# Ghostish/Open3DSOT

Hardware: AMD Instinct MI355X
Metric: template/search pairs/sec (fwd+bwd), BAT KITTI-Car 512/1024 pts (higher is better)
Workload: dtype f32; 1 GPU; BAT_Car.yaml KITTI-Car, template 512 / search 1024 pts, batch 48 per GPU, fwd+bwd+Adam, fp32; global_batch=48, parallelism=dp1, fused_kernels=True, hip_graph=True, rccl_world_size=1

## Files before the change

include/o3dsot.h:

```cpp
#ifndef O3DSOT_H_
#define O3DSOT_H_

#include <stdint.h>

#ifdef __cplusplus
extern "C" {
#endif

#define O3D_OK 0
#define O3D_EINVAL (-1)
#define O3D_ELAUNCH (-2)

const char* o3d_version(void);

int o3d_furthest_point_sampling(const float* xyz, int B, int N, int npoint, float* temp,
                                int32_t* idx, void* stream);

int o3d_furthest_point_sampling_shfl(const float* xyz, int B, int N, int npoint, float* temp, int32_t* idx,
                                     void* stream);

int o3d_furthest_point_sampling_pair(const float* xyz0, int N0, int npoint0, int32_t* idx0, const float* xyz1,
                                     int N1, int npoint1, int32_t* idx1, int B, void* stream);

int o3d_gather_points(const float* feats, const int32_t* idx, int B, int C, int N, int npoint,
                      float* out, void* stream);
int o3d_gather_points_grad(const float* grad_out, const int32_t* idx, int B, int C, int N,
                           int npoint, float* grad_feats, void* stream);

int o3d_gather_rows(const float* src, const int32_t* idx, int B, int N, int D, int npoint, float* out, void* stream);

int o3d_gather_rows2(const float* a, int Da, const float* b, int Db, const int32_t* idx, long ld_idx, int B, int N, int npoint,
                     float* outa, float* outb, void* stream);

int o3d_ball_query(const float* new_xyz, const float* xyz, int B, int N, int npoint, float radius,
                   int nsample, int32_t* idx, void* stream);

int o3d_sample_query(const float* xyz0, const int32_t* sidx0, int N0, int npoint0, int32_t* idx0, const float* xyz1,
                     const int32_t* sidx1, int N1, int npoint1, int32_t* idx1, int B, float radius, int nsample,
                     float* centers, void* stream);

int o3d_group_points(const float* feats, const int32_t* idx, int B, int C, int N, int npoint,
                     int nsample, float* out, void* stream);
int o3d_group_points_grad(const float* grad_out, const int32_t* idx, int B, int C, int N,
                          int npoint, int nsample, float* grad_feats, void* stream);

int o3d_three_nn(const float* unknown, const float* known, int B, int n, int m, float* dist2,
                 int32_t* idx, void* stream);
int o3d_three_interpolate(const float* feats, const int32_t* idx, const float* weight, int B,
                          int c, int m, int n, float* out, void* stream);
int o3d_three_interpolate_grad(const float* grad_out, const int32_t* idx, const float* weight,
                               int B, int c, int n, int m, float* grad_feats, void* stream);

int o3d_knn(const float* query, const float* ref, int B, int Q, int R, int D, int k,
            int32_t* idx, void* stream);



int o3d_mlp_conv_fwd(const float* X, const float* W, const float* in_scale, const float* in_shift,
                     int B, int Cin, int Cout, int P, float* Y, float* part, const float* stat_c,
                     void* stream);

typedef struct {
    const float* part; int nparts, C; double count; const float* stat_c; const float* gamma; const float* beta;
    float* running_mean; float* running_var; float momentum, eps; float* mean; float* invstd; float* scale; float* shift;
    const int32_t* meta; int tile, nparts1; double count1;
} o3d_bn_fin_args;
int o3d_bn_finalize(const o3d_bn_fin_args* jobs, int njobs, void* stream);

int o3d_bn_relu_maxpool_fwd(const float* Y, const float* scale, const float* shift, int B, int C,
                            int npoint, int ns, float* out, int32_t* arg, float* yarg, void* stream);

int o3d_pool_bwd_partials_split(const float* dOut, const float* out, const float* yarg, const float* mean, int C,
                                int npoint, int nsplit, float* part, const int32_t* arg, float* pk, void* stream);

typedef struct {
    const float* part; int nparts, C; double count; const float* gamma; const float* mean; const float* invstd;
    float* dgamma; float* dbeta; float* A1; float* A2; float* A3;
    const int32_t* meta; int tile, nparts1; double count1;
} o3d_bn_bwd_fin_args;
int o3d_bn_bwd_finalize(const o3d_bn_bwd_fin_args* jobs, int njobs, void* stream);

int o3d_mlp_conv_dgrad(const float* dN, const float* dOut, const float* out, const int32_t* arg,
                       int ns, const float* Y, const float* A1, const float* A2, const float* A3,
                       const float* W, int B, int Cin, int Cout, int P, const float* Yprev,
                       const float* scale_p, const float* shift_p, const float* mean_p,
                       float* dNprev, float* part, void* stream);

int o3d_mlp_conv_dgrad_wt(const float* dN, const float* dOut, const float* out, const int32_t* arg,
                          int ns, const float* Y, const float* A1, const float* A2, const float* A3,
                          const float* W, const float* Wt, const float* pk, int B, int Cin, int Cout, int P,
                          const float* Yprev, const float* scale_p, const float* shift_p,
                          const float* mean_p, float* dNprev, float* part, void* stream);

int o3d_mlp_conv_dgrad_plain(const float* dN, const float* Y, const float* A1, const float* A2,
                             const float* A3, const float* W, int B, int Cin, int Cout, int P,
                             float* dX, void* stream);

int o3d_mlp_conv_wgrad(const float* dN, const float* dOut, const float* out, const int32_t* arg, int ns,
                       const float* Y, const float* A1, const float* A2, const float* A3,
                       const float* X, const float* in_scale, const float* in_shift, int B, int Cin, int Cout,
                       int P, int nslices, float* part, float* dW, void* stream);


int o3d_compact_build(const int32_t* idx, int B, int npoint, int ns, int ld, int col_base, int pt_base,
                      int ball_base, int dummy_ball, int32_t* ball_cnt, int32_t* ball_off, int32_t* gp,
                      int32_t* cball, float* cw, int32_t* meta, void* stream);

int o3d_group_dw0_xyz(const float* dN, const float* Y0, long ldp, const float* A1, const float* A2, const float* A3,
                      const int32_t* gp, const int32_t* cball, const float* cw, const float* X, long ldz,
                      const float* centers, const int32_t* meta, long start1, int C0, float* part, float* dW, void* stream);

int o3d_compact_build2(const int32_t* idx0, int npoint0, int ld0, const int32_t* idx1, int npoint1, int ld1, int B,
                       int ns, int col_base1, int pt_base1, int dummy_ball, int32_t* ball_cnt, int32_t* ball_off,
                       int32_t* gp, int32_t* cball, float* cw, int32_t* meta, void* stream);

int o3d_group_expand_c(const float* Z, long ldz, const int32_t* gp, const int32_t* cball, const float* cw,
                       const float* centers, const float* W0, int ldw, int C0, const int32_t* meta, long start1,
                       long ldp, float* Y0, float* part, const float* stat_c, void* stream);

int o3d_group_expand_c3(const float* X3, long ldz, const int32_t* gp, const int32_t* cball, const float* cw,
                        const float* centers, const float* W0, int ldw, int C0, const int32_t* meta, long start1, long ldp,
                        float* Y0, float* part, const float* stat_c, void* stream);

int o3d_direct_tile(long P, int M, int compact);
int o3d_direct_tail_slots(int M);
int o3d_direct_tail_override(int slots);
int o3d_direct_class(long ldp, int M, int K, int tile);
int o3d_mlp_conv_fwd_c(const float* X, const float* W, const float* in_scale, const float* in_shift, int Cin,
                       int Cout, long ldp, const float* w, const int32_t* meta, long start1, int tile, float* Y,
                       float* part, const float* stat_c, void* stream);
int o3d_mlp_conv_dgrad_c(const float* dN, const float* Y, const float* A1, const float* A2, const float* A3,
                         const float* Wt, int Cin, int Cout, long ldp, const float* w, const int32_t* meta,
                         long start1, int tile, const float* Yprev, const float* scale_p, const float* shift_p,
                         const float* mean_p, float* dNprev, float* part, void* stream);
int o3d_mlp_conv_wgrad2_c(const float* dN, const float* Y, const float* A1, const float* A2, const float* A3,
                          const float* X, const float* in_scale, const float* in_shift, int Cin, int Cout,
                          long ldp, const float* w, const int32_t* meta, long start1, float* scratch, float* dW,
                          void* stream);

int o3d_pool_fwd_c(const float* Y, long ldp, const float* scale, const float* shift, const int32_t* ball_off,
                   const int32_t* ball_cnt, int B, int C, int npoint0, int npoint1, float* out, int32_t* argq,
                   float* yarg, void* stream);

int o3d_pool_fwd_ct(const float* Y, long ldp, const float* scale, const float* shift, const int32_t* ball_off,
                    const int32_t* ball_cnt, const int32_t* cball, const int32_t* meta, long start1, int B, int C,
                    int npoint0, int npoint1, int nsample, float* out, int32_t* argq, float* yarg, void* stream);

#define O3D_POOL_BWD_SPLIT 8
int o3d_pool_bwd_c(const float* dOut, const float* out, const int32_t* argq, const float* yarg,
                   const float* mean, int B, int C, int npoint0, int npoint1, const int32_t* meta, long start1,
                   long ldp, float* D, float* part, void* stream);

int o3d_pool_bwd_dense(const float* dOut0, long sb0, long sc0, const float* dOut1, long sb1, long sc1, const float* out,
                       const int32_t* argq, const float* yarg, const float* mean,
                       const int32_t* cball, const int32_t* ball_off, const int32_t* meta, long start1, long ldp, int B,
                       int C, int npoint0, int npoint1, float* D, float* part, void* stream);

long o3d_group_reduce_gather_scratch(int B, int nseg, int npoint0, int ld0, int npoint1, int ld1, int spanmax);
int o3d_group_reduce_gather(const float* dN, const float* Y0, long ldp, const float* A1, const float* A2,
                            const float* A3, const int32_t* gp, const float* cw, const int32_t* ball_off,
                            const int32_t* ball_cnt, int B, int nseg, int npoint0, int ld0, int npoint1, int ld1, int C0,
                            int spanmax, int32_t* perm, int32_t* poff, float* S, float* T, void* stream);

int o3d_pack_points(const float* xyz0, const float* feats0, int N0, int ld0, const float* xyz1, const float* feats1,
                    int N1, int ld1, int B, int nxyz, int C, float inv_radius, int rows, float* X0, void* stream);

int o3d_center_term(const float* T, const float* centers, int C0, int nballs, int ldw, float* dW, void* stream);
int o3d_center_term_out(const float* T, const float* centers, int C0, int nballs, int ldw, const float* dW, int ncols,
                        float* out, void* stream);

int o3d_center_grad(const float* T, const float* W0, int ldw, int C0, int nballs, float scale, float* out, void* stream);

int o3d_group_reduce_c(const float* dN, const float* Y0, long ldp, const float* A1, const float* A2,
                       const float* A3, const int32_t* gp, const int32_t* cball, const float* cw,
                       const int32_t* ball_off, const int32_t* ball_cnt, int B, int nseg, int npoint0, int ld0,
                       int npoint1, int ld1, int C0, float* S, float* T, void* stream);

int o3d_bn_relu_apply(const float* Y, const float* scale, const float* shift, int C, long P, float* out,
                      void* stream);
int o3d_act_bwd_partials(const float* g, const float* Y, const float* scale, const float* shift,
                         const float* mean, int C, long P, float* dN, float* part, void* stream);
int o3d_gmax_fwd(const float* Y, const float* scale, const float* shift, int B, int C, int N, float* out,
                 int32_t* argq, float* yarg, void* stream);

long o3d_mlp_conv_wgrad2_scratch(int B, int Cin, int Cout, int P);
int o3d_mlp_conv_wgrad2(const float* dN, const float* pk, int ns, const float* Y, const float* A1,
                        const float* A2, const float* A3, const float* X, const float* in_scale,
                        const float* in_shift, int B, int Cin, int Cout, int P, float* scratch, float* dW,
                        void* stream);

typedef struct { const float* p; long sb, sc, sn; int C; } o3d_rows_src;

int o3d_pack_rows(const o3d_rows_src* srcs, int nsrc, int B, int N, int rows, float* X, void* stream);
int o3d_pack_rows_ld(const o3d_rows_src* srcs, int nsrc, int B, int N, int rows, float* X, long ld, void* stream);

int o3d_rpn_votes_fwd(const float* cla, long cla_sb, long cla_sn, const float* vote, long v_sb, long v_sc, long v_sn, int B, int N,
                      int f, float* score, float* vote_xyz, float* vote_feature, void* stream);
int o3d_rpn_votes_bwd(const float* score, const float* dvf, long f_sb, long f_sc, long f_sn, const float* dvx, long x_sb, long x_sc,
                      long x_sn, int B, int N, int f, float* dcla, float* dvote, void* stream);
int o3d_box_assemble(const float* offsets, long o_sb, long o_sc, long o_sn, const float* centers, int B, int P, float* boxes,
                     void* stream);

int o3d_prep_weights(const long* jobs, int njobs, void* stream);

int o3d_row_sum(const float* G, int C, long P, float* out, void* stream);

int o3d_pw_tile(long P, int M);
int o3d_pw_class(long P, int M, int K);

int o3d_mlp_conv_bwd_fused_rows(int Cin, int Cout, long P);
long o3d_mlp_conv_bwd_fused_scratch(int Cin, int Cout, long P);
int o3d_mlp_conv_bwd_fused_c(const float* dN, const float* Y, const float* A1, const float* A2, const float* A3,
                             const float* X, const float* in_scale, const float* in_shift, const float* in_mean,
                             const float* Wt, int Cin, int Cout, long ldp, const float* w, const int32_t* meta,
                             long start1, float* scratch, float* dW, float* part_s, float* dNprev, void* stream);

typedef struct {
    const float* X; const float* W; const float* in_scale; const float* in_shift; const float* bias; const float* resid;
    int Cin, Cout; long P;
    float* Y; float* part; const float* stat_c;
} o3d_pw_fwd_args;
typedef struct {
    const float* dN; const float* Y; const float* A1; const float* A2; const float* A3; const float* Wt;
    int Cin, Cout; long P;
    const float* Yprev; const float* scale_p; const float* shift_p; const float* mean_p; const float* resid;
    float* dNprev; float* part;
} o3d_pw_dgrad_args;
int o3d_pw_fwd_pair(const o3d_pw_fwd_args* a, const o3d_pw_fwd_args* b, void* stream);
int o3d_pw_dgrad_pair(const o3d_pw_dgrad_args* a, const o3d_pw_dgrad_args* b, void* stream);

typedef struct {
    const float* dN; const float* Y; const float* A1; const float* A2; const float* A3;
    const float* X; const float* in_scale; const float* in_shift;
    int Cin, Cout; long P;
    float* scratch; float* dW;
    int out_rows, out_cols;
} o3d_wgrad_job;
int o3d_mlp_conv_wgrad2_group(const o3d_wgrad_job* jobs, int njobs, void* stream);

int o3d_adam_step(const long* jobs, int njobs, float* params, float* exp_avg, float* exp_avg_sq, double lr,
                  double beta1, double beta2, double eps, double weight_decay, double bc1, double bc2, void* stream);

int o3d_best_proposal(const float* boxes, int B, int P, float* out, int32_t* out_idx, void* stream);

int o3d_pw_fwd_cloud(const float* X, const float* W, const float* cbias, int B, int N, int Cin, int Cout, float* Y,
                     float* part, const float* stat_c, void* stream);
int o3d_cloud_sum_dy(const float* dN, const float* Y, const float* A1, const float* A2, const float* A3, int C, int B,
                     int N, float* out, void* stream);

int o3d_bn_eval_consts(const float* running_mean, const float* running_var, const float* gamma, const float* beta,
                       const float* conv_bias, float eps, int C, int nrep, float* vec, void* stream);

int o3d_pw_fwd(const float* X, const float* W, const float* in_scale, const float* in_shift, const float* bias,
               const float* resid, int Cin, int Cout, long P, float* Y, float* part, const float* stat_c,
               void* stream);

int o3d_pw_dgrad(const float* dN, const float* Y, const float* A1, const float* A2, const float* A3,
                 const float* Wt, int Cin, int Cout, long P, const float* Yprev, const float* scale_p,
                 const float* shift_p, const float* mean_p, const float* resid, float* dNprev, float* part,
                 void* stream);

int o3d_xcorr_expand(const float* Z, long ldz, const float* sim, const float* W0, int ldw, int B, int M, int N, int C0,
                     float* Y0, float* part, const float* stat_c, void* stream);

long o3d_xcorr_reduce_groups(int C0);
int o3d_xcorr_reduce(const float* dN, const float* Y0, const float* A1, const float* A2, const float* A3,
                     const float* sim, const float* W0, int ldw, int B, int M, int N, int C0, float* S, long lds,
                     float* dsim_part, float* dw_part, void* stream);

int o3d_sa_eval_fused(const float* Z, long ldz, const int32_t* idx, const float* centers, const float* W0, int ldw,
                      const float* v0, const float* W1, const float* v1, const float* W2, const float* v2, int C0, int C1,
                      int C2, int B, int np, int ns, int ld, long pt_base, float* out, void* stream);

int o3d_cosine_sim_fwd(const float* t, long tsb, long tsc, long tsn, const float* s, long ssb, long ssc, long ssn, int B, int f,
                       int M, int N, float* sim, float* tn, float* sn, void* stream);
// ... 166 lines not shown
```

open3dsot_amd/csrc/compact.hip:

```cpp
#include <cstdlib>
#include "o3d_common.hpp"

namespace {

__global__ __launch_bounds__(256) void compact_count_kernel(const int32_t* __restrict__ idx, long nslots, int ns,
                                                            int32_t* __restrict__ ball_cnt) {
    const long s = (long)blockIdx.x * 256 + threadIdx.x;
    const int lane = threadIdx.x & 63;
    const int v = s < nslots ? idx[s] : -1;
    const int base = lane & ~(ns - 1), k = lane - base;
    const int first = __shfl(v, base, 64);
    const unsigned long long m = __ballot(v != first);
    const unsigned long long seg = ns == 64 ? ~0ull : (((1ull << ns) - 1) << base);
    const unsigned long long other = m & seg;
    if (k == 0 && s < nslots) ball_cnt[s / ns] = other ? (63 - __clzll((long long)other)) - base + 1 : 1;
}

__global__ __launch_bounds__(1024) void compact_scan_kernel(const int32_t* __restrict__ ball_cnt, int n,
                                                            int col_base, int32_t* __restrict__ ball_off,
                                                            int32_t* __restrict__ meta) {
    __shared__ int sh[1024];
    const int per = (n + 1023) / 1024;
    const int i0 = threadIdx.x * per;
    int local = 0;
    for (int i = i0; i < i0 + per && i < n; ++i) local += ball_cnt[i];
    sh[threadIdx.x] = local;
    __syncthreads();
    for (int off = 1; off < 1024; off <<= 1) {
        const int v = (int)threadIdx.x >= off ? sh[threadIdx.x - off] : 0;
        __syncthreads();
        sh[threadIdx.x] += v;
        __syncthreads();
    }
    int run = col_base + sh[threadIdx.x] - local;
    for (int i = i0; i < i0 + per && i < n; ++i) {
        ball_off[i] = run;
        run += ball_cnt[i];
    }
    if (threadIdx.x == 1023) {
        const int tot = sh[1023];
        meta[0] = (tot + 255) & ~255;
        meta[1] = tot;
        meta[2] = n;
        meta[3] = 0;
    }
}

__global__ __launch_bounds__(256) void compact_fill_kernel(const int32_t* __restrict__ idx, long nslots, int ns,
                                                           int npoint, int ld, int col_base, int pt_base,
                                                           int ball_base, int dummy_ball,
                                                           const int32_t* __restrict__ ball_cnt,
                                                           const int32_t* __restrict__ ball_off,
                                                           const int32_t* __restrict__ meta,
                                                           int32_t* __restrict__ gp, int32_t* __restrict__ cball,
                                                           float* __restrict__ cw) {
    if (blockIdx.x == gridDim.x - 1) {
        const int q = meta[1] + threadIdx.x;
        if (q < meta[0]) { gp[col_base + q] = 0; cball[col_base + q] = dummy_ball; cw[col_base + q] = 0.f; }
        return;
    }
    const long s = (long)blockIdx.x * 256 + threadIdx.x;
    if (s >= nslots) return;
    const int ball = (int)(s / ns), k = (int)(s - (long)ball * ns);
    const int cnt = ball_cnt[ball];
    if (k >= cnt) return;
    const int q = ball_off[ball] + k;
    gp[q] = pt_base + (ball / npoint) * ld + idx[s];
    cball[q] = ball_base + ball;
    cw[q] = k == 0 ? (float)(1 + ns - cnt) : 1.f;
}

template <bool CENTERS, bool DIRECT = false>
__global__ __launch_bounds__(256) void expand_c_kernel(const float* __restrict__ Z, long ldz,
                                                       const int32_t* __restrict__ gp,
                                                       const int32_t* __restrict__ cball,
                                                       const float* __restrict__ cw,
                                                       const float* __restrict__ centers,
                                                       const float* __restrict__ W0, int ldw, int C0,
                                                       const int32_t* __restrict__ meta, long start1, long ldp,
                                                       float* __restrict__ Y0, float* __restrict__ part,
                                                       const float* __restrict__ stat_c) {
    const int q0 = blockIdx.x * 256;
    const int seg = (start1 > 0 && q0 >= start1) ? 1 : 0;
    if (q0 - (seg ? start1 : 0) >= meta[4 * seg]) return;
    if (stat_c && seg) stat_c += C0;
    const int lane = threadIdx.x & 63, wave = threadIdx.x >> 6;
    const int q = q0 + 4 * lane;
    const int4 id = *reinterpret_cast<const int4*>(&gp[q]);
    const float4 w = *reinterpret_cast<const float4*>(&cw[q]);
    float cx[4] = {0.f, 0.f, 0.f, 0.f}, cy[4] = {0.f, 0.f, 0.f, 0.f}, cz[4] = {0.f, 0.f, 0.f, 0.f};
    if constexpr (CENTERS) {
        const int4 bj = *reinterpret_cast<const int4*>(&cball[q]);
        const int bb[4] = {bj.x, bj.y, bj.z, bj.w};
#pragma unroll
        for (int t = 0; t < 4; ++t) {
            const float* c = centers + (long)bb[t] * 3;
            cx[t] = c[0]; cy[t] = c[1]; cz[t] = c[2];
        }
        if constexpr (DIRECT) {
            const int ids[4] = {id.x, id.y, id.z, id.w};
#pragma unroll
            for (int t = 0; t < 4; ++t) { cx[t] -= Z[ids[t]]; cy[t] -= Z[ldz + ids[t]]; cz[t] -= Z[2 * ldz + ids[t]]; }
        }
    }
    constexpr int EG = 8;
    const int cper = (C0 + gridDim.y - 1) / gridDim.y;
    const int cbeg = blockIdx.y * cper, cend = cbeg + cper < C0 ? cbeg + cper : C0;
    for (int g0 = cbeg + wave; g0 < cend; g0 += 4 * EG) {
        float4 y[EG];
        float w0[EG], w1[EG], w2[EG], sc_[EG];
#pragma unroll
        for (int g = 0; g < EG; ++g) {
            const int co = g0 + 4 * g < cend ? g0 + 4 * g : cend - 1;
            if constexpr (DIRECT) {
                y[g] = make_float4(0.f, 0.f, 0.f, 0.f);
            } else {
                const float* z = Z + (long)co * ldz;
                y[g].x = z[id.x]; y[g].y = z[id.y]; y[g].z = z[id.z]; y[g].w = z[id.w];
            }
            w0[g] = w1[g] = w2[g] = 0.f;
            if constexpr (CENTERS) { const float* wr = W0 + (long)co * ldw; w0[g] = wr[0]; w1[g] = wr[1]; w2[g] = wr[2]; }
            sc_[g] = (part && stat_c) ? stat_c[co] : 0.f;
        }
        float s[EG], v[EG];
#pragma unroll
        for (int g = 0; g < EG; ++g) {
            const int co = g0 + 4 * g;
            if (co >= cend) { s[g] = 0.f; v[g] = 0.f; continue; }
            y[g].x -= fmaf(w2[g], cz[0], fmaf(w1[g], cy[0], w0[g] * cx[0]));
            y[g].y -= fmaf(w2[g], cz[1], fmaf(w1[g], cy[1], w0[g] * cx[1]));
            y[g].z -= fmaf(w2[g], cz[2], fmaf(w1[g], cy[2], w0[g] * cx[2]));
            y[g].w -= fmaf(w2[g], cz[3], fmaf(w1[g], cy[3], w0[g] * cx[3]));
            *reinterpret_cast<float4*>(&Y0[(long)co * ldp + q]) = y[g];
            const float c = sc_[g];
            s[g] = fmaf(w.x, y[g].x, fmaf(w.y, y[g].y, fmaf(w.z, y[g].z, w.w * y[g].w)));
            v[g] = w.x * (y[g].x - c) * (y[g].x - c) + w.y * (y[g].y - c) * (y[g].y - c) +
                   w.z * (y[g].z - c) * (y[g].z - c) + w.w * (y[g].w - c) * (y[g].w - c);
        }
        if (part) {
#pragma unroll
            for (int g = 0; g < EG; ++g) { s[g] = wave_sum(s[g]); v[g] = wave_sum(v[g]); }
            if (lane == 0)
#pragma unroll
                for (int g = 0; g < EG; ++g) {
                    const int co = g0 + 4 * g;
                    if (co < cend) {
                        part[((long)blockIdx.x * 2 + 0) * C0 + co] = s[g];
                        part[((long)blockIdx.x * 2 + 1) * C0 + co] = v[g];
                    }
                }
        }
    }
}

constexpr int POOL_BWD_SPLIT = 8;

__device__ __forceinline__ long pool_index(int c, int ball, int C, int seg1_ball, int np0, int np1) {
    const bool s1 = ball >= seg1_ball;
    const int local = s1 ? ball - seg1_ball : ball, np = s1 ? np1 : np0;
    const int b = local / np, j = local - b * np;
    return (s1 ? (long)seg1_ball * C : 0) + ((long)b * C + c) * np + j;
}

template <int POOL_CH>
__global__ __launch_bounds__(256) void pool_c_kernel(const float* __restrict__ Y, long ldp,
                                                     const float* __restrict__ scale,
                                                     const float* __restrict__ shift,
                                                     const int32_t* __restrict__ ball_off,
                                                     const int32_t* __restrict__ ball_cnt, int C, int seg1_ball,
                                                     int np0, int np1, int nballs, float* __restrict__ out,
                                                     int32_t* __restrict__ argq, float* __restrict__ yarg) {
    const int e = threadIdx.x & 7;
    int ball = blockIdx.x * 32 + (threadIdx.x >> 3);
    const bool live = ball < nballs;
    if (!live) ball = nballs - 1;
    const int q0 = ball_off[ball], q1 = q0 + ball_cnt[ball];
    const int c0 = blockIdx.y * POOL_CH;
    if (ball >= seg1_ball) { scale += C; shift += C; }
    constexpr int PU = 4;
    float v[POOL_CH][PU], sc[POOL_CH], sf[POOL_CH];
#pragma unroll
    for (int cc = 0; cc < POOL_CH; ++cc) {
        const int c = c0 + cc < C ? c0 + cc : C - 1;
        const float* y = Y + (long)c * ldp;
#pragma unroll
        for (int i = 0; i < PU; ++i) {
            const int q = q0 + e + 8 * i;
            v[cc][i] = y[q < q1 ? q : q1 - 1];
        }
        sc[cc] = scale[c];
        sf[cc] = shift[c];
    }
    float rbest[POOL_CH], ryb[POOL_CH];
    int rbq[POOL_CH];
#pragma unroll
    for (int cc = 0; cc < POOL_CH; ++cc) {
        float best = -INFINITY, yb = 0.f;
        int bq = 0x7fffffff;
#pragma unroll
        for (int i = 0; i < PU; ++i) {
            const int q = q0 + e + 8 * i;
            const float n = fmaf(v[cc][i], sc[cc], sf[cc]);
            if (q < q1 && n > best) { best = n; bq = q; yb = v[cc][i]; }
        }
        if (q1 - q0 > 8 * PU) {
            const float* y = Y + (long)(c0 + cc < C ? c0 + cc : C - 1) * ldp;
            for (int q = q0 + e + 8 * PU; q < q1; q += 8) {
                const float w = y[q], n = fmaf(w, sc[cc], sf[cc]);
                if (n > best) { best = n; bq = q; yb = w; }
            }
        }
        {
            const float ob = dpp_f<0xB1>(best), oy = dpp_f<0xB1>(yb);
            const int oq = dpp_i<0xB1>(bq);
            if (ob > best || (ob == best && oq < bq)) { best = ob; bq = oq; yb = oy; }
        }
        {
            const float ob = dpp_f<0x4E>(best), oy = dpp_f<0x4E>(yb);
            const int oq = dpp_i<0x4E>(bq);
            if (ob > best || (ob == best && oq < bq)) { best = ob; bq = oq; yb = oy; }
        }
        {
            const float ob = dpp_f<0x141>(best), oy = dpp_f<0x141>(yb);
            const int oq = dpp_i<0x141>(bq);
            if (ob > best || (ob == best && oq < bq)) { best = ob; bq = oq; yb = oy; }
        }
        rbest[cc] = best; ryb[cc] = yb; rbq[cc] = bq;
    }
    if (live && e == 0) {
#pragma unroll
        for (int cc = 0; cc < POOL_CH; ++cc) {
            const int c = c0 + cc;
            if (c < C) {
                const long o = pool_index(c, ball, C, seg1_ball, np0, np1);
                out[o] = fmaxf(rbest[cc], 0.f);
                if (argq) { argq[o] = rbq[cc]; yarg[o] = ryb[cc]; }
            }
        }
    }
}

constexpr int PT_CH = 32, PT_COLS = 128, PT_OVER = 32, PT_LD = PT_COLS + PT_OVER + 3;
constexpr int PT_RB = 32, PT_RLD = PT_CH + 1;

__device__ __forceinline__ void pool_t_item(const float* __restrict__ Y, long ldp,
                                            const float* __restrict__ scale, const float* __restrict__ shift,
                                            const int32_t* __restrict__ ball_off,
                                            const int32_t* __restrict__ ball_cnt,
                                            const int32_t* __restrict__ cball,
                                            const int32_t* __restrict__ meta, long start1, int C,
                                            int seg1_ball, int np0, int np1, int nballs,
                                            float* __restrict__ out, int32_t* __restrict__ argq,
                                            float* __restrict__ yarg, const long q0, const int c0, float* pt_tile) {
    int* pt_off = reinterpret_cast<int*>(pt_tile + PT_CH * PT_LD);
    int* pt_cnt = pt_off + PT_COLS;
    int* pt_ob = pt_cnt + PT_COLS;
    float* pt_res = reinterpret_cast<float*>(pt_ob + PT_COLS);
    const int seg = (start1 > 0 && q0 >= start1) ? 1 : 0;
    const long sbase = seg ? start1 : 0;
    if (q0 - sbase >= meta[4 * seg]) return;
    const long qend = sbase + meta[4 * seg + 1];
    if (q0 >= qend) return;
    int bfirst = cball[q0];
    if (ball_off[bfirst] < q0) ++bfirst;
    const long qlast = (q0 + PT_COLS < qend ? q0 + PT_COLS : qend) - 1;
    const int blast = cball[qlast];
    const int nb = blast - bfirst + 1;
    const int np = seg ? np1 : np0;
    const long segbase = seg ? (long)seg1_ball * C : 0;
    const int ball0 = seg ? seg1_ball : 0;
    constexpr int F4 = (PT_COLS + PT_OVER) / 4;
    constexpr int NLD = PT_CH * F4 / 256;
    static_assert(PT_CH * F4 % 256 == 0, "tile loads must divide evenly over the workgroup");
    {
        float4 v[NLD];
        int bo = 0, bc = 0;
        if ((int)threadIdx.x < nb) { bo = ball_off[bfirst + threadIdx.x]; bc = ball_cnt[bfirst + threadIdx.x]; }
#pragma unroll
        for (int u = 0; u < NLD; ++u) {
            const int i = threadIdx.x + 256 * u;
            const int r = i / F4, f = i - r * F4;
            long q = q0 + 4 * f;
            if (q + 4 > ldp) q = ldp - 4;
            v[u] = *reinterpret_cast<const float4*>(&Y[(long)(c0 + r) * ldp + q]);
        }
        __builtin_amdgcn_sched_barrier(0);
// ... 456 lines not shown
#pragma unroll
            for (int c = 0; c < CS; ++c) {
                d[it][c] = *reinterpret_cast<const float4*>(&dN[(long)crow[c] * ldp + qc]);
                y[it][c] = *reinterpret_cast<const float4*>(&Y0[(long)crow[c] * ldp + qc]);
            }
        }
        __builtin_amdgcn_sched_barrier(0);
        __syncthreads();
#pragma unroll
        for (int it = 0; it < CH / 1024; ++it) {
            const int i = 4 * threadIdx.x + 1024 * it;
#pragma unroll
            for (int c = 0; c < CS; ++c) {
                float4 o;
                o.x = fmaf(a1[c], d[it][c].x, w4[it].x * fmaf(a2[c], y[it][c].x, a3[c]));
                o.y = fmaf(a1[c], d[it][c].y, w4[it].y * fmaf(a2[c], y[it][c].y, a3[c]));
                o.z = fmaf(a1[c], d[it][c].z, w4[it].z * fmaf(a2[c], y[it][c].z, a3[c]));
                o.w = fmaf(a1[c], d[it][c].w, w4[it].w * fmaf(a2[c], y[it][c].w, a3[c]));
                *reinterpret_cast<float4*>(&dy[c * CH + i]) = o;
            }
        }
#pragma unroll
        for (int u = 0; u < CH / 256; ++u) lst[threadIdx.x + 256 * u] = ent[u];
        __syncthreads();
        {
            const int per = (cnt + 255) / 256;
            const int e0 = threadIdx.x * per, e1 = e0 + per < cnt ? e0 + per : cnt;
            int cur = -1;
            float sr[CS];
#pragma unroll
            for (int c = 0; c < CS; ++c) sr[c] = 0.f;
            for (int a = e0; a < e1; ++a) {
                const int e = lst[a];
                const int n = e >> 16, i = e & 0xffff;
                if (n != cur) {
                    if (cur >= 0) {
#pragma unroll
                        for (int c = 0; c < CS; ++c) atomicAdd(&sacc[c * ld + cur], sr[c]);
                    }
                    cur = n;
#pragma unroll
                    for (int c = 0; c < CS; ++c) sr[c] = 0.f;
                }
#pragma unroll
                for (int c = 0; c < CS; ++c) sr[c] += dy[c * CH + i];
            }
            if (cur >= 0) {
#pragma unroll
                for (int c = 0; c < CS; ++c) atomicAdd(&sacc[c * ld + cur], sr[c]);
            }
        }
        if (T)
            for (int j = threadIdx.x; j < npoint; j += 256) {
                const int b0 = ball_off[bbase + j], b1 = b0 + ball_cnt[bbase + j];
                const int s0 = b0 > lo ? b0 : lo, s1 = b1 < hi ? b1 : hi;
                if (s0 >= s1) continue;
                float t[CS];
#pragma unroll
                for (int c = 0; c < CS; ++c) t[c] = 0.f;
                for (int q = s0; q < s1; ++q)
#pragma unroll
                    for (int c = 0; c < CS; ++c) t[c] += dy[c * CH + (q - lo)];
#pragma unroll
                for (int c = 0; c < CS; ++c) tacc[c * npoint + j] += t[c];
            }
    }
    __syncthreads();
    for (int i = threadIdx.x; i < CS * ld; i += 256) {
        const int c = i / ld, n = i - c * ld;
        if (c0 + c < C0) S[(long)(c0 + c) * lds_row + pbase + n] = sacc[i];
    }
    if (T)
        for (int i = threadIdx.x; i < CS * npoint; i += 256) {
            const int c = i / npoint, j = i - c * npoint;
            if (c0 + c < C0) T[(long)(c0 + c) * nballs + bbase + j] = tacc[i];
        }
}

__global__ __launch_bounds__(1024) void center_term_kernel(const float* __restrict__ T,
                                                           const float* __restrict__ centers, int nballs, int ldw,
                                                           float* __restrict__ dW, float* __restrict__ out = nullptr,
                                                           int ncols = 0) {
    __shared__ float red[16][3];
    const int c = blockIdx.x, tid = threadIdx.x;
    const float* t = T + (long)c * nballs;
    float s0 = 0.f, s1 = 0.f, s2 = 0.f;
    for (int ball = tid; ball < nballs; ball += 1024) {
        const float v = t[ball];
        s0 = fmaf(v, centers[3 * ball], s0);
        s1 = fmaf(v, centers[3 * ball + 1], s1);
        s2 = fmaf(v, centers[3 * ball + 2], s2);
    }
#pragma unroll
    for (int off = 32; off >= 1; off >>= 1) {
        s0 += __shfl_xor(s0, off, 64);
        s1 += __shfl_xor(s1, off, 64);
        s2 += __shfl_xor(s2, off, 64);
    }
    if ((tid & 63) == 0) { red[tid >> 6][0] = s0; red[tid >> 6][1] = s1; red[tid >> 6][2] = s2; }
    __syncthreads();
    if (tid < 3) {
        float a = 0.f;
#pragma unroll
        for (int w = 0; w < 16; ++w) a += red[w][tid];
        if (out) out[(long)c * ncols + tid] = dW[(long)c * ldw + tid] - a;
        else dW[(long)c * ldw + tid] -= a;
    }
    if (out)
        for (int k = 3 + tid; k < ncols; k += 1024) out[(long)c * ncols + k] = dW[(long)c * ldw + k];
}

struct PackSeg { const float* xyz; const float* feats; int N, ld; };

__global__ __launch_bounds__(256) void pack_points_kernel(PackSeg s0, PackSeg s1, int B, int nxyz, int C, float inv_radius,
                                                          long ldz, float* __restrict__ X0) {
    const long col = (long)blockIdx.x * 256 + threadIdx.x;
    if (col >= ldz) return;
    const int r = blockIdx.y;
    const long base1 = (long)B * s0.ld;
    const bool second = col >= base1;
    const PackSeg sg = second ? s1 : s0;
    const long local = second ? col - base1 : col;
    const int b = (int)(local / sg.ld), n = (int)(local - (long)b * sg.ld);
    float v = 0.f;
    if (n < sg.N) {
        if (r < nxyz) v = sg.xyz[((long)b * sg.N + n) * 3 + r] * inv_radius;
        else if (r < nxyz + C) v = sg.feats[((long)b * C + (r - nxyz)) * sg.N + n];
    }
    X0[(long)r * ldz + col] = v;
}

}

static bool pow2(int v) { return v > 0 && (v & (v - 1)) == 0; }
constexpr long O3D_MAX_BALLS = 1L << 20;

extern "C" int o3d_compact_build(const int32_t* idx, int B, int npoint, int ns, int ld, int col_base, int pt_base,
                                 int ball_base, int dummy_ball, int32_t* ball_cnt, int32_t* ball_off, int32_t* gp,
                                 int32_t* cball, float* cw, int32_t* meta, void* stream) {
    const long nballs = (long)B * npoint, nslots = nballs * ns;
    if (!idx || !ball_cnt || !ball_off || !gp || !cball || !cw || !meta || B <= 0 || npoint <= 0 || ns < 1 ||
        ns > 64 || !pow2(ns) || nballs > O3D_MAX_BALLS || nslots % 256 != 0 || ld <= 0 || col_base < 0 || col_base % 256 != 0)
        return O3D_EINVAL;
    hipStream_t s = o3d_stream(stream);
    const int blocks = (int)(nslots / 256);
    hipLaunchKernelGGL(compact_count_kernel, dim3(blocks), dim3(256), 0, s, idx, nslots, ns, ball_cnt);
    hipLaunchKernelGGL(compact_scan_kernel, dim3(1), dim3(1024), 0, s, ball_cnt, (int)nballs, col_base, ball_off, meta);
    hipLaunchKernelGGL(compact_fill_kernel, dim3(blocks + 1), dim3(256), 0, s, idx, nslots, ns, npoint, ld, col_base,
                       pt_base, ball_base, dummy_ball, ball_cnt, ball_off, meta, gp, cball, cw);
    return o3d_launch_status();
}

namespace {
template <int CPW>
__global__ __launch_bounds__(256) void dw0_xyz_kernel(const float* __restrict__ dN, const float* __restrict__ Y0, long ldp,
                                                      const float* __restrict__ A1, const float* __restrict__ A2,
                                                      const float* __restrict__ A3, const int32_t* __restrict__ gp,
                                                      const int32_t* __restrict__ cball, const float* __restrict__ cw,
                                                      const float* __restrict__ X, long ldz,
                                                      const float* __restrict__ centers,
                                                      const int32_t* __restrict__ meta, long start1, int C0,
                                                      float* __restrict__ part) {
    const long q0 = (long)blockIdx.x * 256;
    const int seg = (start1 > 0 && q0 >= start1) ? 1 : 0;
    float* prow = part + (long)blockIdx.x * C0 * 3;
    if (q0 - (seg ? start1 : 0) >= meta[4 * seg]) {
        for (int i = threadIdx.x; i < C0 * 3; i += 256) prow[i] = 0.f;
        return;
    }
    const int lane = threadIdx.x & 63, wave = threadIdx.x >> 6;
    const long q = q0 + 4 * lane;
    const int4 id = *reinterpret_cast<const int4*>(&gp[q]);
    const int4 bj = *reinterpret_cast<const int4*>(&cball[q]);
    const float4 w = *reinterpret_cast<const float4*>(&cw[q]);
    const int ids[4] = {id.x, id.y, id.z, id.w}, bb[4] = {bj.x, bj.y, bj.z, bj.w};
    const float wv[4] = {w.x, w.y, w.z, w.w};
    float rel[4][3];
#pragma unroll
    for (int t = 0; t < 4; ++t)
#pragma unroll
        for (int k = 0; k < 3; ++k)
            rel[t][k] = wv[t] != 0.f ? X[(long)k * ldz + ids[t]] - centers[(long)bb[t] * 3 + k] : 0.f;
    const float* a1 = A1 + seg * C0;
    const float* a2 = A2 + seg * C0;
    const float* a3 = A3 + seg * C0;
    for (int cbase = 0; cbase < C0; cbase += 4 * CPW) {
        float acc[CPW][3];
        float4 d[CPW], y[CPW];
#pragma unroll
        for (int i = 0; i < CPW; ++i) {
            const int c = cbase + wave + 4 * i;
            const int cc = c < C0 ? c : C0 - 1;
            d[i] = *reinterpret_cast<const float4*>(&dN[(long)cc * ldp + q]);
            y[i] = *reinterpret_cast<const float4*>(&Y0[(long)cc * ldp + q]);
        }
#pragma unroll
        for (int i = 0; i < CPW; ++i) {
            const int c = cbase + wave + 4 * i;
            const int cc = c < C0 ? c : C0 - 1;
            const float k1 = a1[cc], k2 = a2[cc], k3 = a3[cc];
            const float dv[4] = {d[i].x, d[i].y, d[i].z, d[i].w}, yv[4] = {y[i].x, y[i].y, y[i].z, y[i].w};
            float s0 = 0.f, s1 = 0.f, s2 = 0.f;
#pragma unroll
            for (int t = 0; t < 4; ++t) {
                const float dy = wv[t] != 0.f ? fmaf(k1, dv[t], wv[t] * fmaf(k2, yv[t], k3)) : 0.f;
                s0 = fmaf(dy, rel[t][0], s0); s1 = fmaf(dy, rel[t][1], s1); s2 = fmaf(dy, rel[t][2], s2);
            }
            acc[i][0] = s0; acc[i][1] = s1; acc[i][2] = s2;
        }
#pragma unroll
        for (int i = 0; i < CPW; ++i) {
            const int c = cbase + wave + 4 * i;
#pragma unroll
            for (int k = 0; k < 3; ++k) {
                const float t = wave_sum(acc[i][k]);
                if (lane == 0 && c < C0) prow[c * 3 + k] = t;
            }
        }
    }
}

__global__ __launch_bounds__(256) void dw0_reduce_kernel(const float* __restrict__ part, int nblk, int n,
                                                         float* __restrict__ out) {
    __shared__ float sh[4];
    const int i = blockIdx.x;
    float s = 0.f;
    for (int r = threadIdx.x; r < nblk; r += 256) s += part[(long)r * n + i];
    s = wave_sum(s);
    if ((threadIdx.x & 63) == 0) sh[threadIdx.x >> 6] = s;
    __syncthreads();
    if (threadIdx.x == 0) out[i] = (sh[0] + sh[1]) + (sh[2] + sh[3]);
}
}

extern "C" int o3d_group_dw0_xyz(const float* dN, const float* Y0, long ldp, const float* A1, const float* A2,
                                 const float* A3, const int32_t* gp, const int32_t* cball, const float* cw,
                                 const float* X, long ldz, const float* centers, const int32_t* meta, long start1, int C0,
                                 float* part, float* dW, void* stream) {
    if (!dN || !Y0 || !A1 || !A2 || !A3 || !gp || !cball || !cw || !X || !centers || !meta || !part || !dW || C0 <= 0 ||
        ldp <= 0 || ldp % 256 != 0 || ldz <= 0 || start1 < 0 || start1 % 256 != 0)
        return O3D_EINVAL;
    hipStream_t s = o3d_stream(stream);
    const int nblk = (int)(ldp / 256);
    hipLaunchKernelGGL(dw0_xyz_kernel<8>, dim3(nblk), dim3(256), 0, s, dN, Y0, ldp, A1, A2, A3, gp, cball, cw, X, ldz, centers,
                       meta, start1, C0, part);
    hipLaunchKernelGGL(dw0_reduce_kernel, dim3(C0 * 3), dim3(256), 0, s, part, nblk, C0 * 3, dW);
    return o3d_launch_status();
}

namespace {
struct CompactSeg {
    const int32_t* idx; long nslots; int npoint, ld, col_base, pt_base, ball_base, nballs;
    int32_t* ball_cnt; int32_t* ball_off; int32_t* meta;
};

__global__ __launch_bounds__(256) void compact_count2_kernel(CompactSeg s0, CompactSeg s1, int ns, int blocks0) {
    const bool second = (int)blockIdx.x >= blocks0;
    const CompactSeg& sg = second ? s1 : s0;
    const long s = (long)(blockIdx.x - (second ? blocks0 : 0)) * 256 + threadIdx.x;
    const int lane = threadIdx.x & 63;
    const int v = s < sg.nslots ? sg.idx[s] : -1;
    const int base = lane & ~(ns - 1), k = lane - base;
    const int first = __shfl(v, base, 64);
    const unsigned long long m = __ballot(v != first);
    const unsigned long long seg = ns == 64 ? ~0ull : (((1ull << ns) - 1) << base);
    const unsigned long long other = m & seg;
    if (k == 0 && s < sg.nslots) sg.ball_cnt[s / ns] = other ? (63 - __clzll((long long)other)) - base + 1 : 1;
}

__global__ __launch_bounds__(1024) void compact_scan2_kernel(CompactSeg s0, CompactSeg s1) {
    const CompactSeg& sg = blockIdx.x ? s1 : s0;
    const int n = sg.nballs;
    __shared__ int sh[1024];
    const int per = (n + 1023) / 1024;
    const int i0 = threadIdx.x * per;
    int local = 0;
    for (int i = i0; i < i0 + per && i < n; ++i) local += sg.ball_cnt[i];
    sh[threadIdx.x] = local;
    __syncthreads();
    for (int off = 1; off < 1024; off <<= 1) {
        const int v = (int)threadIdx.x >= off ? sh[threadIdx.x - off] : 0;
        __syncthreads();
        sh[threadIdx.x] += v;
        __syncthreads();
    }
    int run = sg.col_base + sh[threadIdx.x] - local;
    for (int i = i0; i < i0 + per && i < n; ++i) {
        sg.ball_off[i] = run;
        run += sg.ball_cnt[i];
    }
    if (threadIdx.x == 1023) {
        const int tot = sh[1023];
        sg.meta[0] = (tot + 255) & ~255;
        sg.meta[1] = tot;
        sg.meta[2] = n;
        sg.meta[3] = 0;
    }
}

__global__ __launch_bounds__(256) void compact_fill2_kernel(CompactSeg s0, CompactSeg s1, int ns, int blocks0, int dummy_ball,
                                                            int32_t* __restrict__ gp, int32_t* __restrict__ cball,
                                                            float* __restrict__ cw) {
    const bool second = (int)blockIdx.x >= blocks0 + 1;
    const CompactSeg& sg = second ? s1 : s0;
    const int blk = blockIdx.x - (second ? blocks0 + 1 : 0);
    const int nblk = (int)(sg.nslots / 256);
    if (blk == nblk) {
        const int q = sg.meta[1] + threadIdx.x;
        if (q < sg.meta[0]) { gp[sg.col_base + q] = 0; cball[sg.col_base + q] = dummy_ball; cw[sg.col_base + q] = 0.f; }
        return;
    }
    const long s = (long)blk * 256 + threadIdx.x;
    if (s >= sg.nslots) return;
    const int ball = (int)(s / ns), k = (int)(s - (long)ball * ns);
    const int cnt = sg.ball_cnt[ball];
    if (k >= cnt) return;
    const int q = sg.ball_off[ball] + k;
    gp[q] = sg.pt_base + (ball / sg.npoint) * sg.ld + sg.idx[s];
    cball[q] = sg.ball_base + ball;
    cw[q] = k == 0 ? (float)(1 + ns - cnt) : 1.f;
}
}

extern "C" int o3d_compact_build2(const int32_t* idx0, int npoint0, int ld0, const int32_t* idx1, int npoint1, int ld1,
                                  int B, int ns, int col_base1, int pt_base1, int dummy_ball, int32_t* ball_cnt,
                                  int32_t* ball_off, int32_t* gp, int32_t* cball, float* cw, int32_t* meta, void* stream) {
    const long nb0 = (long)B * npoint0, nb1 = (long)B * npoint1;
    if (!idx0 || !idx1 || !ball_cnt || !ball_off || !gp || !cball || !cw || !meta || B <= 0 || npoint0 <= 0 ||
        npoint1 <= 0 || ns < 1 || ns > 64 || !pow2(ns) || nb0 > O3D_MAX_BALLS || nb1 > O3D_MAX_BALLS || (nb0 * ns) % 256 != 0 ||
        (nb1 * ns) % 256 != 0 || ld0 <= 0 || ld1 <= 0 || col_base1 < 0 || col_base1 % 256 != 0 || pt_base1 < 0)
        return O3D_EINVAL;
    CompactSeg s0 = {idx0, nb0 * ns, npoint0, ld0, 0, 0, 0, (int)nb0, ball_cnt, ball_off, meta};
    CompactSeg s1 = {idx1, nb1 * ns, npoint1, ld1, col_base1, pt_base1, (int)nb0, (int)nb1, ball_cnt + nb0, ball_off + nb0,
                     meta + 4};
    hipStream_t s = o3d_stream(stream);
    const int b0 = (int)(s0.nslots / 256), b1 = (int)(s1.nslots / 256);
    hipLaunchKernelGGL(compact_count2_kernel, dim3(b0 + b1), dim3(256), 0, s, s0, s1, ns, b0);
    hipLaunchKernelGGL(compact_scan2_kernel, dim3(2), dim3(1024), 0, s, s0, s1);
    hipLaunchKernelGGL(compact_fill2_kernel, dim3(b0 + b1 + 2), dim3(256), 0, s, s0, s1, ns, b0, dummy_ball, gp, cball, cw);
    return o3d_launch_status();
}

extern "C" int o3d_group_expand_c(const float* Z, long ldz, const int32_t* gp, const int32_t* cball,
                                  const float* cw, const float* centers, const float* W0, int ldw, int C0,
                                  const int32_t* meta, long start1, long ldp, float* Y0, float* part,
                                  const float* stat_c, void* stream) {
    if (!Z || !gp || !cball || !cw || !meta || !Y0 || C0 <= 0 || ldp <= 0 || ldp % 256 != 0 || start1 < 0 ||
        start1 % 256 != 0 || (centers && (!W0 || ldw < 3)))
        return O3D_EINVAL;
    const int ysplit = C0 >= 128 ? 4 : C0 >= 64 ? 2 : 1;
    if (centers)
        hipLaunchKernelGGL(expand_c_kernel<true>, dim3((unsigned)(ldp / 256), ysplit), dim3(256), 0, o3d_stream(stream), Z,
                           ldz, gp, cball, cw, centers, W0, ldw, C0, meta, start1, ldp, Y0, part, stat_c);
    else
        hipLaunchKernelGGL(expand_c_kernel<false>, dim3((unsigned)(ldp / 256), ysplit), dim3(256), 0, o3d_stream(stream), Z,
                           ldz, gp, cball, cw, centers, W0, ldw, C0, meta, start1, ldp, Y0, part, stat_c);
    return o3d_launch_status();
}

extern "C" int o3d_group_expand_c3(const float* X3, long ldz, const int32_t* gp, const int32_t* cball, const float* cw,
                                   const float* centers, const float* W0, int ldw, int C0, const int32_t* meta,
                                   long start1, long ldp, float* Y0, float* part, const float* stat_c, void* stream) {
    if (!X3 || !gp || !cball || !cw || !centers || !W0 || ldw < 3 || !meta || !Y0 || C0 <= 0 || ldp <= 0 ||
        ldp % 256 != 0 || start1 < 0 || start1 % 256 != 0)
        return O3D_EINVAL;
    const int ysplit = C0 >= 128 ? 4 : C0 >= 64 ? 2 : 1;
    hipLaunchKernelGGL((expand_c_kernel<true, true>), dim3((unsigned)(ldp / 256), ysplit), dim3(256), 0, o3d_stream(stream),
                       X3, ldz, gp, cball, cw, centers, W0, ldw, C0, meta, start1, ldp, Y0, part, stat_c);
    return o3d_launch_status();
}

extern "C" int o3d_pool_fwd_c(const float* Y, long ldp, const float* scale, const float* shift,
                              const int32_t* ball_off, const int32_t* ball_cnt, int B, int C, int npoint0,
                              int npoint1, float* out, int32_t* argq, float* yarg, void* stream) {
    if (!Y || !scale || !shift || !ball_off || !ball_cnt || !out || B <= 0 || C <= 0 || npoint0 <= 0 || npoint1 < 0 ||
        (argq && !yarg))
        return O3D_EINVAL;
    const int seg1_ball = B * npoint0, nballs = B * (npoint0 + npoint1);
    constexpr int POOL_CH = 8;
    hipLaunchKernelGGL(pool_c_kernel<8>, dim3(o3d_cdiv(nballs, 32), o3d_cdiv(C, POOL_CH)), dim3(256), 0,
                       o3d_stream(stream), Y, ldp, scale, shift, ball_off, ball_cnt, C, seg1_ball, npoint0,
                       npoint1 > 0 ? npoint1 : npoint0, nballs, out, argq, yarg);
    return o3d_launch_status();
}

extern "C" int o3d_pool_fwd_ct(const float* Y, long ldp, const float* scale, const float* shift, const int32_t* ball_off,
                               const int32_t* ball_cnt, const int32_t* cball, const int32_t* meta, long start1, int B, int C,
                               int npoint0, int npoint1, int nsample, float* out, int32_t* argq, float* yarg, void* stream) {
    if (!Y || !scale || !shift || !ball_off || !ball_cnt || !cball || !meta || !out || B <= 0 || C <= 0 || C % PT_CH != 0 ||
        npoint0 <= 0 || npoint1 < 0 || nsample < 1 || nsample > PT_OVER || (argq && !yarg) || ldp < PT_COLS + PT_OVER ||
        ldp % PT_COLS != 0 || start1 < 0 || start1 % PT_COLS != 0)
        return O3D_EINVAL;
    const int seg1_ball = B * npoint0, nballs = B * (npoint0 + npoint1);
    const size_t lds = sizeof(float) * (PT_CH * PT_LD + 3 * PT_RB * PT_RLD) + sizeof(int) * 3 * PT_COLS;
    static const bool attr_ok = hipFuncSetAttribute(reinterpret_cast<const void*>(pool_t_kernel),
                                                    hipFuncAttributeMaxDynamicSharedMemorySize, (int)lds) == hipSuccess;
    if (!attr_ok) return O3D_ELAUNCH;
    const long worst = (ldp / PT_COLS) * (C / PT_CH);
    hipLaunchKernelGGL(pool_t_kernel, dim3((unsigned)(worst < PT_GRID ? worst : PT_GRID)), dim3(256), lds, o3d_stream(stream), Y, ldp,
                       scale, shift, ball_off, ball_cnt, cball, meta, start1, C, seg1_ball, npoint0,
                       npoint1 > 0 ? npoint1 : npoint0, nballs, out, argq, yarg);
    return o3d_launch_status();
}

extern "C" int o3d_pool_bwd_c(const float* dOut, const float* out, const int32_t* argq, const float* yarg,
                              const float* mean, int B, int C, int npoint0, int npoint1, const int32_t* meta,
                              long start1, long ldp, float* D, float* part, void* stream) {
    if (!dOut || !out || !argq || !yarg || !mean || !meta || !D || !part || B <= 0 || C <= 0 || npoint0 <= 0 ||
        npoint1 < 0 || ldp <= 0 || ldp % 4 != 0)
        return O3D_EINVAL;
    hipStream_t s = o3d_stream(stream);
    const int nseg = npoint1 > 0 ? 2 : 1;
    const int seg1_ball = B * npoint0, nballs = B * (npoint0 + npoint1), np1 = npoint1 > 0 ? npoint1 : npoint0;
    hipLaunchKernelGGL(zero_cols_kernel, dim3((unsigned)o3d_cdiv(ldp, 1024), C), dim3(256), 0, s, D, ldp, meta, start1);
    hipLaunchKernelGGL(pool_bwd_partials_c_kernel, dim3(C, nseg, POOL_BWD_SPLIT), dim3(256), 0, s, dOut, out, yarg, mean, C,
                       nballs, seg1_ball, npoint0, np1, part, argq, D, ldp);
    return o3d_launch_status();
}

extern "C" int o3d_pool_bwd_dense(const float* dOut0, long sb0, long sc0, const float* dOut1, long sb1, long sc1,
                                  const float* out, const int32_t* argq, const float* yarg,
                                  const float* mean, const int32_t* cball, const int32_t* ball_off, const int32_t* meta,
                                  long start1, long ldp, int B, int C, int npoint0, int npoint1, float* D, float* part,
                                  void* stream) {
    if (!out || !argq || !yarg || !mean || !cball || !ball_off || !meta || !D || !part || B <= 0 || C <= 0 ||
        C % PBD_CH != 0 || npoint0 <= 0 || npoint1 < 0 || ldp <= 0 || ldp % PBD_COLS != 0 || start1 < 0 ||
        start1 % PBD_COLS != 0 || ldp > 0x7fffffffL)
        return O3D_EINVAL;
    const int seg1_ball = B * npoint0, np1 = npoint1 > 0 ? npoint1 : npoint0;
    const PoolGrad g0 = {dOut0, sb0, sc0}, g1 = {dOut1, sb1, sc1};
    PoolBwdDense a = {g0, g1, out, argq, yarg, mean, cball, ball_off, meta, npoint1 > 0 ? start1 : 0, ldp, C,
                      B * (npoint0 + npoint1), seg1_ball, npoint0, np1, D, part};
    const long worst = (ldp / PBD_COLS) * (C / PBD_CH);
    const unsigned grid = (unsigned)(worst < PBD_GRID ? worst : PBD_GRID);
    hipLaunchKernelGGL(pool_bwd_dense_kernel, dim3(grid), dim3(256), 0, o3d_stream(stream), a);
    return o3d_launch_status();
}

template <int CS, int BT = 256>
static int launch_reduce_c(const float* dN, const float* Y0, long ldp, const float* A1, const float* A2,
                           const float* A3, const int32_t* gp, const int32_t* cball, const float* cw,
                           const int32_t* ball_off, const int32_t* ball_cnt, int B, int nseg, SegParams sp0,
                           SegParams sp1, int C0,
                           long lds_row, int nballs, float* S, float* T, hipStream_t s) {
    const int span = (sp0.ld + sp0.npoint) > (sp1.ld + sp1.npoint) ? (sp0.ld + sp0.npoint) : (sp1.ld + sp1.npoint);
    const size_t lds = sizeof(float) * CS * (size_t)span;
    if (lds > 64 * 1024) return O3D_EINVAL;
    if (lds > 48 * 1024 &&
        hipFuncSetAttribute(reinterpret_cast<const void*>(reduce_c_kernel<CS, BT>),
                            hipFuncAttributeMaxDynamicSharedMemorySize, (int)lds) != hipSuccess)
        return O3D_ELAUNCH;
    const int slabs = (C0 + CS - 1) / CS;
    hipLaunchKernelGGL((reduce_c_kernel<CS, BT>), dim3(B * nseg * slabs), dim3(BT), lds, s, dN, Y0, ldp, A1, A2, A3, gp, cball,
                       cw, ball_off, ball_cnt, B, sp0, sp1, C0, lds_row, S, T, nballs);
    return o3d_launch_status();
}

extern "C" int o3d_group_reduce_c(const float* dN, const float* Y0, long ldp, const float* A1, const float* A2,
                                  const float* A3, const int32_t* gp, const int32_t* cball, const float* cw,
                                  const int32_t* ball_off, const int32_t* ball_cnt, int B, int nseg, int npoint0,
                                  int ld0, int npoint1, int ld1, int C0, float* S, float* T, void* stream) {
    if (!dN || !Y0 || !A1 || !A2 || !A3 || !gp || !cball || !cw || !ball_off || !ball_cnt || !S || B <= 0 || npoint0 <= 0 ||
        ld0 <= 0 || C0 <= 0 || (nseg != 1 && nseg != 2) || (nseg == 2 && (npoint1 <= 0 || ld1 <= 0)))
        return O3D_EINVAL;
    hipStream_t s = o3d_stream(stream);
    const SegParams sp0 = {npoint0, ld0, 0, 0};
    const SegParams sp1 = nseg == 2 ? SegParams{npoint1, ld1, B * ld0, B * npoint0} : sp0;
    const long lds_row = (long)B * ld0 + (nseg == 2 ? (long)B * ld1 : 0);
    const int nballs = B * npoint0 + (nseg == 2 ? B * npoint1 : 0);
    return launch_reduce_c<1>(dN, Y0, ldp, A1, A2, A3, gp, cball, cw, ball_off, ball_cnt, B, nseg, sp0, sp1, C0,
                              lds_row, nballs, S, T, s);
}

extern "C" int o3d_center_term(const float* T, const float* centers, int C0, int nballs, int ldw, float* dW,
                               void* stream) {
    if (!T || !centers || !dW || C0 <= 0 || nballs <= 0 || ldw < 3) return O3D_EINVAL;
    hipLaunchKernelGGL(center_term_kernel, dim3(C0), dim3(1024), 0, o3d_stream(stream), T, centers, nballs, ldw, dW,
                       static_cast<float*>(nullptr), 0);
    return o3d_launch_status();
}

extern "C" int o3d_center_term_out(const float* T, const float* centers, int C0, int nballs, int ldw, const float* dW,
                                   int ncols, float* out, void* stream) {
    if (!T || !centers || !dW || !out || C0 <= 0 || nballs <= 0 || ncols < 3 || ldw < ncols) return O3D_EINVAL;
    hipLaunchKernelGGL(center_term_kernel, dim3(C0), dim3(1024), 0, o3d_stream(stream), T, centers, nballs, ldw,
                       const_cast<float*>(dW), out, ncols);
    return o3d_launch_status();
}

namespace {
__global__ __launch_bounds__(256) void center_grad_kernel(const float* __restrict__ T, const float* __restrict__ W0, int ldw, int C0,
                                                          int nballs, float scale, float* __restrict__ out) {
    const int ball = blockIdx.x * 256 + threadIdx.x;
    if (ball >= nballs) return;
    float s0 = 0.f, s1 = 0.f, s2 = 0.f;
#pragma unroll 8
    for (int c = 0; c < C0; ++c) {
        const float t = T[(long)c * nballs + ball];
        s0 = fmaf(W0[(long)c * ldw + 0], t, s0);
        s1 = fmaf(W0[(long)c * ldw + 1], t, s1);
        s2 = fmaf(W0[(long)c * ldw + 2], t, s2);
    }
    out[ball] = scale * s0;
    out[(long)nballs + ball] = scale * s1;
    out[2L * nballs + ball] = scale * s2;
}
}

extern "C" int o3d_center_grad(const float* T, const float* W0, int ldw, int C0, int nballs, float scale, float* out, void* stream) {
    if (!T || !W0 || !out || C0 <= 0 || nballs <= 0 || ldw < 3) return O3D_EINVAL;
    hipLaunchKernelGGL(center_grad_kernel, dim3(o3d_cdiv(nballs, 256)), dim3(256), 0, o3d_stream(stream), T, W0, ldw, C0, nballs,
                       scale, out);
    return o3d_launch_status();
}

extern "C" int o3d_pack_points(const float* xyz0, const float* feats0, int N0, int ld0, const float* xyz1,
                               const float* feats1, int N1, int ld1, int B, int nxyz, int C, float inv_radius, int rows,
                               float* X0, void* stream) {
    if (!X0 || B <= 0 || N0 <= 0 || ld0 < N0 || N1 < 0 || (N1 > 0 && ld1 < N1) || (nxyz != 0 && nxyz != 3) || C < 0 ||
        rows < nxyz + C || (nxyz && (!xyz0 || (N1 > 0 && !xyz1))) || (C && (!feats0 || (N1 > 0 && !feats1))))
        return O3D_EINVAL;
// ... 56 lines not shown
```

open3dsot_amd/csrc/mlp_direct.hip:

```cpp
#include <type_traits>
#include "mlp_common.hpp"

namespace {

constexpr int DT_M = 64;

template <int NT>
__device__ __forceinline__ void ldv(float (&d)[NT], const float* p) {
    if constexpr (NT == 4) {
        const float4 t = *reinterpret_cast<const float4*>(p);
        d[0] = t.x; d[1] = t.y; d[2] = t.z; d[3] = t.w;
    } else if constexpr (NT == 2) {
        const float2 t = *reinterpret_cast<const float2*>(p);
        d[0] = t.x; d[1] = t.y;
    } else {
        d[0] = *p;
    }
}
template <int NT>
__device__ __forceinline__ void stv(float* p, const float (&d)[NT]) {
    if constexpr (NT == 4)      *reinterpret_cast<float4*>(p) = make_float4(d[0], d[1], d[2], d[3]);
    else if constexpr (NT == 2) *reinterpret_cast<float2*>(p) = make_float2(d[0], d[1]);
    else                        *p = d[0];
}

template <int NT>
struct RawB {
    float v[4][NT];
    float y[4][NT];
    float4 c1, c2, c3;
};

enum BMode { B_PLAIN = 0, B_XFORM = 1, B_DY = 2, B_DYPOOL = 3 };

struct DirectArgs {
    const float* A;
    const float* X;
    const float* Y;
    const float* c1; const float* c2; const float* c3;
    const float2* pk; int ns;
    float* Out;
    int M, K, P, B;
    const float* w;
    const int32_t* meta;
    long start1;
    float* part;
    const float* stat_c;
    const float* Yprev; const float* scale_p; const float* shift_p; const float* mean_p;
    const float* bias;
    const float* resid;
    const float* cbias; int cb_N, cb_B;
    int tail_slots; long extra_row0;
};

template <int MODE, int NT>
__device__ __forceinline__ void load_b(const DirectArgs& a, const float* xb, const float* yb, long rowP, int kb,
                                       long pool_base, int np, RawB<NT>& f) {
#pragma unroll
    for (int s = 0; s < 4; ++s) {
        if (MODE != B_DYPOOL) ldv<NT>(f.v[s], xb + (long)(kb + s) * rowP);
        if (MODE >= B_DY) ldv<NT>(f.y[s], yb + (long)(kb + s) * rowP);
        if constexpr (MODE == B_DYPOOL && NT >= 2) {
            const float2 t = a.pk[pool_base + (long)(kb + s) * np];
            f.v[s][0] = t.x; f.v[s][1] = t.y;
        }
    }
    if (MODE != B_PLAIN) {
        f.c1 = *reinterpret_cast<const float4*>(a.c1 + kb);
        f.c2 = *reinterpret_cast<const float4*>(a.c2 + kb);
        if (MODE >= B_DY) f.c3 = *reinterpret_cast<const float4*>(a.c3 + kb);
    }
}

template <int MODE, int NT, int MT>
__device__ __forceinline__ void compute_group(const RawB<NT>& f, const float4& a0v, const float4& a1v, int kk,
                                              const float (&wv)[NT], f32x16 (&acc)[MT][NT]) {
    const float a0[4] = {a0v.x, a0v.y, a0v.z, a0v.w}, a1[4] = {a1v.x, a1v.y, a1v.z, a1v.w};
    const float c1[4] = {f.c1.x, f.c1.y, f.c1.z, f.c1.w}, c2[4] = {f.c2.x, f.c2.y, f.c2.z, f.c2.w};
    const float c3[4] = {f.c3.x, f.c3.y, f.c3.z, f.c3.w};
#pragma unroll
    for (int s = 0; s < 4; ++s) {
        float bv[NT];
        if constexpr (MODE == B_DYPOOL && NT >= 2) {
            const float go = f.v[s][0];
            const int ak = __float_as_int(f.v[s][1]);
#pragma unroll
            for (int t = 0; t < NT; ++t) bv[t] = (kk + t == ak) ? go : 0.f;
        } else {
#pragma unroll
            for (int t = 0; t < NT; ++t) bv[t] = f.v[s][t];
        }
        if (MODE == B_XFORM) {
#pragma unroll
            for (int t = 0; t < NT; ++t) bv[t] = fmaxf(fmaf(bv[t], c1[s], c2[s]), 0.f);
        } else if (MODE >= B_DY) {
#pragma unroll
            for (int t = 0; t < NT; ++t) bv[t] = fmaf(c1[s], bv[t], wv[t] * fmaf(c2[s], f.y[s][t], c3[s]));
        }
#pragma unroll
        for (int t = 0; t < NT; ++t) {
            acc[0][t] = mfma32(a0[s], bv[t], acc[0][t]);
            if constexpr (MT == 2) acc[1][t] = mfma32(a1[s], bv[t], acc[1][t]);
        }
    }
}

template <int WAVES, int MODE, int EPI, int NT, int MT = 2>
__device__ __forceinline__ void direct_gemm_body(DirectArgs& a, const int bx, const int by, const long part_row = -1) {
    constexpr int POS = 32 * NT;
    constexpr int DT_MW = 32 * MT;
    const int lane = threadIdx.x & 63, wave = threadIdx.x >> 6;
    const int l31 = lane & 31, h = lane >> 5;
    const int tiles_per_b = a.P / POS;
    const int tile = bx;
    const int b = tile / tiles_per_b, p0 = (tile - b * tiles_per_b) * POS;
    if (a.meta) {
        const long c0 = (long)tile * POS;
        const int seg = (a.start1 > 0 && c0 >= a.start1) ? 1 : 0;
        if (c0 - (seg ? a.start1 : 0) >= a.meta[4 * seg]) return;
        if (seg) {
            if (a.c1) a.c1 += a.K;
            if (a.c2) a.c2 += a.K;
            if (a.c3) a.c3 += a.K;
            if (a.stat_c) a.stat_c += a.M;
            if (a.scale_p) { a.scale_p += a.M; a.shift_p += a.M; a.mean_p += a.M; }
        }
    }
    const int m0 = (by * WAVES + wave) * DT_MW;
    const int p = p0 + NT * l31;
    float wv[NT];
#pragma unroll
    for (int t = 0; t < NT; ++t) wv[t] = 1.f;
    if (a.w) ldv<NT>(wv, a.w + (long)b * a.P + p);
    const long rowP = a.P;
    const float* xb = (MODE != B_DYPOOL) ? a.X + (long)b * a.K * rowP + p : nullptr;
    const float* yb = (MODE >= B_DY) ? a.Y + (long)b * a.K * rowP + p : nullptr;
    const float* wa = a.A + (long)(m0 + l31) * a.K + 4 * h;
    const long wstep = 32L * a.K;
    int np = 1, kk = 0;
    long pool_base = 0;
    if (MODE == B_DYPOOL) {
        np = a.P / a.ns;
        const int j = p / a.ns;
        kk = p - j * a.ns;
        pool_base = (long)b * a.K * np + j;
    }

    f32x16 acc[MT][NT];
#pragma unroll
    for (int i = 0; i < MT; ++i)
#pragma unroll
        for (int t = 0; t < NT; ++t)
#pragma unroll
            for (int r = 0; r < 16; ++r) acc[i][t][r] = 0.f;

    const int G = a.K / 8;
    RawB<NT> f[2];
    float4 wa0[2], wa1[2];
    auto load = [&](auto stc, int g) {
        constexpr int st = decltype(stc)::value;
        const int kb = 8 * g + 4 * h;
        load_b<MODE, NT>(a, xb, yb, rowP, kb, pool_base, np, f[st]);
        wa0[st] = *reinterpret_cast<const float4*>(wa + 8 * g);
        if constexpr (MT == 2) wa1[st] = *reinterpret_cast<const float4*>(wa + 8 * g + wstep);
        else wa1[st] = wa0[st];
    };
    {
        load(std::integral_constant<int, 0>{}, 0);
        for (int g = 0; g < G; g += 2) {
            load(std::integral_constant<int, 1>{}, g + 1);
            __builtin_amdgcn_sched_barrier(0);
            compute_group<MODE, NT, MT>(f[0], wa0[0], wa1[0], kk, wv, acc);
            __builtin_amdgcn_sched_barrier(0);
            load(std::integral_constant<int, 0>{}, g + 2 < G ? g + 2 : G - 1);
            __builtin_amdgcn_sched_barrier(0);
            compute_group<MODE, NT, MT>(f[1], wa0[1], wa1[1], kk, wv, acc);
            __builtin_amdgcn_sched_barrier(0);
        }
    }

    int cloud = 0;
    if constexpr (EPI == 3) cloud = (int)(((long)b * a.P + p0) / a.cb_N);
    const bool stats = EPI != 2 && a.part != nullptr;
    float4 kc1[MT][4], kc2[MT][4];
    if constexpr (EPI != 1) {
#pragma unroll
        for (int i = 0; i < MT; ++i)
#pragma unroll
            for (int q = 0; q < 4; ++q) {
                const int mb = m0 + 32 * i + 4 * h + 8 * q;
                kc1[i][q] = kc2[i][q] = make_float4(0.f, 0.f, 0.f, 0.f);
                if constexpr (EPI == 2) {
                    if (a.bias) kc1[i][q] = *reinterpret_cast<const float4*>(a.bias + mb);
                } else {
                    if (a.stat_c) kc1[i][q] = *reinterpret_cast<const float4*>(a.stat_c + mb);
                    if constexpr (EPI == 3) {
                        kc2[i][q].x = a.cbias[(long)(mb + 0) * a.cb_B + cloud];
                        kc2[i][q].y = a.cbias[(long)(mb + 1) * a.cb_B + cloud];
                        kc2[i][q].z = a.cbias[(long)(mb + 2) * a.cb_B + cloud];
                        kc2[i][q].w = a.cbias[(long)(mb + 3) * a.cb_B + cloud];
                    }
                }
            }
    }
#pragma unroll
    for (int i = 0; i < MT; ++i) {
        float red[32];
#pragma unroll
        for (int hb = 0; hb < 2; ++hb) {
            const int mb = m0 + 32 * i + 16 * hb + 4 * h;
            const long ob = ((long)b * a.M + mb) * rowP + p;
            float ex[8][NT];
            float4 k1[2], k2[2], k3[2];
            if constexpr (EPI == 1 || EPI == 2) {
                const float* src = EPI == 1 ? a.Yprev : a.resid;
#pragma unroll
                for (int r = 0; r < 8; ++r) {
#pragma unroll
                    for (int t = 0; t < NT; ++t) ex[r][t] = 0.f;
                    if (EPI == 1 || src) ldv<NT>(ex[r], src + ob + (long)(8 * (r >> 2) + (r & 3)) * rowP);
                }
            }
#pragma unroll
            for (int q = 0; q < 2; ++q) {
                k3[q] = make_float4(0.f, 0.f, 0.f, 0.f);
                if constexpr (EPI == 1) {
                    k1[q] = *reinterpret_cast<const float4*>(a.scale_p + mb + 8 * q);
                    k2[q] = *reinterpret_cast<const float4*>(a.shift_p + mb + 8 * q);
                    k3[q] = *reinterpret_cast<const float4*>(a.mean_p + mb + 8 * q);
                } else {
                    k1[q] = kc1[i][2 * hb + q];
                    k2[q] = kc2[i][2 * hb + q];
                }
            }
#pragma unroll
            for (int r8 = 0; r8 < 8; ++r8) {
                const int q = r8 >> 2, j = r8 & 3, r = 8 * hb + r8;
                const float c1 = j == 0 ? k1[q].x : j == 1 ? k1[q].y : j == 2 ? k1[q].z : k1[q].w;
                const float c2 = j == 0 ? k2[q].x : j == 1 ? k2[q].y : j == 2 ? k2[q].z : k2[q].w;
                const float c3 = j == 0 ? k3[q].x : j == 1 ? k3[q].y : j == 2 ? k3[q].z : k3[q].w;
                float v[NT];
#pragma unroll
                for (int t = 0; t < NT; ++t) v[t] = acc[i][t][r];
                float s1 = 0.f, s2 = 0.f;
                if constexpr (EPI == 1) {
#pragma unroll
                    for (int t = 0; t < NT; ++t) {
                        v[t] = fmaf(ex[r8][t], c1, c2) > 0.f ? v[t] : 0.f;
                        s1 += v[t];
                        s2 = fmaf(v[t], ex[r8][t] - c3, s2);
                    }
                } else if constexpr (EPI == 2) {
#pragma unroll
                    for (int t = 0; t < NT; ++t) v[t] = (v[t] + c1) + ex[r8][t];
                } else {
#pragma unroll
                    for (int t = 0; t < NT; ++t) {
                        if constexpr (EPI == 3) v[t] += c2;
                        s1 = fmaf(wv[t], v[t], s1);
                        s2 += wv[t] * (v[t] - c1) * (v[t] - c1);
                    }
                }
                stv<NT>(a.Out + ob + (long)(8 * q + j) * rowP, v);
                red[r] = s1;
                red[16 + r] = s2;
            }
        }
        if (stats) {
            reduce_scatter32(red, l31);
            a.part[(part_row >= 0 ? part_row : (long)tile) * 2 * a.M + (long)(l31 >> 4) * a.M + m0 + 32 * i + acc_row(l31 & 15, h)] = red[0];
        }
    }
}


template <int WAVES, int MODE, int EPI, int NT, int MT = 2>
__global__ __launch_bounds__(WAVES * 64) __attribute__((amdgpu_waves_per_eu(2, (NT == 4 && MT == 2) ? 2 : 4)))
void direct_gemm_kernel(DirectArgs a) {
    direct_gemm_body<WAVES, MODE, EPI, NT, MT>(a, blockIdx.x, blockIdx.y);
}

template <int WAVES, int MODE, int EPI>
__global__ __launch_bounds__(WAVES * 64) __attribute__((amdgpu_waves_per_eu(2, 2)))
void direct_gemm_tail_kernel(DirectArgs a) {
    const int tile = blockIdx.x;
    const int seg = (a.start1 > 0 && (long)tile * 128 >= a.start1) ? 1 : 0;
    const int t0 = seg ? (int)(a.start1 / 128) : 0;
    const int cap = a.start1 > 0 ? (seg ? (int)((a.P - a.start1) / 128) : (int)(a.start1 / 128)) : a.P / 128;
    const int T = a.meta[4 * seg] / 128;
    const TailPlan pl = tail_plan(T, a.tail_slots, cap);
    const int tl = tile - t0;
    if (tl < pl.full) { direct_gemm_body<WAVES, MODE, EPI, 4, 2>(a, tile, blockIdx.y); return; }
    const int u = tl - pl.full;
    if (u >= pl.R * pl.f) return;
    const int j = u / pl.f, blk = u - j * pl.f;
    const int tt = t0 + pl.full + j;
    const long row = blk == 0 ? (long)tt : a.extra_row0 + (long)seg * a.tail_slots + (long)j * (pl.f - 1) + (blk - 1);
    if (pl.f == 4) direct_gemm_body<WAVES, MODE, EPI, 1, 2>(a, tt * 4 + blk, blockIdx.y, row);
    else           direct_gemm_body<WAVES, MODE, EPI, 2, 2>(a, tt * 2 + blk, blockIdx.y, row);
}

template <int WAVES, int MODE, int EPI, int NT, int MT>
__global__ __launch_bounds__(WAVES * 64) __attribute__((amdgpu_waves_per_eu(2, NT == 4 ? 2 : 4)))
void direct_gemm_pair_kernel(DirectArgs a0, DirectArgs a1) {
    if (blockIdx.z == 0) {
        if ((int)blockIdx.y * WAVES * 32 * MT < a0.M) direct_gemm_body<WAVES, MODE, EPI, NT, MT>(a0, blockIdx.x, blockIdx.y);
    } else {
        if ((int)blockIdx.y * WAVES * 32 * MT < a1.M) direct_gemm_body<WAVES, MODE, EPI, NT, MT>(a1, blockIdx.x, blockIdx.y);
    }
}

constexpr int SK_ROWS = 32, SK_COLS = 64;

__device__ __forceinline__ float reduce_scatter8(float (&x)[8], int l31) {
#pragma unroll
    for (int m = 4; m >= 1; m >>= 1) {
        const bool up = (l31 & m) != 0;
#pragma unroll
        for (int v = 0; v < m; ++v) {
            float lo = x[v], hi = x[v + m];
            asm volatile("" : "+v"(lo), "+v"(hi));
            const float keep = up ? hi : lo;
            const float send = up ? lo : hi;
            x[v] = keep + __shfl_xor(send, m, 64);
        }
    }
    float r = x[0];
    r += __shfl_xor(r, 8, 64);
    r += __shfl_xor(r, 16, 64);
    return r;
}

template <int MODE, int EPI>
__device__ __forceinline__ void splitk_body(DirectArgs& a, const int bx, const int by, float* __restrict__ red) {
    static_assert(MODE <= B_DY && EPI <= 2, "split-K tile: plain / transformed / BatchNorm-backward operands only");
    constexpr int NT = 2;
    const int lane = threadIdx.x & 63, wave = threadIdx.x >> 6;
    const int l31 = lane & 31, h = lane >> 5;
    const int tiles_per_b = a.P / SK_COLS;
    const int tile = bx;
    const int b = tile / tiles_per_b, p0 = (tile - b * tiles_per_b) * SK_COLS;
    if (a.meta) {
        const long c0 = (long)tile * SK_COLS;
        const int seg = (a.start1 > 0 && c0 >= a.start1) ? 1 : 0;
        if (c0 - (seg ? a.start1 : 0) >= a.meta[4 * seg]) return;
        if (seg) {
            if (a.c1) a.c1 += a.K;
            if (a.c2) a.c2 += a.K;
            if (a.c3) a.c3 += a.K;
            if (a.stat_c) a.stat_c += a.M;
            if (a.scale_p) { a.scale_p += a.M; a.shift_p += a.M; a.mean_p += a.M; }
        }
    }
    const int m0 = by * SK_ROWS;
    const int p = p0 + NT * l31;
    float wv[NT] = {1.f, 1.f};
    if (a.w) ldv<NT>(wv, a.w + (long)b * a.P + p);
    const long rowP = a.P;
    const float* xb = a.X + (long)b * a.K * rowP + p;
    const float* yb = (MODE >= B_DY) ? a.Y + (long)b * a.K * rowP + p : nullptr;
    const float* wa = a.A + (long)(m0 + l31) * a.K + 4 * h;

    const int mrow = m0 + 8 * wave + 4 * h;
    const long ob = ((long)b * a.M + mrow) * rowP + p;
    float ex[4][NT];
    float4 k1 = make_float4(0.f, 0.f, 0.f, 0.f), k2 = k1, k3 = k1;
    if constexpr (EPI == 1 || EPI == 2) {
        const float* src = EPI == 1 ? a.Yprev : a.resid;
#pragma unroll
        for (int j = 0; j < 4; ++j) {
            ex[j][0] = ex[j][1] = 0.f;
            if (EPI == 1 || src) ldv<NT>(ex[j], src + ob + (long)j * rowP);
        }
    }
    if constexpr (EPI == 1) {
        k1 = *reinterpret_cast<const float4*>(a.scale_p + mrow);
        k2 = *reinterpret_cast<const float4*>(a.shift_p + mrow);
        k3 = *reinterpret_cast<const float4*>(a.mean_p + mrow);
    } else if constexpr (EPI == 2) {
        if (a.bias) k1 = *reinterpret_cast<const float4*>(a.bias + mrow);
    } else {
        if (a.stat_c) k1 = *reinterpret_cast<const float4*>(a.stat_c + mrow);
    }

    f32x16 acc[1][NT];
#pragma unroll
    for (int t = 0; t < NT; ++t)
#pragma unroll
        for (int r = 0; r < 16; ++r) acc[0][t][r] = 0.f;

    const int npair = a.K / 16;
    const int q = npair / 4, rem = npair - 4 * q;
    const int ps = wave * q + (wave < rem ? wave : rem);
    const int gs = 2 * ps, ge = 2 * (ps + q + (wave < rem ? 1 : 0));
    RawB<NT> f[2];
    float4 wa0[2];
    auto load = [&](auto stc, int g) {
        constexpr int st = decltype(stc)::value;
        load_b<MODE, NT>(a, xb, yb, rowP, 8 * g + 4 * h, 0, 1, f[st]);
        wa0[st] = *reinterpret_cast<const float4*>(wa + 8 * g);
    };
    if (gs < ge) {
        load(std::integral_constant<int, 0>{}, gs);
        for (int g = gs; g < ge; g += 2) {
            load(std::integral_constant<int, 1>{}, g + 1);
            __builtin_amdgcn_sched_barrier(0);
            compute_group<MODE, NT, 1>(f[0], wa0[0], wa0[0], 0, wv, acc);
            __builtin_amdgcn_sched_barrier(0);
            load(std::integral_constant<int, 0>{}, g + 2 < ge ? g + 2 : ge - 1);
            __builtin_amdgcn_sched_barrier(0);
            compute_group<MODE, NT, 1>(f[1], wa0[1], wa0[1], 0, wv, acc);
            __builtin_amdgcn_sched_barrier(0);
        }
    }

#pragma unroll
    for (int r = 0; r < 16; ++r)
        *reinterpret_cast<float2*>(red + ((wave * SK_ROWS + acc_row(r, h)) * SK_COLS + NT * l31)) =
            make_float2(acc[0][0][r], acc[0][1][r]);
    __syncthreads();
    float x8[8];
    const bool stats = EPI != 2 && a.part != nullptr;
#pragma unroll
    for (int j = 0; j < 4; ++j) {
        const int row = 8 * wave + 4 * h + j;
        float v[NT] = {0.f, 0.f};
#pragma unroll
        for (int w4 = 0; w4 < 4; ++w4) {
            const float2 t = *reinterpret_cast<const float2*>(red + ((w4 * SK_ROWS + row) * SK_COLS + NT * l31));
            v[0] += t.x; v[1] += t.y;
        }
        const float c1 = j == 0 ? k1.x : j == 1 ? k1.y : j == 2 ? k1.z : k1.w;
        const float c2 = j == 0 ? k2.x : j == 1 ? k2.y : j == 2 ? k2.z : k2.w;
        const float c3 = j == 0 ? k3.x : j == 1 ? k3.y : j == 2 ? k3.z : k3.w;
        float s1 = 0.f, s2 = 0.f;
        if constexpr (EPI == 1) {
#pragma unroll
            for (int t = 0; t < NT; ++t) {
                v[t] = fmaf(ex[j][t], c1, c2) > 0.f ? v[t] : 0.f;
                s1 += v[t];
                s2 = fmaf(v[t], ex[j][t] - c3, s2);
            }
        } else if constexpr (EPI == 2) {
#pragma unroll
            for (int t = 0; t < NT; ++t) v[t] = (v[t] + c1) + ex[j][t];
        } else {
#pragma unroll
            for (int t = 0; t < NT; ++t) {
                s1 = fmaf(wv[t], v[t], s1);
                s2 += wv[t] * (v[t] - c1) * (v[t] - c1);
            }
        }
        stv<NT>(a.Out + ob + (long)j * rowP, v);
        x8[j] = s1;
        x8[4 + j] = s2;
    }
    if (stats) {
        const float r = reduce_scatter8(x8, l31);
        if (l31 < 8) a.part[(long)tile * 2 * a.M + (long)(l31 >> 2) * a.M + mrow + (l31 & 3)] = r;
    }
}

template <int MODE, int EPI>
__global__ __launch_bounds__(256) __attribute__((amdgpu_waves_per_eu(3, 4)))
void splitk_gemm_kernel(DirectArgs a) {
    __shared__ float red[4 * SK_ROWS * SK_COLS];
    splitk_body<MODE, EPI>(a, blockIdx.x, blockIdx.y, red);
}

template <int MODE, int EPI>
__global__ __launch_bounds__(256) __attribute__((amdgpu_waves_per_eu(3, 4)))
void splitk_gemm_pair_kernel(DirectArgs a0, DirectArgs a1) {
    __shared__ float red[4 * SK_ROWS * SK_COLS];
    if (blockIdx.z == 0) {
        if ((int)blockIdx.y * SK_ROWS < a0.M) splitk_body<MODE, EPI>(a0, blockIdx.x, blockIdx.y, red);
    } else {
        if ((int)blockIdx.y * SK_ROWS < a1.M) splitk_body<MODE, EPI>(a1, blockIdx.x, blockIdx.y, red);
    }
}

static long splitk_max() { return 16L << 20; }
static bool splitk_ok(const DirectArgs& a, int tile) {
    return tile == 64 && a.K % 16 == 0 && a.K >= 64 && a.M % SK_ROWS == 0 && a.P % SK_COLS == 0 && !a.pk &&
           (long)a.M * a.B * a.P <= splitk_max();
}
template <int MODE, int EPI>
int launch_splitk(const DirectArgs& a, hipStream_t st) {
    if constexpr (MODE <= B_DY && EPI <= 2) {
        hipLaunchKernelGGL((splitk_gemm_kernel<MODE, EPI>), dim3(a.B * (a.P / SK_COLS), a.M / SK_ROWS), dim3(256), 0, st, a);
        return o3d_launch_status();
    } else {
        return O3D_EINVAL;
    }
}

template <int MODE, int EPI, int NT, int MT = 2>
int launch_direct_nt(const DirectArgs& a, hipStream_t st) {
    const int tiles = a.B * (a.P / (32 * NT));
    const int slabs = a.M / (32 * MT);
    if constexpr (NT == 4 && MT == 2 && MODE != B_DYPOOL && EPI <= 1) {
        if (a.tail_slots > 0 && a.meta && a.B == 1) {
            if (slabs % 4 == 0)      hipLaunchKernelGGL((direct_gemm_tail_kernel<4, MODE, EPI>), dim3(tiles, slabs / 4), dim3(256), 0, st, a);
            else if (slabs % 2 == 0) hipLaunchKernelGGL((direct_gemm_tail_kernel<2, MODE, EPI>), dim3(tiles, slabs / 2), dim3(128), 0, st, a);
            else                     hipLaunchKernelGGL((direct_gemm_tail_kernel<1, MODE, EPI>), dim3(tiles, slabs), dim3(64), 0, st, a);
            return o3d_launch_status();
        }
    }
    if (slabs % 4 == 0) {
        hipLaunchKernelGGL((direct_gemm_kernel<4, MODE, EPI, NT, MT>), dim3(tiles, slabs / 4), dim3(256), 0, st, a);
    } else if (slabs % 2 == 0) {
        hipLaunchKernelGGL((direct_gemm_kernel<2, MODE, EPI, NT, MT>), dim3(tiles, slabs / 2), dim3(128), 0, st, a);
    } else {
        hipLaunchKernelGGL((direct_gemm_kernel<1, MODE, EPI, NT, MT>), dim3(tiles, slabs), dim3(64), 0, st, a);
    }
    return o3d_launch_status();
}

static int pw_tile(long P, int M) { return o3d_direct_tile(P, M, 0); }

static bool narrow_ok(const DirectArgs& a, int tile) { return tile == 128 && a.M <= 128 && !a.pk; }

static int small_class(const DirectArgs& a, int tile) {
    if (splitk_ok(a, tile)) return 4;
    return tile == 64 ? 2 : 3;
}

template <int MODE, int EPI>
int launch_direct_small(const DirectArgs& a, int tile, hipStream_t st) {
    if constexpr (MODE <= B_DY && EPI <= 2) {
        if (splitk_ok(a, tile)) return launch_splitk<MODE, EPI>(a, st);
    }
    if constexpr (MODE != B_DYPOOL) {
        if (narrow_ok(a, tile)) return launch_direct_nt<MODE, EPI, 4, 1>(a, st);
    }
    return tile == 64 ? launch_direct_nt<MODE, EPI, 2>(a, st) : launch_direct_nt<MODE, EPI, 4>(a, st);
}

template <int MODE, int EPI>
int launch_direct(const DirectArgs& a, int tile, hipStream_t st) {
    if constexpr (MODE <= B_DY && EPI <= 2) {
        if (splitk_ok(a, tile)) return launch_splitk<MODE, EPI>(a, st);
    }
    return tile == 64 ? launch_direct_nt<MODE, EPI, 2>(a, st) : launch_direct_nt<MODE, EPI, 4>(a, st);
}

}

bool o3d_direct_ok(int M, int K, int P) { return M % DT_M == 0 && K % 16 == 0 && P % 128 == 0; }

static int g_tail_override = -1;
extern "C" int o3d_direct_tail_override(int slots) { g_tail_override = slots; return O3D_OK; }

extern "C" int o3d_direct_tail_slots(int M) {
    if (g_tail_override >= 0) return (M > 0 && M % DT_M == 0) ? g_tail_override : 0;
    static int cus_of[64] = {};
    int dev = 0;
    if (hipGetDevice(&dev) != hipSuccess || dev < 0 || dev >= 64) dev = 0;
    if (cus_of[dev] == 0) {
        int n = 0;
        if (hipDeviceGetAttribute(&n, hipDeviceAttributeMultiprocessorCount, dev) != hipSuccess || n <= 0) n = 256;
        cus_of[dev] = n;
    }
    const int cus = cus_of[dev];
    if (M <= 0 || M % DT_M != 0) return 0;
    const int slabs = M / DT_M;
    const int waves = slabs % 4 == 0 ? 4 : (slabs % 2 == 0 ? 2 : 1);
    const int per_tile = slabs / waves;
    const int slots = (8 / waves) * cus / per_tile;
    return slots >= 64 ? slots : 0;
}

extern "C" int o3d_direct_tile(long P, int M, int compact) {
    (void)M; (void)compact;
    return P <= 65536L ? 64 : 128;
}

extern "C" int o3d_direct_class(long ldp, int M, int K, int tile) {
    if (ldp <= 0 || ldp > 0x7fffffff || M <= 0 || K <= 0 || !o3d_direct_ok(M, K, (int)ldp) || (tile != 64 && tile != 128)) return -1;
    DirectArgs a = {};
    a.M = M; a.K = K; a.P = (int)ldp; a.B = 1;
    return small_class(a, tile);
}

int o3d_direct_fwd(const float* X, const float* W, const float* in_scale, const float* in_shift, int B, int Cin,
                   int Cout, int P, float* Y, float* part, const float* stat_c, const float* w, const int32_t* meta,
                   long start1, int tile, hipStream_t st) {
    DirectArgs a = {};
    a.w = w; a.meta = meta; a.start1 = start1;
    a.A = W; a.X = X; a.c1 = in_scale; a.c2 = in_shift; a.Out = Y; a.M = Cout; a.K = Cin; a.P = P; a.B = B;
    a.part = part; a.stat_c = stat_c; a.ns = 4;
    if (meta && tile == 128 && B == 1 && in_scale) { a.tail_slots = o3d_direct_tail_slots(Cout); a.extra_row0 = P / 128; }
    return in_scale ? launch_direct<B_XFORM, 0>(a, tile, st) : launch_direct<B_PLAIN, 0>(a, tile, st);
}

int o3d_direct_dgrad(const float* dN, const float* pk, int ns,
                     const float* Y, const float* A1, const float* A2, const float* A3, const float* Wt, int B,
                     int Cin, int Cout, int P, const float* Yprev, const float* scale_p, const float* shift_p,
                     const float* mean_p, float* dNprev, float* part, const float* w, const int32_t* meta,
                     long start1, int tile, hipStream_t st) {
    DirectArgs a = {};
    a.w = w; a.meta = meta; a.start1 = start1;
    a.A = Wt; a.X = dN; a.Y = Y; a.c1 = A1; a.c2 = A2; a.c3 = A3; a.pk = reinterpret_cast<const float2*>(pk); a.ns = ns;
    a.Out = dNprev; a.M = Cin; a.K = Cout; a.P = P; a.B = B; a.part = part;
    a.Yprev = Yprev; a.scale_p = scale_p; a.shift_p = shift_p; a.mean_p = mean_p;
    if (meta && tile == 128 && B == 1 && dN) { a.tail_slots = o3d_direct_tail_slots(Cin); a.extra_row0 = P / 128; }
    return dN ? launch_direct<B_DY, 1>(a, tile, st) : launch_direct<B_DYPOOL, 1>(a, tile, st);
}


extern "C" int o3d_pw_tile(long P, int M) { return pw_tile(P, M); }

extern "C" int o3d_pw_class(long P, int M, int K) {
    if (P <= 0 || P > 0x7fffffff || P % 64 != 0 || M <= 0 || M % DT_M != 0 || K <= 0 || K % 16 != 0) return -1;
    const int tile = pw_tile(P, M);
    if (tile == 128 && P % 128 != 0) return -1;
    DirectArgs a = {};
    a.M = M; a.K = K; a.P = (int)P; a.B = 1;
    const int cls = small_class(a, tile);
    return cls == 3 && narrow_ok(a, tile) ? 5 : cls;
}

extern "C" int o3d_pw_fwd(const float* X, const float* W, const float* in_scale, const float* in_shift,
                          const float* bias, const float* resid, int Cin, int Cout, long P, float* Y, float* part,
                          const float* stat_c, void* stream) {
    if (!X || !W || !Y || P <= 0 || P > 0x7fffffff || P % 64 != 0 || Cin <= 0 || Cin % 16 != 0 || Cout <= 0 ||
        Cout % DT_M != 0 || (in_scale == nullptr) != (in_shift == nullptr) || (part && (bias || resid)))
        return O3D_EINVAL;
    const int tile = pw_tile(P, Cout);
    if (tile == 128 && P % 128 != 0) return O3D_EINVAL;
    DirectArgs a = {};
    a.A = W; a.X = X; a.c1 = in_scale; a.c2 = in_shift; a.Out = Y; a.M = Cout; a.K = Cin; a.P = (int)P; a.B = 1;
    a.part = part; a.stat_c = stat_c; a.ns = 4; a.bias = bias; a.resid = resid;
    hipStream_t st = reinterpret_cast<hipStream_t>(stream);
    if (part || (!bias && !resid))
        return in_scale ? launch_direct_small<B_XFORM, 0>(a, tile, st) : launch_direct_small<B_PLAIN, 0>(a, tile, st);
    return in_scale ? launch_direct_small<B_XFORM, 2>(a, tile, st) : launch_direct_small<B_PLAIN, 2>(a, tile, st);
}

extern "C" int o3d_pw_dgrad(const float* dN, const float* Y, const float* A1, const float* A2, const float* A3,
                            const float* Wt, int Cin, int Cout, long P, const float* Yprev, const float* scale_p,
                            const float* shift_p, const float* mean_p, const float* resid, float* dNprev, float* part,
                            void* stream) {
    if (!dN || !Wt || !dNprev || P <= 0 || P > 0x7fffffff || P % 64 != 0 || Cin <= 0 || Cin % DT_M != 0 ||
        Cout <= 0 || Cout % 16 != 0 || (Y && (!A1 || !A2 || !A3)) ||
        (Yprev && (!scale_p || !shift_p || !mean_p || !part || resid)) || (!Yprev && part))
        return O3D_EINVAL;
    const int tile = pw_tile(P, Cin);
    if (tile == 128 && P % 128 != 0) return O3D_EINVAL;
    DirectArgs a = {};
    a.A = Wt; a.X = dN; a.Y = Y; a.c1 = A1; a.c2 = A2; a.c3 = A3; a.ns = 4;
    a.Out = dNprev; a.M = Cin; a.K = Cout; a.P = (int)P; a.B = 1; a.part = part;
    a.Yprev = Yprev; a.scale_p = scale_p; a.shift_p = shift_p; a.mean_p = mean_p; a.resid = resid;
    hipStream_t st = reinterpret_cast<hipStream_t>(stream);
    if (Yprev) return Y ? launch_direct_small<B_DY, 1>(a, tile, st) : launch_direct_small<B_PLAIN, 1>(a, tile, st);
    return Y ? launch_direct_small<B_DY, 2>(a, tile, st) : launch_direct_small<B_PLAIN, 2>(a, tile, st);
}

namespace {
template <int MODE, int EPI, int NT, int MT>
int launch_pair_nt(const DirectArgs& a, const DirectArgs& b, hipStream_t st) {
    const int tiles = a.P / (32 * NT);
    const int sa = a.M / (32 * MT), sb = b.M / (32 * MT);
    const int smax = sa > sb ? sa : sb;
    if (sa % 4 == 0 && sb % 4 == 0)
        hipLaunchKernelGGL((direct_gemm_pair_kernel<4, MODE, EPI, NT, MT>), dim3(tiles, smax / 4, 2), dim3(256), 0, st, a, b);
    else if (sa % 2 == 0 && sb % 2 == 0)
        hipLaunchKernelGGL((direct_gemm_pair_kernel<2, MODE, EPI, NT, MT>), dim3(tiles, smax / 2, 2), dim3(128), 0, st, a, b);
    else
        hipLaunchKernelGGL((direct_gemm_pair_kernel<1, MODE, EPI, NT, MT>), dim3(tiles, smax, 2), dim3(64), 0, st, a, b);
    return o3d_launch_status();
}

template <int MODE, int EPI>
int launch_pair(const DirectArgs& a, const DirectArgs& b, int cls, hipStream_t st) {
    if (cls == 4) {
        const int sa = a.M / SK_ROWS, sb = b.M / SK_ROWS;
        hipLaunchKernelGGL((splitk_gemm_pair_kernel<MODE, EPI>), dim3(a.P / SK_COLS, sa > sb ? sa : sb, 2), dim3(256), 0, st, a, b);
        return o3d_launch_status();
    }
    return cls == 2 ? launch_pair_nt<MODE, EPI, 2, 2>(a, b, st) : launch_pair_nt<MODE, EPI, 4, 2>(a, b, st);
}

static bool pw_fwd_args_ok(const o3d_pw_fwd_args& q) {
    return q.X && q.W && q.Y && q.P > 0 && q.P <= 0x7fffffff && q.P % 64 == 0 && q.Cin > 0 && q.Cin % 16 == 0 && q.Cout > 0 &&
           q.Cout % DT_M == 0 && (q.in_scale == nullptr) == (q.in_shift == nullptr) && !(q.part && (q.bias || q.resid));
}
static DirectArgs pw_fwd_direct(const o3d_pw_fwd_args& q) {
    DirectArgs a = {};
    a.A = q.W; a.X = q.X; a.c1 = q.in_scale; a.c2 = q.in_shift; a.Out = q.Y; a.M = q.Cout; a.K = q.Cin; a.P = (int)q.P; a.B = 1;
    a.part = q.part; a.stat_c = q.stat_c; a.ns = 4; a.bias = q.bias; a.resid = q.resid;
    return a;
}
static bool pw_dgrad_args_ok(const o3d_pw_dgrad_args& q) {
    return q.dN && q.Wt && q.dNprev && q.P > 0 && q.P <= 0x7fffffff && q.P % 64 == 0 && q.Cin > 0 && q.Cin % DT_M == 0 &&
           q.Cout > 0 && q.Cout % 16 == 0 && !(q.Y && (!q.A1 || !q.A2 || !q.A3)) &&
           !(q.Yprev && (!q.scale_p || !q.shift_p || !q.mean_p || !q.part || q.resid)) && !(!q.Yprev && q.part);
}
static DirectArgs pw_dgrad_direct(const o3d_pw_dgrad_args& q) {
    DirectArgs a = {};
    a.A = q.Wt; a.X = q.dN; a.Y = q.Y; a.c1 = q.A1; a.c2 = q.A2; a.c3 = q.A3; a.ns = 4;
    a.Out = q.dNprev; a.M = q.Cin; a.K = q.Cout; a.P = (int)q.P; a.B = 1; a.part = q.part;
    a.Yprev = q.Yprev; a.scale_p = q.scale_p; a.shift_p = q.shift_p; a.mean_p = q.mean_p; a.resid = q.resid;
    return a;
}
}

extern "C" int o3d_pw_fwd_pair(const o3d_pw_fwd_args* pa, const o3d_pw_fwd_args* pb, void* stream) {
    if (!pa || !pb || !pw_fwd_args_ok(*pa) || !pw_fwd_args_ok(*pb)) return O3D_EINVAL;
    const o3d_pw_fwd_args &x = *pa, &y = *pb;
    const int ta = pw_tile(x.P, x.Cout), tb = pw_tile(y.P, y.Cout);
    if ((ta == 128 && x.P % 128) || (tb == 128 && y.P % 128)) return O3D_EINVAL;
    DirectArgs a = pw_fwd_direct(x), b = pw_fwd_direct(y);
    const bool epi2a = !(x.part || (!x.bias && !x.resid)), epi2b = !(y.part || (!y.bias && !y.resid));
    const int ca = small_class(a, ta), cb = small_class(b, tb);
    hipStream_t st = reinterpret_cast<hipStream_t>(stream);
    if (x.P != y.P || ta != tb || ca != cb || epi2a != epi2b || (x.in_scale == nullptr) != (y.in_scale == nullptr)) {
        const int rc = o3d_pw_fwd(x.X, x.W, x.in_scale, x.in_shift, x.bias, x.resid, x.Cin, x.Cout, x.P, x.Y, x.part, x.stat_c, stream);
        if (rc != O3D_OK) return rc;
        return o3d_pw_fwd(y.X, y.W, y.in_scale, y.in_shift, y.bias, y.resid, y.Cin, y.Cout, y.P, y.Y, y.part, y.stat_c, stream);
    }
    if (!epi2a) return x.in_scale ? launch_pair<B_XFORM, 0>(a, b, ca, st) : launch_pair<B_PLAIN, 0>(a, b, ca, st);
    return x.in_scale ? launch_pair<B_XFORM, 2>(a, b, ca, st) : launch_pair<B_PLAIN, 2>(a, b, ca, st);
}

extern "C" int o3d_pw_dgrad_pair(const o3d_pw_dgrad_args* pa, const o3d_pw_dgrad_args* pb, void* stream) {
    if (!pa || !pb || !pw_dgrad_args_ok(*pa) || !pw_dgrad_args_ok(*pb)) return O3D_EINVAL;
    const o3d_pw_dgrad_args &x = *pa, &y = *pb;
    const int ta = pw_tile(x.P, x.Cin), tb = pw_tile(y.P, y.Cin);
    if ((ta == 128 && x.P % 128) || (tb == 128 && y.P % 128)) return O3D_EINVAL;
    DirectArgs a = pw_dgrad_direct(x), b = pw_dgrad_direct(y);
    const int ca = small_class(a, ta), cb = small_class(b, tb);
    hipStream_t st = reinterpret_cast<hipStream_t>(stream);
    if (x.P != y.P || ta != tb || ca != cb || (x.Yprev == nullptr) != (y.Yprev == nullptr) || (x.Y == nullptr) != (y.Y == nullptr)) {
        const int rc = o3d_pw_dgrad(x.dN, x.Y, x.A1, x.A2, x.A3, x.Wt, x.Cin, x.Cout, x.P, x.Yprev, x.scale_p, x.shift_p, x.mean_p,
                                    x.resid, x.dNprev, x.part, stream);
        if (rc != O3D_OK) return rc;
        return o3d_pw_dgrad(y.dN, y.Y, y.A1, y.A2, y.A3, y.Wt, y.Cin, y.Cout, y.P, y.Yprev, y.scale_p, y.shift_p, y.mean_p, y.resid,
                            y.dNprev, y.part, stream);
    }
    if (x.Yprev) return x.Y ? launch_pair<B_DY, 1>(a, b, ca, st) : launch_pair<B_PLAIN, 1>(a, b, ca, st);
    return x.Y ? launch_pair<B_DY, 2>(a, b, ca, st) : launch_pair<B_PLAIN, 2>(a, b, ca, st);
}

extern "C" int o3d_pw_fwd_cloud(const float* X, const float* W, const float* cbias, int B, int N, int Cin, int Cout,
                                float* Y, float* part, const float* stat_c, void* stream) {
// ... 10 lines not shown
```

open3dsot_amd/csrc/mlp_wgrad.hip:

```cpp
#include "mlp_common.hpp"

namespace {

struct Wgrad2Args {
    const float* dN;
    const float2* pk;
    int ns;
    const float* Y;
    const float* A1; const float* A2; const float* A3;
    const float* X;
    const float* in_scale; const float* in_shift;
    int B, Cin, Cout, P;
    int chunks_per_block, total_chunks, nslices;
    float* part;
    const float* w;
    const int32_t* meta;
    long start1;
};

template <int TM, int TN, int POOLED>
__device__ __forceinline__ void wgrad2_body(const Wgrad2Args& a, const int bid, float* smem) {
    constexpr int WM = TM / 64, WN = TN / 64, WK = 4 / (WM * WN);
    constexpr int CP = (TM + TN == 128) ? 64 : 32;
    constexpr int LD = CP + 4;
    constexpr int F = CP / 4;
    constexpr int RPP = 256 / F;
    constexpr int PA = TM / RPP, PB = TN / RPP;
    constexpr int NG = CP / WK / 8;
    auto As = [&](int buf) -> float* { return smem + buf * ((TM + TN) * LD); };
    auto Bs = [&](int buf) -> float* { return smem + buf * ((TM + TN) * LD) + TM * LD; };

    const int tid = threadIdx.x, lane = tid & 63, wave = tid >> 6;
    const int l31 = lane & 31, h = lane >> 5;
    const int wk = wave / (WM * WN), wmn = wave - wk * (WM * WN);
    const int wm0 = (wmn / WN) * 64, wn0 = (wmn % WN) * 64;
    const int tiles_ci = a.Cin / TN, ntile = tiles_ci * (a.Cout / TM);
    int tile_id, slice;
    if ((a.nslices & 7) == 0) {
        const int xcd = bid & 7, local = bid >> 3;
        tile_id = local % ntile;
        slice = (local / ntile) * 8 + xcd;
    } else {
        tile_id = bid % ntile;
        slice = bid / ntile;
    }
    const int ci0 = (tile_id % tiles_ci) * TN, co0 = (tile_id / tiles_ci) * TM;
    int c_begin, c_end;
    int seg = 0;
    long col0 = 0;
    if (a.meta) {
        const int n0 = a.meta[0] / CP, n1 = a.start1 > 0 ? a.meta[4] / CP : 0;
        int nsl0 = a.nslices;
        if (n1 > 0) {
            nsl0 = (int)(((long)a.nslices * n0 + (n0 + n1) / 2) / (n0 + n1));
            nsl0 = nsl0 < 1 ? 1 : (nsl0 > a.nslices - 1 ? a.nslices - 1 : nsl0);
        }
        seg = slice >= nsl0 ? 1 : 0;
        const int nsl = seg ? a.nslices - nsl0 : nsl0, ls = seg ? slice - nsl0 : slice, n = seg ? n1 : n0;
        const int per = (n + nsl - 1) / nsl;
        c_begin = ls * per;
        c_end = c_begin + per < n ? c_begin + per : n;
        col0 = seg ? a.start1 : 0;
    } else {
        c_begin = slice * a.chunks_per_block;
        c_end = c_begin + a.chunks_per_block < a.total_chunks ? c_begin + a.chunks_per_block : a.total_chunks;
    }
    const float* A1 = a.A1 + (seg ? a.Cout : 0);
    const float* A2 = a.A2 + (seg ? a.Cout : 0);
    const float* A3 = a.A3 + (seg ? a.Cout : 0);
    const bool plain_x = a.in_scale == nullptr;
    const float* in_scale = plain_x ? nullptr : a.in_scale + (seg ? a.Cin : 0);
    const float* in_shift = plain_x ? nullptr : a.in_shift + (seg ? a.Cin : 0);
    const float x_floor = plain_x ? -INFINITY : 0.f;
    const int chunks_per_b = a.P / CP;
    const int r0 = tid / F, c4 = tid % F;
    const int np = POOLED == 1 ? a.P / a.ns : 1;

    float ka1[PA], ka2[PA], ka3[PA], ksc[PB], ksh[PB];
#pragma unroll
    for (int i = 0; i < PA; ++i) {
        const int co = co0 + r0 + RPP * i;
        ka1[i] = A1[co]; ka2[i] = A2[co]; ka3[i] = A3[co];
    }
#pragma unroll
    for (int i = 0; i < PB; ++i) {
        const int ci = ci0 + r0 + RPP * i;
        ksc[i] = plain_x ? 1.f : in_scale[ci]; ksh[i] = plain_x ? 0.f : in_shift[ci];
    }

    float4 rg[PA], ry[PA], rx[PB];
    float4 rw = make_float4(1.f, 1.f, 1.f, 1.f);
    int rk = 0;
    auto load_chunk = [&](int chl) {
        const long chg = col0 / CP + chl;
        const long b = chg / chunks_per_b;
        const int p = (int)(chg - b * chunks_per_b) * CP + 4 * c4;
        if (a.w) rw = *reinterpret_cast<const float4*>(&a.w[b * a.P + p]);
#pragma unroll
        for (int i = 0; i < PA; ++i) {
            const long row = b * a.Cout + co0 + r0 + RPP * i;
            ry[i] = *reinterpret_cast<const float4*>(&a.Y[row * a.P + p]);
            if (POOLED) {
                const int j = p / a.ns;
                const float2 t = a.pk[row * np + j];
                rg[i].x = t.x; rg[i].y = t.y;
                rk = p - j * a.ns;
            } else {
                rg[i] = *reinterpret_cast<const float4*>(&a.dN[row * a.P + p]);
            }
        }
#pragma unroll
        for (int i = 0; i < PB; ++i)
            rx[i] = *reinterpret_cast<const float4*>(&a.X[(b * a.Cin + ci0 + r0 + RPP * i) * a.P + p]);
    };
    auto store_chunk = [&](int buf) {
#pragma unroll
        for (int i = 0; i < PA; ++i) {
            float4 g;
            if (POOLED) {
                const int ak = __float_as_int(rg[i].y);
                const float go = rg[i].x;
                g.x = (rk + 0 == ak) ? go : 0.f; g.y = (rk + 1 == ak) ? go : 0.f;
                g.z = (rk + 2 == ak) ? go : 0.f; g.w = (rk + 3 == ak) ? go : 0.f;
            } else {
                g = rg[i];
            }
            float4 o;
            o.x = fmaf(ka1[i], g.x, rw.x * fmaf(ka2[i], ry[i].x, ka3[i])); o.y = fmaf(ka1[i], g.y, rw.y * fmaf(ka2[i], ry[i].y, ka3[i]));
            o.z = fmaf(ka1[i], g.z, rw.z * fmaf(ka2[i], ry[i].z, ka3[i])); o.w = fmaf(ka1[i], g.w, rw.w * fmaf(ka2[i], ry[i].w, ka3[i]));
            *reinterpret_cast<float4*>(&As(buf)[(r0 + RPP * i) * LD + 4 * c4]) = o;
        }
#pragma unroll
        for (int i = 0; i < PB; ++i) {
            float4 v = rx[i];
            v.x = fmaxf(fmaf(v.x, ksc[i], ksh[i]), x_floor); v.y = fmaxf(fmaf(v.y, ksc[i], ksh[i]), x_floor);
            v.z = fmaxf(fmaf(v.z, ksc[i], ksh[i]), x_floor); v.w = fmaxf(fmaf(v.w, ksc[i], ksh[i]), x_floor);
            *reinterpret_cast<float4*>(&Bs(buf)[(r0 + RPP * i) * LD + 4 * c4]) = v;
        }
    };

    f32x16 acc[2][2];
#pragma unroll
    for (int i = 0; i < 2; ++i)
#pragma unroll
        for (int j = 0; j < 2; ++j)
#pragma unroll
            for (int r = 0; r < 16; ++r) acc[i][j][r] = 0.f;

    if (c_begin < c_end) {
        load_chunk(c_begin);
        store_chunk(0);
        __syncthreads();
        for (int ch = c_begin; ch < c_end; ++ch) {
            const int t = ch - c_begin;
            if (ch + 1 < c_end) load_chunk(ch + 1);
            const float* A_ = As(t & 1) + wk * (CP / WK);
            const float* B_ = Bs(t & 1) + wk * (CP / WK);
#pragma unroll
            for (int g = 0; g < NG; ++g) {
                float av[2][4], bv[2][4];
#pragma unroll
                for (int u = 0; u < 2; ++u) {
                    const float4 x = *reinterpret_cast<const float4*>(&A_[(wm0 + 32 * u + l31) * LD + 8 * g + 4 * h]);
                    av[u][0] = x.x; av[u][1] = x.y; av[u][2] = x.z; av[u][3] = x.w;
                    const float4 y = *reinterpret_cast<const float4*>(&B_[(wn0 + 32 * u + l31) * LD + 8 * g + 4 * h]);
                    bv[u][0] = y.x; bv[u][1] = y.y; bv[u][2] = y.z; bv[u][3] = y.w;
                }
#pragma unroll
                for (int s = 0; s < 4; ++s)
#pragma unroll
                    for (int tm = 0; tm < 2; ++tm)
#pragma unroll
                        for (int tn = 0; tn < 2; ++tn) acc[tm][tn] = mfma32(av[tm][s], bv[tn][s], acc[tm][tn]);
            }
            if (ch + 1 < c_end) store_chunk((t + 1) & 1);
            __syncthreads();
        }
    }
    float* dst = a.part + (long)(slice * WK + wk) * a.Cout * a.Cin;
#pragma unroll
    for (int tm = 0; tm < 2; ++tm)
#pragma unroll
        for (int r = 0; r < 16; ++r) {
            const int co = co0 + wm0 + 32 * tm + acc_row(r, h);
#pragma unroll
            for (int tn = 0; tn < 2; ++tn) dst[(long)co * a.Cin + ci0 + wn0 + 32 * tn + l31] = acc[tm][tn][r];
        }
}

template <int TM, int TN, int POOLED>
__global__ __launch_bounds__(256) void wgrad2_kernel(Wgrad2Args a) {
    extern __shared__ __attribute__((aligned(16))) float smem[];
    wgrad2_body<TM, TN, POOLED>(a, blockIdx.x, smem);
}

constexpr int WG_MAXJOBS = 8;
struct Wgrad2Group {
    Wgrad2Args job[WG_MAXJOBS];
    int first[WG_MAXJOBS + 1];
    int kind[WG_MAXJOBS];
    int njobs;
};

__device__ __forceinline__ void row_sum_body(const Wgrad2Args& a, const int bid, float* smem) {
    const float* g = a.dN + (long)bid * a.P;
    float s = 0.f;
    for (long p = 4L * threadIdx.x; p < a.P; p += 1024) {
        const float4 v = *reinterpret_cast<const float4*>(g + p);
        s += (v.x + v.y) + (v.z + v.w);
    }
#pragma unroll
    for (int off = 32; off >= 1; off >>= 1) s += __shfl_xor(s, off, 64);
    if ((threadIdx.x & 63) == 0) smem[threadIdx.x >> 6] = s;
    __syncthreads();
    if (threadIdx.x == 0) a.part[bid] = (smem[0] + smem[1]) + (smem[2] + smem[3]);
}

__global__ __launch_bounds__(256) void wgrad2_group_kernel(Wgrad2Group g) {
    extern __shared__ __attribute__((aligned(16))) float smem[];
    int j = 0;
    while (j + 1 < g.njobs && (int)blockIdx.x >= g.first[j + 1]) ++j;
    const int bid = blockIdx.x - g.first[j];
    switch (g.kind[j]) {
        case 0: wgrad2_body<128, 128, 0>(g.job[j], bid, smem); break;
        case 1: wgrad2_body<128, 64, 0>(g.job[j], bid, smem); break;
        case 2: wgrad2_body<64, 128, 0>(g.job[j], bid, smem); break;
        case 3: wgrad2_body<64, 64, 0>(g.job[j], bid, smem); break;
        default: row_sum_body(g.job[j], bid, smem); break;
    }
}

struct ReduceGroup {
    const float* part[WG_MAXJOBS]; float* out[WG_MAXJOBS];
    long n[WG_MAXJOBS]; int nslices[WG_MAXJOBS]; int first[WG_MAXJOBS + 1]; int njobs;
    int ld[WG_MAXJOBS], orows[WG_MAXJOBS], ocols[WG_MAXJOBS];
};

__global__ __launch_bounds__(256) void wgrad_reduce_group_kernel(ReduceGroup r) {
    __shared__ float sh[8][32];
    int j = 0;
    while (j + 1 < r.njobs && (int)blockIdx.x >= r.first[j + 1]) ++j;
    const float* __restrict__ part = r.part[j];
    const long n = r.n[j];
    const int nslices = r.nslices[j];
    const int col = threadIdx.x & 31, grp = threadIdx.x >> 5;
    const long i = (long)(blockIdx.x - r.first[j]) * 32 + col;
    const int per = (nslices + 7) / 8, z0 = grp * per;
    int z1 = z0 + per;
    if (z1 > nslices) z1 = nslices;
    float s0 = 0.f, s1 = 0.f, s2 = 0.f, s3 = 0.f;
    if (i < n) {
        int z = z0;
        for (; z + 3 < z1; z += 4) {
            s0 += part[(long)z * n + i]; s1 += part[(long)(z + 1) * n + i];
            s2 += part[(long)(z + 2) * n + i]; s3 += part[(long)(z + 3) * n + i];
        }
        for (; z < z1; ++z) s0 += part[(long)z * n + i];
    }
    sh[grp][col] = (s0 + s1) + (s2 + s3);
    __syncthreads();
    if (grp == 0 && i < n) {
        float t = 0.f;
#pragma unroll
        for (int g = 0; g < 8; ++g) t += sh[g][col];
        const int ld = r.ld[j];
        const long row = i / ld;
        const int cc = (int)(i - row * ld);
        if (row < r.orows[j] && cc < r.ocols[j]) r.out[j][row * r.ocols[j] + cc] = t;
    }
}

template <int TM, int TN>
int launch_wgrad2(const Wgrad2Args& a, hipStream_t s) {
    constexpr int CP = (TM + TN == 128) ? 64 : 32;
    const size_t lds = sizeof(float) * 2 * (TM + TN) * (CP + 4);
    const void* fn = a.dN ? reinterpret_cast<const void*>(wgrad2_kernel<TM, TN, 0>)
                          : reinterpret_cast<const void*>(wgrad2_kernel<TM, TN, 1>);
    if (lds > 48 * 1024 &&
        hipFuncSetAttribute(fn, hipFuncAttributeMaxDynamicSharedMemorySize, (int)lds) != hipSuccess)
        return O3D_ELAUNCH;
    const int ntile = (a.Cout / TM) * (a.Cin / TN);
    if (a.dN) hipLaunchKernelGGL((wgrad2_kernel<TM, TN, 0>), dim3(ntile * a.nslices), dim3(256), lds, s, a);
    else      hipLaunchKernelGGL((wgrad2_kernel<TM, TN, 1>), dim3(ntile * a.nslices), dim3(256), lds, s, a);
    return o3d_launch_status();
}

struct FusedBwdArgs {
    const float* dN; const float* Y;
    const float* A1; const float* A2; const float* A3;
    const float* X;
    const float* in_scale; const float* in_shift; const float* in_mean;
    const float* Wt;
    int Cin, Cout, P;
    int chunks_per_block, total_chunks, nslices;
    const float* w; const int32_t* meta; long start1;
    float* part_w;
    float* part_s;
    float* dX;
};

template <int TM>
__global__ __launch_bounds__(256) void fused_bwd_kernel(FusedBwdArgs a) {
    constexpr int TN = 64;
    constexpr int WM = TM / 64, WK = 4 / WM;
    constexpr int CP = (TM + TN == 128) ? 64 : 32;
    constexpr int NPT = CP / 32;
    constexpr int LD = CP + 4;
    constexpr int F = CP / 4, RPP = 256 / F, PA = TM / RPP, PB = TN / RPP;
    constexpr int NG = CP / WK / 8;
    constexpr int GD = TM / 8;
    extern __shared__ __attribute__((aligned(16))) float smem[];
    auto As = [&](int buf) -> float* { return smem + buf * ((TM + TN) * LD); };
    auto Bs = [&](int buf) -> float* { return smem + buf * ((TM + TN) * LD) + TM * LD; };

    const int tid = threadIdx.x, lane = tid & 63, wave = tid >> 6;
    const int l31 = lane & 31, h = lane >> 5;
    const int wk = wave / WM, wm0 = (wave % WM) * 64;
    const int dci = (wave & 1) * 32, dpt = wave >> 1;
    const bool dactive = dpt < NPT;
    const int slice = blockIdx.x;
    int c_begin, c_end, seg = 0;
    long col0 = 0;
    if (a.meta) {
        const int n0 = a.meta[0] / CP, n1 = a.start1 > 0 ? a.meta[4] / CP : 0;
        int nsl0 = a.nslices;
        if (n1 > 0) {
            nsl0 = (int)(((long)a.nslices * n0 + (n0 + n1) / 2) / (n0 + n1));
            nsl0 = nsl0 < 1 ? 1 : (nsl0 > a.nslices - 1 ? a.nslices - 1 : nsl0);
        }
        seg = slice >= nsl0 ? 1 : 0;
        const int nsl = seg ? a.nslices - nsl0 : nsl0, ls = seg ? slice - nsl0 : slice, n = seg ? n1 : n0;
        const int per = (n + nsl - 1) / nsl;
        c_begin = ls * per;
        c_end = c_begin + per < n ? c_begin + per : n;
        col0 = seg ? a.start1 : 0;
    } else {
        c_begin = slice * a.chunks_per_block;
        c_end = c_begin + a.chunks_per_block < a.total_chunks ? c_begin + a.chunks_per_block : a.total_chunks;
    }
    const float* A1 = a.A1 + (seg ? a.Cout : 0);
    const float* A2 = a.A2 + (seg ? a.Cout : 0);
    const float* A3 = a.A3 + (seg ? a.Cout : 0);
    const float* in_scale = a.in_scale + (seg ? a.Cin : 0);
    const float* in_shift = a.in_shift + (seg ? a.Cin : 0);
    const float* in_mean = a.in_mean + (seg ? a.Cin : 0);
    const int r0 = tid / F, c4 = tid % F;

    float ka1[PA], ka2[PA], ka3[PA], ksc[PB], ksh[PB];
#pragma unroll
    for (int i = 0; i < PA; ++i) { const int co = r0 + RPP * i; ka1[i] = A1[co]; ka2[i] = A2[co]; ka3[i] = A3[co]; }
#pragma unroll
    for (int i = 0; i < PB; ++i) { const int ci = r0 + RPP * i; ksc[i] = in_scale[ci]; ksh[i] = in_shift[ci]; }

    float4 wt[GD];
#pragma unroll
    for (int g = 0; g < GD; ++g) wt[g] = *reinterpret_cast<const float4*>(a.Wt + (long)(dci + l31) * TM + 8 * g + 4 * h);

    float4 rg[PA], ry[PA], rx[PB];
    float4 rw = make_float4(1.f, 1.f, 1.f, 1.f);
    auto load_chunk = [&](int chl) {
        const long p = (col0 / CP + chl) * CP + 4 * c4;
        if (a.w) rw = *reinterpret_cast<const float4*>(&a.w[p]);
#pragma unroll
        for (int i = 0; i < PA; ++i) {
            const long row = r0 + RPP * i;
            ry[i] = *reinterpret_cast<const float4*>(&a.Y[row * a.P + p]);
            rg[i] = *reinterpret_cast<const float4*>(&a.dN[row * a.P + p]);
        }
#pragma unroll
        for (int i = 0; i < PB; ++i) rx[i] = *reinterpret_cast<const float4*>(&a.X[(long)(r0 + RPP * i) * a.P + p]);
    };
    auto store_chunk = [&](int buf) {
#pragma unroll
        for (int i = 0; i < PA; ++i) {
            float4 o;
            o.x = fmaf(ka1[i], rg[i].x, rw.x * fmaf(ka2[i], ry[i].x, ka3[i]));
            o.y = fmaf(ka1[i], rg[i].y, rw.y * fmaf(ka2[i], ry[i].y, ka3[i]));
            o.z = fmaf(ka1[i], rg[i].z, rw.z * fmaf(ka2[i], ry[i].z, ka3[i]));
            o.w = fmaf(ka1[i], rg[i].w, rw.w * fmaf(ka2[i], ry[i].w, ka3[i]));
            *reinterpret_cast<float4*>(&As(buf)[(r0 + RPP * i) * LD + 4 * c4]) = o;
        }
#pragma unroll
        for (int i = 0; i < PB; ++i) {
            float4 v = rx[i];
            v.x = fmaxf(fmaf(v.x, ksc[i], ksh[i]), 0.f); v.y = fmaxf(fmaf(v.y, ksc[i], ksh[i]), 0.f);
            v.z = fmaxf(fmaf(v.z, ksc[i], ksh[i]), 0.f); v.w = fmaxf(fmaf(v.w, ksc[i], ksh[i]), 0.f);
            *reinterpret_cast<float4*>(&Bs(buf)[(r0 + RPP * i) * LD + 4 * c4]) = v;
        }
    };

    f32x16 acc[2][2];
#pragma unroll
    for (int i = 0; i < 2; ++i)
#pragma unroll
        for (int j = 0; j < 2; ++j)
#pragma unroll
            for (int r = 0; r < 16; ++r) acc[i][j][r] = 0.f;

    float sacc[32];
#pragma unroll
    for (int r = 0; r < 32; ++r) sacc[r] = 0.f;

    if (c_begin < c_end) {
        load_chunk(c_begin);
        store_chunk(0);
        __syncthreads();
        for (int ch = c_begin; ch < c_end; ++ch) {
            const int t = ch - c_begin;
            if (ch + 1 < c_end) load_chunk(ch + 1);
            const float* A_ = As(t & 1);
            const float* B_ = Bs(t & 1);
            {
                const float* Aw = A_ + wk * (CP / WK);
                const float* Bw = B_ + wk * (CP / WK);
#pragma unroll
                for (int g = 0; g < NG; ++g) {
                    float av[2][4], bv[2][4];
#pragma unroll
                    for (int u = 0; u < 2; ++u) {
                        const float4 x = *reinterpret_cast<const float4*>(&Aw[(wm0 + 32 * u + l31) * LD + 8 * g + 4 * h]);
                        av[u][0] = x.x; av[u][1] = x.y; av[u][2] = x.z; av[u][3] = x.w;
                        const float4 y = *reinterpret_cast<const float4*>(&Bw[(32 * u + l31) * LD + 8 * g + 4 * h]);
                        bv[u][0] = y.x; bv[u][1] = y.y; bv[u][2] = y.z; bv[u][3] = y.w;
                    }
#pragma unroll
                    for (int s = 0; s < 4; ++s)
#pragma unroll
                        for (int tm = 0; tm < 2; ++tm)
#pragma unroll
                            for (int tn = 0; tn < 2; ++tn) acc[tm][tn] = mfma32(av[tm][s], bv[tn][s], acc[tm][tn]);
                }
            }
            if (dactive) {
                f32x16 d;
#pragma unroll
                for (int r = 0; r < 16; ++r) d[r] = 0.f;
                const float* Bd = A_ + 32 * dpt + l31;
#pragma unroll
                for (int g = 0; g < GD; ++g) {
                    const float b0 = Bd[(8 * g + 4 * h + 0) * LD], b1 = Bd[(8 * g + 4 * h + 1) * LD];
                    const float b2 = Bd[(8 * g + 4 * h + 2) * LD], b3 = Bd[(8 * g + 4 * h + 3) * LD];
                    d = mfma32(wt[g].x, b0, d);
                    d = mfma32(wt[g].y, b1, d);
                    d = mfma32(wt[g].z, b2, d);
                    d = mfma32(wt[g].w, b3, d);
                }
                const long q = (col0 / CP + ch) * CP + 32 * dpt + l31;
#pragma unroll
                for (int r = 0; r < 16; ++r) {
                    const int row = acc_row(r, h);
                    const float xt = B_[(dci + row) * LD + 32 * dpt + l31];
                    const float gq = xt > 0.f ? d[r] : 0.f;
                    a.dX[(long)(dci + row) * a.P + q] = gq;
                    sacc[r] += gq;
                    sacc[16 + r] = fmaf(gq, xt, sacc[16 + r]);
                }
            }
            if (ch + 1 < c_end) store_chunk((t + 1) & 1);
            __syncthreads();
        }
    }
    float* dst = a.part_w + (long)(slice * WK + wk) * TM * TN;
#pragma unroll
    for (int tm = 0; tm < 2; ++tm)
#pragma unroll
        for (int r = 0; r < 16; ++r) {
            const int co = wm0 + 32 * tm + acc_row(r, h);
#pragma unroll
            for (int tn = 0; tn < 2; ++tn) dst[(long)co * TN + 32 * tn + l31] = acc[tm][tn][r];
        }
    if (dactive) {
        reduce_scatter32(sacc, l31);
        const int ci = dci + acc_row(l31 & 15, h);
        const int which = l31 >> 4;
        const float other = __shfl_xor(sacc[0], 16, 64);
        const float s1 = which ? other : sacc[0], s2x = which ? sacc[0] : other;
        const float sc = in_scale[ci], beta = fmaf(sc, in_mean[ci], in_shift[ci]);
        float s2 = sc != 0.f ? (s2x - beta * s1) / sc : 0.f;
        if (sc == 0.f && which) {
            asm volatile("s_waitcnt vmcnt(0)" ::: "memory");
            const float mu = in_mean[ci];
            float t2 = 0.f;
            for (int ch = c_begin; ch < c_end; ++ch) {
                const long qb = (col0 / CP + ch) * CP + 32 * dpt;
                for (int j = 0; j < 32; ++j)
                    t2 = fmaf(a.dX[(long)ci * a.P + qb + j], a.X[(long)ci * a.P + qb + j] - mu, t2);
            }
            s2 = t2;
        }
        const long rows = (long)a.nslices * NPT, row = (long)slice * NPT + dpt;
        float* mine = a.part_s + ((long)seg * rows + row) * 2 * TN;
        float* theirs = a.part_s + ((long)(1 - seg) * rows + row) * 2 * TN;
        mine[which * TN + ci] = which ? s2 : s1;
        theirs[which * TN + ci] = 0.f;
    }
}

template <int TM>
int launch_fused_bwd(const FusedBwdArgs& a, hipStream_t s) {
    constexpr int CP = (TM + 64 == 128) ? 64 : 32;
    const size_t lds = sizeof(float) * 2 * (TM + 64) * (CP + 4);
    const void* fn = reinterpret_cast<const void*>(fused_bwd_kernel<TM>);
    if (lds > 48 * 1024 && hipFuncSetAttribute(fn, hipFuncAttributeMaxDynamicSharedMemorySize, (int)lds) != hipSuccess)
        return -3;
    hipLaunchKernelGGL((fused_bwd_kernel<TM>), dim3(a.nslices), dim3(256), lds, s, a);
    return hipGetLastError() == hipSuccess ? 0 : -3;
}

}

void o3d_wgrad_reduce(const float* part, int nslices, long n, float* dW, hipStream_t s);

static void wgrad2_plan(int Cin, int Cout, int B, int P, int& TM, int& TN, int& WK, int& CP, int& nsl) {
    TM = Cout % 128 == 0 ? 128 : 64;
    TN = Cin % 128 == 0 ? 128 : 64;
    WK = 4 / ((TM / 64) * (TN / 64));
    CP = (TM + TN == 128) ? 64 : 32;
    const int ntile = (Cout / TM) * (Cin / TN);
    const long total = (long)B * (P / CP);
    constexpr int wgs = 512;
    nsl = wgs / ntile;
    if (nsl < 8) nsl = 8;
    while (nsl > 8 && total / nsl < 4) nsl -= 8;
    if (nsl > total) nsl = (int)total;
}

extern "C" long o3d_mlp_conv_wgrad2_scratch(int B, int Cin, int Cout, int P) {
    if (Cin <= 0 || Cout <= 0 || Cin % 64 || Cout % 64 || P <= 0 || P % 64 || B <= 0) return -1;
    int TM, TN, WK, CP, nsl;
    wgrad2_plan(Cin, Cout, B, P, TM, TN, WK, CP, nsl);
    return ((long)nsl * WK + 16) * Cout * Cin;
}

static int wgrad2_impl(const float* dN, const float* pk, int ns, const float* Y, const float* A1, const float* A2,
                       const float* A3, const float* X, const float* in_scale, const float* in_shift, int B, int Cin,
                       int Cout, int P, const float* w, const int32_t* meta, long start1, float* scratch, float* dW,
                       void* stream) {
    if (B <= 0 || Cin <= 0 || Cout <= 0 || Cin % 64 || Cout % 64 || P <= 0 || P % 64 || !Y || !A1 || !A2 || !A3 ||
        !X || (in_scale == nullptr) != (in_shift == nullptr) || !scratch || !dW || (!dN && (!pk || ns < 4 || ns % 4)))
        return O3D_EINVAL;
    int TM, TN, WK, CP, nsl;
    wgrad2_plan(Cin, Cout, B, P, TM, TN, WK, CP, nsl);
    Wgrad2Args a = {};
    a.dN = dN; a.pk = reinterpret_cast<const float2*>(pk); a.ns = ns > 0 ? ns : 4; a.Y = Y;
    a.A1 = A1; a.A2 = A2; a.A3 = A3; a.X = X; a.in_scale = in_scale; a.in_shift = in_shift;
    a.B = B; a.Cin = Cin; a.Cout = Cout; a.P = P;
    a.total_chunks = B * (P / CP);
    a.chunks_per_block = (a.total_chunks + nsl - 1) / nsl;
    a.nslices = nsl;
    a.part = scratch;
    a.w = w; a.meta = meta; a.start1 = start1;
    hipStream_t s = o3d_stream(stream);
    int rc;
    if (TM == 128 && TN == 128) rc = launch_wgrad2<128, 128>(a, s);
    else if (TM == 128)         rc = launch_wgrad2<128, 64>(a, s);
    else if (TN == 128)         rc = launch_wgrad2<64, 128>(a, s);
    else                        rc = launch_wgrad2<64, 64>(a, s);
    if (rc != O3D_OK) return rc;
    const long n = (long)Cout * Cin;
    o3d_wgrad_reduce(scratch, nsl * WK, n, dW, s);
    return o3d_launch_status();
}

extern "C" int o3d_mlp_conv_wgrad2(const float* dN, const float* pk, int ns, const float* Y, const float* A1,
                                   const float* A2, const float* A3, const float* X, const float* in_scale,
                                   const float* in_shift, int B, int Cin, int Cout, int P, float* scratch,
                                   float* dW, void* stream) {
    return wgrad2_impl(dN, pk, ns, Y, A1, A2, A3, X, in_scale, in_shift, B, Cin, Cout, P, nullptr, nullptr, 0, scratch,
                       dW, stream);
}

extern "C" int o3d_mlp_conv_wgrad2_c(const float* dN, const float* Y, const float* A1, const float* A2,
                                     const float* A3, const float* X, const float* in_scale, const float* in_shift,
                                     int Cin, int Cout, long ldp, const float* w, const int32_t* meta, long start1,
                                     float* scratch, float* dW, void* stream) {
    if (!dN || !w || !meta || ldp <= 0 || ldp > 0x7fffffff || start1 < 0 || start1 % 256 != 0) return O3D_EINVAL;
    return wgrad2_impl(dN, nullptr, 4, Y, A1, A2, A3, X, in_scale, in_shift, 1, Cin, Cout, (int)ldp, w, meta, start1,
                       scratch, dW, stream);
}


extern "C" int o3d_mlp_conv_wgrad2_group(const o3d_wgrad_job* jobs, int njobs, void* stream) {
    if (!jobs || njobs < 1 || njobs > WG_MAXJOBS) return O3D_EINVAL;
    Wgrad2Group g = {};
    ReduceGroup r = {};
    g.njobs = r.njobs = njobs;
    size_t lds = 0;
    int nblk = 0, rblk = 0;
    for (int i = 0; i < njobs; ++i) {
        const o3d_wgrad_job& q = jobs[i];
        if (q.dN && !q.X && !q.Y && q.dW && q.Cout > 0 && q.P > 0 && q.P % 4 == 0 && q.P <= 0x7fffffff) {
            Wgrad2Args& a = g.job[i];
            a.dN = q.dN; a.P = (int)q.P; a.Cout = q.Cout; a.part = q.dW;
            g.kind[i] = 4;
            g.first[i] = nblk;
            nblk += q.Cout;
            r.part[i] = q.dW; r.out[i] = q.dW; r.n[i] = 0; r.nslices[i] = 0; r.ld[i] = 1; r.orows[i] = r.ocols[i] = 0;
            r.first[i] = rblk;
            continue;
        }
        if (!q.dN || !q.Y || !q.A1 || !q.A2 || !q.A3 || !q.X || (q.in_scale == nullptr) != (q.in_shift == nullptr) ||
            !q.scratch || !q.dW || q.Cin <= 0 || q.Cout <= 0 || q.Cin % 64 || q.Cout % 64 || q.P <= 0 || q.P % 64 ||
            q.P > 0x7fffffff)
            return O3D_EINVAL;
        int TM, TN, WK, CP, nsl;
        wgrad2_plan(q.Cin, q.Cout, 1, (int)q.P, TM, TN, WK, CP, nsl);
        Wgrad2Args& a = g.job[i];
        a.dN = q.dN; a.ns = 4; a.Y = q.Y; a.A1 = q.A1; a.A2 = q.A2; a.A3 = q.A3; a.X = q.X;
        a.in_scale = q.in_scale; a.in_shift = q.in_shift; a.B = 1; a.Cin = q.Cin; a.Cout = q.Cout; a.P = (int)q.P;
        a.total_chunks = (int)(q.P / CP);
        a.chunks_per_block = (a.total_chunks + nsl - 1) / nsl;
        a.nslices = nsl;
        a.part = q.scratch;
        g.kind[i] = TM == 128 ? (TN == 128 ? 0 : 1) : (TN == 128 ? 2 : 3);
        g.first[i] = nblk;
        nblk += (q.Cout / TM) * (q.Cin / TN) * nsl;
        const size_t l = sizeof(float) * 2 * (TM + TN) * (CP + 4);
        lds = l > lds ? l : lds;
        if (q.out_rows < 0 || q.out_rows > q.Cout || q.out_cols < 0 || q.out_cols > q.Cin) return O3D_EINVAL;
        r.part[i] = q.scratch; r.out[i] = q.dW; r.n[i] = (long)q.Cout * q.Cin; r.nslices[i] = nsl * WK;
        r.ld[i] = q.Cin; r.orows[i] = q.out_rows > 0 ? q.out_rows : q.Cout; r.ocols[i] = q.out_cols > 0 ? q.out_cols : q.Cin;
        r.first[i] = rblk;
        rblk += o3d_cdiv(r.n[i], 32);
    }
    g.first[njobs] = nblk;
    r.first[njobs] = rblk;
    static const bool attr_ok = hipFuncSetAttribute(reinterpret_cast<const void*>(wgrad2_group_kernel),
                                                    hipFuncAttributeMaxDynamicSharedMemorySize, 80 * 1024) == hipSuccess;
    if (!attr_ok || lds > 80 * 1024) return O3D_ELAUNCH;
    hipStream_t s = o3d_stream(stream);
    if (lds < 16) lds = 16;
    hipLaunchKernelGGL(wgrad2_group_kernel, dim3(nblk), dim3(256), lds, s, g);
    if (rblk > 0) hipLaunchKernelGGL(wgrad_reduce_group_kernel, dim3(rblk), dim3(256), 0, s, r);
    return o3d_launch_status();
}


static int fused_bwd_slices(int Cout, long P) {
    constexpr int wgs = 256;
    const int CP = (Cout + 64 == 128) ? 64 : 32;
    const long total = P / CP;
    int nsl = wgs;
    while (nsl > 8 && total / nsl < 4) nsl -= 8;
    if (nsl > total) nsl = (int)total;
    return nsl < 1 ? 1 : nsl;
}
static bool fused_bwd_ok(int Cin, int Cout, long P) {
    return Cin == 64 && (Cout == 64 || Cout == 128) && P > 0 && P % 64 == 0 && P <= 0x7fffffff;
}

extern "C" int o3d_mlp_conv_bwd_fused_rows(int Cin, int Cout, long P) {
    return fused_bwd_ok(Cin, Cout, P) ? fused_bwd_slices(Cout, P) * (Cout == 64 ? 2 : 1) : -1;
}
extern "C" long o3d_mlp_conv_bwd_fused_scratch(int Cin, int Cout, long P) {
    return fused_bwd_ok(Cin, Cout, P) ? (long)fused_bwd_slices(Cout, P) * (4 / (Cout / 64)) * Cout * Cin : -1;
}

extern "C" int o3d_mlp_conv_bwd_fused_c(const float* dN, const float* Y, const float* A1, const float* A2, const float* A3,
                                        const float* X, const float* in_scale, const float* in_shift, const float* in_mean,
                                        const float* Wt, int Cin, int Cout, long ldp, const float* w, const int32_t* meta,
                                        long start1, float* scratch, float* dW, float* part_s, float* dNprev, void* stream) {
    if (!dN || !Y || !A1 || !A2 || !A3 || !X || !in_scale || !in_shift || !in_mean || !Wt || !scratch || !dW || !part_s ||
        !dNprev || !fused_bwd_ok(Cin, Cout, ldp) || (meta != nullptr) != (w != nullptr) || start1 < 0 || start1 % 256 != 0)
        return O3D_EINVAL;
    const int CP = (Cout + 64 == 128) ? 64 : 32;
    const int nsl = fused_bwd_slices(Cout, ldp);
    FusedBwdArgs a = {};
    a.dN = dN; a.Y = Y; a.A1 = A1; a.A2 = A2; a.A3 = A3; a.X = X; a.in_scale = in_scale; a.in_shift = in_shift;
    a.in_mean = in_mean; a.Wt = Wt; a.Cin = Cin; a.Cout = Cout; a.P = (int)ldp;
    a.total_chunks = (int)(ldp / CP);
    a.chunks_per_block = (a.total_chunks + nsl - 1) / nsl;
    a.nslices = nsl;
    a.w = w; a.meta = meta; a.start1 = start1; a.part_w = scratch; a.part_s = part_s; a.dX = dNprev;
    hipStream_t s = o3d_stream(stream);
    const int rc = Cout == 64 ? launch_fused_bwd<64>(a, s) : launch_fused_bwd<128>(a, s);
    if (rc != 0) return O3D_ELAUNCH;
    const long n = (long)Cout * Cin;
    o3d_wgrad_reduce(scratch, nsl * (4 / (Cout / 64)), n, dW, s);
    return o3d_launch_status();
}
```

open3dsot_amd/fused.py:

```python
import ctypes

import torch
from torch import nn
from torch.autograd.graph import increment_version as _increment_version

from . import capi
from .ops import QueryAndGroup

POOL_BWD_SPLIT = capi.CONSTANTS["O3D_POOL_BWD_SPLIT"]
_BnFinArgs = capi.struct("o3d_bn_fin_args")
_BnBwdFinArgs = capi.struct("o3d_bn_bwd_fin_args")

TILE = 128
ETILE = 256

_PROF = {"on": False, "events": []}


def _ptr(t):
    return t.data_ptr() if t is not None else None


def _stream():
    return torch.cuda.current_stream().cuda_stream
# ... 222 lines not shown
                     "frac": round(max(t_mfma, t_hbm) / ms1, 3)})
    return rows


def _layers(mlp):
    out = []
    for layer in mlp.children():
        kids = dict(layer.named_children())
        conv, bnw, act = kids.get("conv"), kids.get("bn"), kids.get("activation")
        if conv is None or bnw is None or not isinstance(act, nn.ReLU) or list(kids)[0] != "conv":
            return None
        bn = getattr(bnw, "bn", None)
        if not isinstance(conv, nn.Conv2d) or not isinstance(bn, nn.BatchNorm2d):
            return None
        if conv.bias is not None or conv.kernel_size != (1, 1) or conv.stride != (1, 1) or conv.groups != 1:
            return None
        if not bn.affine or not bn.track_running_stats or bn.momentum is None:
            return None
        out.append((conv, bn))
    return out or None


def supports_mlp(mlp):
    layers = _layers(mlp)
    return layers is not None and len(layers) >= 2


def supports(grouper, mlp, features):
    return isinstance(grouper, QueryAndGroup) and grouper.use_xyz and supports_mlp(mlp)


def _shape_ok(npoint, ns):
    return 4 <= ns <= 256 and (ns & (ns - 1)) == 0 and (npoint * ns) % ETILE == 0


def _const_vec(dev, n, value):
    key = (str(dev), n, value)
    v = _CONST.get(key)
    if v is None:
        v = _CONST[key] = torch.full((n,), float(value), device=dev, dtype=torch.float32)
    return v


_CONST = {}


class _Cfg:
    __slots__ = ("nxyz", "inv_radius", "training", "bns", "eps", "momentum", "centers", "geo", "geo_dims")


def _direct_tile(lib, pmax, m):
    return lib.o3d_direct_tile(pmax, m, 1)


_TAIL = {"on": True, "applied": -1}


def set_tail_split(slots):
    capi.load().o3d_direct_tail_override(int(slots))
    _TAIL["on"], _TAIL["applied"] = int(slots) != 0, int(slots)


def _tail_rows(lib, tile, rows, nseg, layer):
    if not _TAIL["on"] and _TAIL["applied"] != 0:
        lib.o3d_direct_tail_override(0)
        _TAIL["applied"] = 0
    return nseg * lib.o3d_direct_tail_slots(rows) if (tile == 128 and layer >= 1) else 0


class FusedGroupedMLPCompact(torch.autograd.Function):

    @staticmethod
    @capi.on_tensor_device
    def forward(ctx, cfg, nseg, *args):
        lib = capi.load()
        segs = [args[4 * s:4 * s + 4] for s in range(nseg)]
        params = args[4 * nseg:]
        L = len(params) // 3
        Ws = [params[3 * l].detach().reshape(params[3 * l].shape[0], -1).contiguous() for l in range(L)]
        gammas = [params[3 * l + 1].detach().contiguous() for l in range(L)]
        betas = [params[3 * l + 2].detach().contiguous() for l in range(L)]
        nxyz = cfg.nxyz
        geo = getattr(cfg, "geo", None)
        dev = segs[0][3].device if geo is None else geo["gp"].device
        f32, i32 = torch.float32, torch.int32
        st = _stream()
        if geo is None:
            B, _, ns = segs[0][3].shape
            npoints = [sg[3].shape[1] for sg in segs]
        else:
            B, ns, npoints = cfg.geo_dims[0], cfg.geo_dims[1], list(cfg.geo_dims[2])
        C = segs[0][2].shape[1] if segs[0][2] is not None else 0
        Cin0, C0 = nxyz + C, Ws[0].shape[0]
        Ns = [sg[2].shape[2] if sg[2] is not None else sg[0].shape[1] for sg in segs]
        Npads = [-(-n // TILE) * TILE for n in Ns]
        Pmaxs = [B * npt * ns for npt in npoints]
        starts = [0, Pmaxs[0]][:nseg]
        start1 = starts[1] if nseg == 2 else 0
        ldp = sum(Pmaxs)
        pt_bases = [0, B * Npads[0]][:nseg]
        ldz = sum(B * n for n in Npads)
        nballs_s = [B * npt for npt in npoints]
        ball_bases = [0, nballs_s[0]][:nseg]
        nballs = sum(nballs_s)
        need_bwd = any(ctx.needs_input_grad)
        unit = cfg.inv_radius == 1.0
        if geo is not None:
            ball_cnt, ball_off, gp, cball, cw, meta = (geo[k] for k in ("ball_cnt", "ball_off", "gp", "cball", "cw", "meta"))
            assert nseg == 2 and gp.numel() == ldp and ball_cnt.numel() == nballs and meta.numel() == 8
        else:
            ball_cnt = torch.empty((nballs,), device=dev, dtype=i32)
            ball_off = torch.empty((nballs + 1,), device=dev, dtype=i32)
            gp = torch.empty((ldp,), device=dev, dtype=i32)
            cball = torch.empty((ldp,), device=dev, dtype=i32)
            cw = torch.empty((ldp,), device=dev, dtype=f32)
            meta = torch.empty((nseg, 4), device=dev, dtype=i32)
            if nseg == 2:
                _call("compact_build", 0.0, lib.o3d_compact_build2, segs[0][3].data_ptr(), npoints[0], Npads[0],
                      segs[1][3].data_ptr(), npoints[1], Npads[1], B, ns, starts[1], pt_bases[1], nballs, ball_cnt.data_ptr(),
                      ball_off.data_ptr(), gp.data_ptr(), cball.data_ptr(), cw.data_ptr(), meta.data_ptr(), st)
            else:
                for s_, sg in enumerate(segs):
                    _call("compact_build", 0.0, lib.o3d_compact_build, sg[3].data_ptr(), B, npoints[s_], ns, Npads[s_],
                          starts[s_], pt_bases[s_], ball_bases[s_], nballs, ball_cnt[ball_bases[s_]:].data_ptr(),
                          ball_off[ball_bases[s_]:].data_ptr(), gp.data_ptr(), cball.data_ptr(), cw.data_ptr(),
                          meta[s_].data_ptr(), st)
        padded = any(n != npd for n, npd in zip(Ns, Npads))
        Cin0p = -(-Cin0 // 16) * 16 if Cin0 > 16 else Cin0
        Cin0m = -(-Cin0 // 64) * 64 if Cin0 > 16 else Cin0
        X0n = torch.empty((Cin0m, ldz), device=dev, dtype=f32)
        xs = [sg[0].detach().contiguous() if nxyz else None for sg in segs]
        fs = [sg[2].detach().contiguous() if C else None for sg in segs]
        _call("pack_points", 0.0, lib.o3d_pack_points, _ptr(xs[0]), _ptr(fs[0]), Ns[0], Npads[0],
              _ptr(xs[-1]) if nseg == 2 else None, _ptr(fs[-1]) if nseg == 2 else None, Ns[-1] if nseg == 2 else 0,
              Npads[-1] if nseg == 2 else 0, B, nxyz, C, float(cfg.inv_radius), Cin0m, X0n.data_ptr(), st)
        centers = None
        if nxyz:
            centers = getattr(cfg, "centers", None)
            if centers is None:
                centers = torch.cat([sg[1].detach().reshape(-1, 3) for sg in segs] + [_const_vec(dev, 3, 0.0).view(1, 3)])
            if not unit:
                centers = centers * cfg.inv_radius
        from .fused_heads import prep_for
        prep = prep_for(dev)
        direct3 = C == 0 and nxyz == 3
        Z = None
        if not direct3:
            Z = torch.empty((C0, ldz), device=dev, dtype=f32)
            W0p = prep.get(params[0], C0, Cin0p)
            _call("conv_fwd_points", 2.0 * Cin0p * C0 * ldz, lib.o3d_mlp_conv_fwd, X0n.data_ptr(), W0p.data_ptr(),
                  None, None, 1, Cin0p, C0, ldz, Z.data_ptr(), None, None, st, dims=(Cin0p, C0))
        counts = [float(pm) for pm in Pmaxs]
        Ys, means, invstds, scales, shifts = [], [], [], [], []
        if cfg.training:
            if nseg == 1:
                statcs = [bn.running_mean.detach().unsqueeze(0) for bn in cfg.bns]
            else:
                statcs = [prep.snapshot(bn.running_mean, nseg) for bn in cfg.bns]
        for l in range(L):
            Cout, Cin = Ws[l].shape
            bn = cfg.bns[l]
            tile = ETILE if l == 0 else _direct_tile(lib, ldp, Cout)
            Y = torch.empty((Cout, ldp), device=dev, dtype=f32)
            part = torch.empty((ldp // tile + _tail_rows(lib, tile, Cout, nseg, l), 2, Cout), device=dev, dtype=f32) \
                if cfg.training else None
            statc = statcs[l] if cfg.training else None
            if l == 0 and direct3:
                _call("group_expand", 0.0, lib.o3d_group_expand_c3, X0n.data_ptr(), ldz, gp.data_ptr(), cball.data_ptr(),
                      cw.data_ptr(), centers.data_ptr(), Ws[0].data_ptr(), Cin0, C0, meta.data_ptr(), start1, ldp,
                      Y.data_ptr(), _ptr(part), _ptr(statc), st)
            elif l == 0:
                _call("group_expand", 0.0, lib.o3d_group_expand_c, Z.data_ptr(), ldz, gp.data_ptr(), cball.data_ptr(),
                      cw.data_ptr(), _ptr(centers), Ws[0].data_ptr(), Cin0, C0, meta.data_ptr(), start1, ldp, Y.data_ptr(),
                      _ptr(part), _ptr(statc), st)
            else:
                _call("conv_fwd", (2.0 * Cin * Cout, meta, ldp), lib.o3d_mlp_conv_fwd_c, Ys[-1].data_ptr(), Ws[l].data_ptr(),
                      scales[-1].data_ptr(), shifts[-1].data_ptr(), Cin, Cout, ldp, cw.data_ptr(), meta.data_ptr(), start1,
                      tile, Y.data_ptr(), _ptr(part), _ptr(statc), st, dims=(Cin, Cout))
            vec = torch.empty((4, nseg, Cout), device=dev, dtype=f32)
            if cfg.training:
                bn_finalize(lib, st, part, [pm // tile for pm in Pmaxs], counts, bn, gammas[l], betas[l], vec, statc, meta, tile)
            else:
                _eval_consts(lib, bn, gammas[l], betas[l], vec, nseg, st)
            Ys.append(Y)
            means.append(vec[0]); invstds.append(vec[1]); scales.append(vec[2]); shifts.append(vec[3])
        if cfg.training:
            count_batches(cfg.bns, nseg)
        Cl = Ws[-1].shape[0]
        out = torch.empty((nballs * Cl,), device=dev, dtype=f32)
        argq = torch.empty((nballs * Cl,), device=dev, dtype=i32) if need_bwd else None
        yarg = torch.empty((nballs * Cl,), device=dev, dtype=f32) if need_bwd else None
        np1 = npoints[1] if nseg == 2 else 0
        if Cl % 64 == 0 and ns <= 32 and ldp >= 288:
            _call("pool_fwd", 0.0, lib.o3d_pool_fwd_ct, Ys[-1].data_ptr(), ldp, scales[-1].data_ptr(), shifts[-1].data_ptr(),
                  ball_off.data_ptr(), ball_cnt.data_ptr(), cball.data_ptr(), meta.data_ptr(), start1, B, Cl, npoints[0], np1,
                  ns, out.data_ptr(), _ptr(argq), _ptr(yarg), st)
        else:
            _call("pool_fwd", 0.0, lib.o3d_pool_fwd_c, Ys[-1].data_ptr(), ldp, scales[-1].data_ptr(), shifts[-1].data_ptr(),
                  ball_off.data_ptr(), ball_cnt.data_ptr(), B, Cl, npoints[0], np1, out.data_ptr(), _ptr(argq), _ptr(yarg), st)
        if need_bwd:
            ctx.cfg = cfg
            ctx.versions = _versions(params)
            ctx.Wts = [None] + [prep.get(params[3 * l], Ws[l].shape[1], Ws[l].shape[0], transpose=True) for l in range(1, L)]
            want_in = any(ctx.needs_input_grad[2:2 + 4 * nseg])
            ctx.W0t = prep.get(params[0], -(-Cin0 // 64) * 64, C0, transpose=True) if want_in else None
            ctx.geom = (B, ns, C, nseg, Ns, Npads, npoints, Pmaxs, starts, pt_bases, ball_bases, nballs_s)
            ctx.saved = (X0n, centers, ball_off, ball_cnt, gp, cball, cw, meta, Ws, gammas, Ys, means, invstds, scales,
                         shifts, out.detach(), argq, yarg)
        outs = tuple(out[ball_bases[s_] * Cl:(ball_bases[s_] + nballs_s[s_]) * Cl].view(B, Cl, npoints[s_])
                     for s_ in range(nseg))
        return outs if nseg > 1 else outs[0]

    @staticmethod
    @capi.on_tensor_device
    def backward(ctx, *dOuts):
        lib = capi.load()
        cfg = ctx.cfg
        _check_versions(ctx.versions, "FusedGroupedMLPCompact")
        B, ns, C, nseg, Ns, Npads, npoints, Pmaxs, starts, pt_bases, ball_bases, nballs_s = ctx.geom
        (X0n, centers, ball_off, ball_cnt, gp, cball, cw, meta, Ws, gammas, Ys, means, invstds, scales, shifts, out,
         argq, yarg) = ctx.saved
        L = len(Ws)
        dev = out.device
        st = _stream()
        f32 = torch.float32
        nxyz = cfg.nxyz
        ldp, ldz, nballs = sum(Pmaxs), X0n.shape[1], sum(nballs_s)
        start1 = starts[1] if nseg == 2 else 0
        counts = [float(pm) for pm in Pmaxs]
        grads = [None] * (3 * L)
        needs = ctx.needs_input_grad[2:2 + 4 * nseg]
        want_xyz = nxyz > 0 and any(needs[4 * s_] or needs[4 * s_ + 1] for s_ in range(nseg))
        want_feats = C > 0 and any(needs[4 * s_ + 2] for s_ in range(nseg))
        Cl = Ws[-1].shape[0]
        np1 = npoints[1] if nseg == 2 else 0
        dN = torch.empty((Cl, ldp), device=dev, dtype=f32)
        pool_dense = _POOL_BWD_DENSE["on"] and Cl % 8 == 0 and ldp % POOL_DENSE_COLS == 0 and start1 % POOL_DENSE_COLS == 0
        if pool_dense:
            gsrc = []
            for s_ in range(nseg):
                g = dOuts[s_]
                if g is not None and g.stride(2) != 1:
                    g = g.contiguous()
                gsrc += [_ptr(g), g.stride(0) if g is not None else 0, g.stride(1) if g is not None else 0]
            if nseg == 1:
                gsrc += [None, 0, 0]
            part = torch.empty((ldp // POOL_DENSE_COLS, 2, Cl), device=dev, dtype=f32)
            _call("pool_bwd", 0.0, lib.o3d_pool_bwd_dense, *gsrc, out.data_ptr(), argq.data_ptr(), yarg.data_ptr(),
                  means[-1].data_ptr(), cball.data_ptr(), ball_off.data_ptr(), meta.data_ptr(), start1, ldp, B, Cl, npoints[0],
                  np1, dN.data_ptr(), part.data_ptr(), st)
        else:
            if nseg == 1:
                dOut = dOuts[0].contiguous()
            else:
                dOut = torch.empty((nballs * Cl,), device=dev, dtype=f32)
                for s_ in range(nseg):
                    dst = dOut[ball_bases[s_] * Cl:(ball_bases[s_] + nballs_s[s_]) * Cl].view(B, Cl, npoints[s_])
                    if dOuts[s_] is None:
                        dst.zero_()
                    else:
                        dst.copy_(dOuts[s_])
            part = torch.empty((nseg, POOL_BWD_SPLIT, 2, Cl), device=dev, dtype=f32)
            _call("pool_bwd", 0.0, lib.o3d_pool_bwd_c, dOut.data_ptr(), out.data_ptr(), argq.data_ptr(), yarg.data_ptr(),
                  means[-1].data_ptr(), B, Cl, npoints[0], np1, meta.data_ptr(), start1, ldp, dN.data_ptr(),
                  part.data_ptr(), st)
        dtile = POOL_DENSE_COLS if pool_dense else 0
        part_rows = 0
        seg_grads = [[None, None, None] for _ in range(nseg)]
        for l in range(L - 1, -1, -1):
            Cout, Cin = Ws[l].shape
            if l == L - 1 and not pool_dense:
                rows, live = [POOL_BWD_SPLIT] * nseg, ()
            elif part_rows:
                rows, live = [part_rows] * nseg, ()
            else:
                rows, live = [pm // dtile for pm in Pmaxs], (meta, dtile)
            coef, A = bn_bwd_finalize(lib, st, cfg.training, part, rows, counts, gammas[l], means[l], invstds[l], *live)
            grads[3 * l + 1], grads[3 * l + 2] = coef[0, 0], coef[1, 0]
            if l == 0 and C == 0 and nxyz == 3 and not (want_xyz or want_feats):
                part0 = torch.empty((ldp // 256, Cout, 3), device=dev, dtype=f32)
                dW = torch.empty((Cout, 3), device=dev, dtype=f32)
                _call("group_dw0", 0.0, lib.o3d_group_dw0_xyz, dN.data_ptr(), Ys[0].data_ptr(), ldp, A[0], A[1], A[2],
                      gp.data_ptr(), cball.data_ptr(), cw.data_ptr(), X0n.data_ptr(), ldz, centers.data_ptr(), meta.data_ptr(),
                      start1, Cout, part0.data_ptr(), dW.data_ptr(), st)
                grads[0] = dW
                continue
            if l == 0:
                S = torch.empty((Cout, ldz), device=dev, dtype=f32)
                T = torch.empty((Cout, nballs), device=dev, dtype=f32) if nxyz else None
                spanmax = max(npoints) * ns
                npo = lib.o3d_group_reduce_gather_scratch(B, nseg, npoints[0], Npads[0], npoints[-1], Npads[-1],
                                                          spanmax) if _REDUCE_GATHER["on"] else -1
                if npo >= 0:
                    perm = torch.empty((ldp,), device=dev, dtype=torch.int32)
                    poff = torch.empty((npo,), device=dev, dtype=torch.int32)
                    _call("group_reduce", 0.0, lib.o3d_group_reduce_gather, dN.data_ptr(), Ys[0].data_ptr(), ldp, A[0], A[1],
                          A[2], gp.data_ptr(), cw.data_ptr(), ball_off.data_ptr(), ball_cnt.data_ptr(), B, nseg, npoints[0],
                          Npads[0], npoints[-1], Npads[-1], Cout, spanmax, perm.data_ptr(), poff.data_ptr(), S.data_ptr(),
                          _ptr(T), st)
                else:
                    _call("group_reduce", 0.0, lib.o3d_group_reduce_c, dN.data_ptr(), Ys[0].data_ptr(), ldp, A[0], A[1], A[2],
                          gp.data_ptr(), cball.data_ptr(), cw.data_ptr(), ball_off.data_ptr(), ball_cnt.data_ptr(), B, nseg,
                          npoints[0], Npads[0], npoints[-1], Npads[-1], Cout, S.data_ptr(), _ptr(T), st)
                one, zero = _const_vec(dev, Cout, 1.0), _const_vec(dev, Cout, 0.0)
                Cinm = X0n.shape[0]
                aligned = Cinm % 64 == 0
                if aligned:
                    wpart = torch.empty((lib.o3d_mlp_conv_wgrad2_scratch(1, Cinm, Cout, ldz),), device=dev, dtype=f32)
                    dWm = torch.empty((Cout, Cinm), device=dev, dtype=f32)
                else:
                    tiles = ((Cin + 127) // 128) * ((Cout + 127) // 128)
                    total_chunks = ldz // 32
                    nsl = max(1, min(total_chunks // 4 if total_chunks >= 4 else 1, 768 // tiles))
                    wpart = torch.empty((nsl + 16, Cout, Cin), device=dev, dtype=f32)
                    dWm = torch.empty((Cout, Cin), device=dev, dtype=f32)
                fold = bool(nxyz) and dWm.shape[1] != Cin
                dW = torch.empty((Cout, Cin), device=dev, dtype=f32) if fold else None
                if aligned:
                    _call("conv_wgrad_points", 2.0 * Cinm * Cout * ldz, lib.o3d_mlp_conv_wgrad2, S.data_ptr(), None, 4,
                          S.data_ptr(), one.data_ptr(), zero.data_ptr(), zero.data_ptr(), X0n.data_ptr(), None, None, 1,
                          Cinm, Cout, ldz, wpart.data_ptr(), dWm.data_ptr(), st, dims=(Cinm, Cout, True))
                else:
                    _call("conv_wgrad_points", 2.0 * Cin * Cout * ldz, lib.o3d_mlp_conv_wgrad, S.data_ptr(), None, None,
                          None, 4, S.data_ptr(), one.data_ptr(), zero.data_ptr(), zero.data_ptr(), X0n.data_ptr(), None,
                          None, 1, Cin, Cout, ldz, nsl, wpart.data_ptr(), dWm.data_ptr(), st)
                if fold:
                    _call("center_term", 0.0, lib.o3d_center_term_out, T.data_ptr(), centers.data_ptr(), Cout, nballs,
                          dWm.shape[1], dWm.data_ptr(), Cin, dW.data_ptr(), st)
                else:
                    if nxyz:
                        _call("center_term", 0.0, lib.o3d_center_term, T.data_ptr(), centers.data_ptr(), Cout, nballs,
                              dWm.shape[1], dWm.data_ptr(), st)
                    dW = dWm if dWm.shape[1] == Cin else dWm[:, :Cin].contiguous()
                grads[0] = dW
                if want_xyz or want_feats:
                    Cinm = -(-Cin // 64) * 64
                    W0t = ctx.W0t
                    dX = torch.empty((Cinm, ldz), device=dev, dtype=f32)
                    _call("conv_dgrad_points", 2.0 * Cinm * Cout * ldz, lib.o3d_mlp_conv_fwd, S.data_ptr(), W0t.data_ptr(),
                          None, None, 1, Cout, Cinm, ldz, dX.data_ptr(), None, None, st, dims=(Cout, Cinm))
                    dnew_all = None
                    if want_xyz:
                        dnew_all = torch.empty((3, nballs), device=dev, dtype=f32)
                        _call("center_grad", 0.0, lib.o3d_center_grad, T.data_ptr(), Ws[0].data_ptr(), Ws[0].shape[1], Cout, nballs,
                              -float(cfg.inv_radius), dnew_all.data_ptr(), st)
                    for s_ in range(nseg):
                        view = dX[:Cin, pt_bases[s_]:pt_bases[s_] + B * Npads[s_]].view(Cin, B, Npads[s_])
                        if want_feats:
                            seg_grads[s_][2] = view[nxyz:, :, :Ns[s_]].permute(1, 0, 2)
                        if want_xyz:
                            dxyz = view[:3, :, :Ns[s_]].permute(1, 2, 0)
                            seg_grads[s_][0] = dxyz if cfg.inv_radius == 1.0 else dxyz * cfg.inv_radius
                            seg_grads[s_][1] = dnew_all[:, ball_bases[s_]:ball_bases[s_] + nballs_s[s_]].reshape(
                                3, B, npoints[s_]).permute(1, 2, 0)
                continue
            rows_fb = lib.o3d_mlp_conv_bwd_fused_rows(Cin, Cout, ldp) if Cout <= FUSED_BWD_MAX_COUT else -1
            if rows_fb > 0:
                dW = torch.empty((Cout, Cin), device=dev, dtype=f32)
                wpart = torch.empty((lib.o3d_mlp_conv_bwd_fused_scratch(Cin, Cout, ldp),), device=dev, dtype=f32)
                dNp = torch.empty((Cin, ldp), device=dev, dtype=f32)
                part = torch.empty((2, rows_fb, 2, Cin), device=dev, dtype=f32)
                _call("conv_bwd_fused", (4.0 * Cin * Cout, meta, ldp), lib.o3d_mlp_conv_bwd_fused_c, dN.data_ptr(),
                      Ys[l].data_ptr(), A[0], A[1], A[2], Ys[l - 1].data_ptr(), scales[l - 1].data_ptr(),
                      shifts[l - 1].data_ptr(), means[l - 1].data_ptr(), ctx.Wts[l].data_ptr(), Cin, Cout, ldp, cw.data_ptr(),
                      meta.data_ptr(), start1, wpart.data_ptr(), dW.data_ptr(), part.data_ptr(), dNp.data_ptr(), st,
                      dims=(Cin, Cout))
                grads[3 * l] = dW
                dN, part_rows = dNp, rows_fb
                continue
            part_rows = 0
            flops = (2.0 * Cin * Cout, meta, ldp)
            dW = torch.empty((Cout, Cin), device=dev, dtype=f32)
            wpart = torch.empty((lib.o3d_mlp_conv_wgrad2_scratch(1, Cin, Cout, ldp),), device=dev, dtype=f32)
            _call("conv_wgrad", flops, lib.o3d_mlp_conv_wgrad2_c, dN.data_ptr(), Ys[l].data_ptr(), A[0], A[1], A[2],
                  Ys[l - 1].data_ptr(), scales[l - 1].data_ptr(), shifts[l - 1].data_ptr(), Cin, Cout, ldp, cw.data_ptr(),
                  meta.data_ptr(), start1, wpart.data_ptr(), dW.data_ptr(), st, dims=(Cin, Cout))
            grads[3 * l] = dW
            Wt = ctx.Wts[l]
            dNp = torch.empty((Cin, ldp), device=dev, dtype=f32)
            dtile = _direct_tile(lib, ldp, Cin)
            part = torch.empty((ldp // dtile + _tail_rows(lib, dtile, Cin, nseg, 1), 2, Cin), device=dev, dtype=f32)
            _call("conv_dgrad", flops, lib.o3d_mlp_conv_dgrad_c, dN.data_ptr(), Ys[l].data_ptr(), A[0], A[1], A[2], Wt.data_ptr(),
                  Cin, Cout, ldp, cw.data_ptr(), meta.data_ptr(), start1, dtile, Ys[l - 1].data_ptr(),
                  scales[l - 1].data_ptr(), shifts[l - 1].data_ptr(), means[l - 1].data_ptr(), dNp.data_ptr(),
                  part.data_ptr(), st, dims=(Cin, Cout))
            dN = dNp
        gw = []
        for l in range(L):
            shape = (Ws[l].shape[0], Ws[l].shape[1], 1, 1)
            gw += [grads[3 * l].view(shape), grads[3 * l + 1], grads[3 * l + 2]]
        gin = []
        for s_ in range(nseg):
            gin += [seg_grads[s_][0] if needs[4 * s_] else None, seg_grads[s_][1] if needs[4 * s_ + 1] else None,
                    seg_grads[s_][2] if needs[4 * s_ + 2] else None, None]
        return (None, None, *gin, *gw)


POOL_DENSE_COLS = 512
_POOL_BWD_DENSE = {"on": True}


def set_pool_bwd_dense(enabled):
    _POOL_BWD_DENSE["on"] = bool(enabled)


FUSED_BWD_MAX_COUT = 128
_REDUCE_GATHER = {"on": True}


def set_reduce_gather(enabled):
    _REDUCE_GATHER["on"] = bool(enabled)


def reduce_gather_enabled():
    return _REDUCE_GATHER["on"]


_EVAL_FUSED = {"on": True}


def set_eval_fused(enabled):
    _EVAL_FUSED["on"] = bool(enabled)


def _eval_vec(lib, bn, gamma, beta, st):
    key = (bn.running_mean._version, bn.running_var._version, gamma._version, beta._version, bn.running_mean.data_ptr(),
           gamma.data_ptr(), float(bn.eps))
    hit = getattr(bn, "_o3d_eval_vec", None)
    if hit is not None and hit[0] == key:
        return hit[1]
    vec = torch.empty((4, 1, bn.running_mean.numel()), device=bn.running_mean.device, dtype=torch.float32)
    _eval_consts(lib, bn, gamma.detach(), beta.detach(), vec, 1, st)
    object.__setattr__(bn, "_o3d_eval_vec", (key, vec))
    return vec


def _eval_fused_ok(mlp, layers, segs, nxyz):
    if not _EVAL_FUSED["on"] or mlp.training or layers is None or len(layers) != 3:
        return False
    if torch.is_grad_enabled() and (any(t is not None and t.requires_grad for sg in segs for t in sg[:3]) or
                                    any(p.requires_grad for p in mlp.parameters())):
        return False
    c = [conv.out_channels for conv, _ in layers]
    for sg in segs:
        B, npoint, ns = sg[3].shape
        if ns > 32 or (ns & (ns - 1)) or (B * npoint * ns) % 32:
            return False
    return c[0] % 8 == 0 and c[1] % 32 == 0 and c[2] % 32 == 0


def _run_eval(mlp, layers, segs, nxyz, inv_radius):
    lib = capi.load()
    dev = segs[0][3].device
    f32 = torch.float32
    nseg = len(segs)
    B, _, ns = segs[0][3].shape
    C = segs[0][2].shape[1] if segs[0][2] is not None else 0
    Ws = [conv.weight.detach().reshape(conv.out_channels, -1) for conv, _ in layers]
    Cin0, C0 = nxyz + C, Ws[0].shape[0]
    Ns = [sg[2].shape[2] if sg[2] is not None else sg[0].shape[1] for sg in segs]
    Npads = [-(-n // TILE) * TILE for n in Ns]
    pt_bases = [0, B * Npads[0]][:nseg]
    ldz = sum(B * n for n in Npads)
    Cin0p = -(-Cin0 // 16) * 16 if Cin0 > 16 else Cin0
    with torch.cuda.device(dev):
        st = _stream()
        X0n = torch.empty((Cin0p, ldz), device=dev, dtype=f32)
        xs = [sg[0].detach().contiguous() if nxyz else None for sg in segs]
        fs = [sg[2].detach().contiguous() if C else None for sg in segs]
        _call("pack_points", 0.0, lib.o3d_pack_points, _ptr(xs[0]), _ptr(fs[0]), Ns[0], Npads[0],
              _ptr(xs[-1]) if nseg == 2 else None, _ptr(fs[-1]) if nseg == 2 else None, Ns[-1] if nseg == 2 else 0,
              Npads[-1] if nseg == 2 else 0, B, nxyz, C, float(inv_radius), Cin0p, X0n.data_ptr(), st)
        from .fused_heads import prep_for
        W0p = prep_for(dev).get(layers[0][0].weight, C0, Cin0p)
        Z = torch.empty((C0, ldz), device=dev, dtype=f32)
        _call("conv_fwd_points", 2.0 * Cin0p * C0 * ldz, lib.o3d_mlp_conv_fwd, X0n.data_ptr(), W0p.data_ptr(), None, None, 1,
              Cin0p, C0, ldz, Z.data_ptr(), None, None, st)
        vecs = [_eval_vec(lib, bn, bn.weight, bn.bias, st) for _, bn in layers]
        outs = []
        for s_, sg in enumerate(segs):
            npoint = sg[3].shape[1]
            centers = None
            if nxyz:
                centers = sg[1].detach().reshape(-1, 3)
                centers = (centers * inv_radius if inv_radius != 1.0 else centers).contiguous()
            out = torch.empty((B, Ws[2].shape[0], npoint), device=dev, dtype=f32)
            _call("sa_eval_fused", 0.0, lib.o3d_sa_eval_fused, Z.data_ptr(), ldz, sg[3].data_ptr(), _ptr(centers),
                  Ws[0].data_ptr(), Cin0, vecs[0].data_ptr(), Ws[1].data_ptr(), vecs[1].data_ptr(), Ws[2].data_ptr(),
                  vecs[2].data_ptr(), C0, Ws[1].shape[0], Ws[2].shape[0], B, npoint, ns, Npads[s_], pt_bases[s_],
                  out.data_ptr(), st)
            outs.append(out)
    return outs


def _compact_ok(layers, npoint, ns, B):
    if ns > 64 or B * npoint > (1 << 20) or B * npoint * ns >= (1 << 30):
        return False
    for i, (conv, _) in enumerate(layers):
        if i >= 1 and (conv.in_channels % 64 or conv.out_channels % 64):
            return False
    return layers[0][0].out_channels % 64 == 0


def _run(mlp, xyz, new_xyz, feats, idx, nxyz, inv_radius):
    layers = _layers(mlp)
    cfg = _Cfg()
    cfg.nxyz, cfg.inv_radius, cfg.training = nxyz, float(inv_radius), bool(mlp.training)
    cfg.bns = [bn for _, bn in layers]
    params = []
    for conv, bn in layers:
        params += [conv.weight, bn.weight, bn.bias]
    B, npoint, ns = idx.shape
    if _eval_fused_ok(mlp, layers, [(xyz, new_xyz, feats, idx)], nxyz):
        return _run_eval(mlp, layers, [(xyz, new_xyz, feats, idx)], nxyz, float(inv_radius))[0]
# ... 166 lines not shown
```

Measured before the change: 9228 pairs/s.

## Recompute SA0 layer-0 activations from xyz geometry instead of materializing them

For the first set-abstraction MLP, the layer-0 output (a 3-input linear map of relative xyz) is no longer stored. The forward pass runs a stats-only expand kernel, and the layer-1 forward conv, fused layer-1 backward and layer-0 weight-grad kernels rebuild Y0 on the fly from gathered points, centers and W0. This removes writing and re-reading a 64×ldp fp32 tensor, at the cost of extra gathers and FMAs inside the GEMM-style kernels, plus shared-memory setup for a new B_GEO operand mode.

```diff
diff --git a/include/o3dsot.h b/include/o3dsot.h
--- a/include/o3dsot.h
+++ b/include/o3dsot.h
@@ -121,6 +121,23 @@
 int o3d_group_expand_c3(const float* X3, long ldz, const int32_t* gp, const int32_t* cball, const float* cw,
                         const float* centers, const float* W0, int ldw, int C0, const int32_t* meta, long start1, long ldp,
                         float* Y0, float* part, const float* stat_c, void* stream);
+
+int o3d_group_expand_c3_stats(const float* X3, long ldz, const int32_t* gp, const int32_t* cball, const float* cw,
+                              const float* centers, const float* W0, int ldw, int C0, const int32_t* meta, long start1,
+                              long ldp, float* part, const float* stat_c, void* stream);
+int o3d_mlp_conv_fwd_c3(const float* X3, long ldz, const int32_t* gp, const int32_t* cball, const float* centers,
+                        const float* W0, int ldw, const float* W, const float* in_scale, const float* in_shift, int Cout,
+                        long ldp, const float* w, const int32_t* meta, long start1, int tile, float* Y, float* part,
+                        const float* stat_c, void* stream);
+int o3d_mlp_conv_bwd_fused_c3(const float* dN, const float* Y, const float* A1, const float* A2, const float* A3,
+                              const float* X3, long ldz, const int32_t* gp, const int32_t* cball, const float* centers,
+                              const float* W0, int ldw, const float* in_scale, const float* in_shift, const float* in_mean,
+                              const float* Wt, long ldp, const float* w, const int32_t* meta, long start1, float* scratch,
+                              float* dW, float* part_s, float* dNprev, void* stream);
+int o3d_group_dw0_xyz_c3(const float* dN, long ldp, const float* A1, const float* A2, const float* A3, const int32_t* gp,
+                         const int32_t* cball, const float* cw, const float* X, long ldz, const float* centers,
+                         const float* W0, int ldw, const int32_t* meta, long start1, int C0, float* part, float* dW,
+                         void* stream);
 
 int o3d_direct_tile(long P, int M, int compact);
 int o3d_direct_tail_slots(int M);
diff --git a/open3dsot_amd/csrc/compact.hip b/open3dsot_amd/csrc/compact.hip
--- a/open3dsot_amd/csrc/compact.hip
+++ b/open3dsot_amd/csrc/compact.hip
@@ -1,5 +1,6 @@
 #include <cstdlib>
 #include "o3d_common.hpp"
+#include "sa0_layer0.hpp"
 
 namespace {
 
@@ -70,7 +71,7 @@
     cw[q] = k == 0 ? (float)(1 + ns - cnt) : 1.f;
 }
 
-template <bool CENTERS, bool DIRECT = false>
+template <bool CENTERS, bool DIRECT = false, bool STORE = true>
 __global__ __launch_bounds__(256) void expand_c_kernel(const float* __restrict__ Z, long ldz,
                                                        const int32_t* __restrict__ gp,
                                                        const int32_t* __restrict__ cball,
@@ -100,7 +101,10 @@
         if constexpr (DIRECT) {
             const int ids[4] = {id.x, id.y, id.z, id.w};
 #pragma unroll
-            for (int t = 0; t < 4; ++t) { cx[t] -= Z[ids[t]]; cy[t] -= Z[ldz + ids[t]]; cz[t] -= Z[2 * ldz + ids[t]]; }
+            for (int t = 0; t < 4; ++t) {
+                const Sa0Rel r = sa0_rel(Z[ids[t]], Z[ldz + ids[t]], Z[2 * ldz + ids[t]], cx[t], cy[t], cz[t]);
+                cx[t] = r.x; cy[t] = r.y; cz[t] = r.z;
+            }
         }
     }
     constexpr int EG = 8;
@@ -127,11 +131,18 @@
         for (int g = 0; g < EG; ++g) {
             const int co = g0 + 4 * g;
             if (co >= cend) { s[g] = 0.f; v[g] = 0.f; continue; }
-            y[g].x -= fmaf(w2[g], cz[0], fmaf(w1[g], cy[0], w0[g] * cx[0]));
-            y[g].y -= fmaf(w2[g], cz[1], fmaf(w1[g], cy[1], w0[g] * cx[1]));
-            y[g].z -= fmaf(w2[g], cz[2], fmaf(w1[g], cy[2], w0[g] * cx[2]));
-            y[g].w -= fmaf(w2[g], cz[3], fmaf(w1[g], cy[3], w0[g] * cx[3]));
-            *reinterpret_cast<float4*>(&Y0[(long)co * ldp + q]) = y[g];
+            if constexpr (DIRECT) {
+                y[g].x = sa0_y0(w0[g], w1[g], w2[g], Sa0Rel{cx[0], cy[0], cz[0]});
+                y[g].y = sa0_y0(w0[g], w1[g], w2[g], Sa0Rel{cx[1], cy[1], cz[1]});
+                y[g].z = sa0_y0(w0[g], w1[g], w2[g], Sa0Rel{cx[2], cy[2], cz[2]});
+                y[g].w = sa0_y0(w0[g], w1[g], w2[g], Sa0Rel{cx[3], cy[3], cz[3]});
+            } else {
+                y[g].x -= fmaf(w2[g], cz[0], fmaf(w1[g], cy[0], w0[g] * cx[0]));
+                y[g].y -= fmaf(w2[g], cz[1], fmaf(w1[g], cy[1], w0[g] * cx[1]));
+                y[g].z -= fmaf(w2[g], cz[2], fmaf(w1[g], cy[2], w0[g] * cx[2]));
+                y[g].w -= fmaf(w2[g], cz[3], fmaf(w1[g], cy[3], w0[g] * cx[3]));
+            }
+            if constexpr (STORE) *reinterpret_cast<float4*>(&Y0[(long)co * ldp + q]) = y[g];
             const float c = sc_[g];
             s[g] = fmaf(w.x, y[g].x, fmaf(w.y, y[g].y, fmaf(w.z, y[g].z, w.w * y[g].w)));
             v[g] = w.x * (y[g].x - c) * (y[g].x - c) + w.y * (y[g].y - c) * (y[g].y - c) +
@@ -894,7 +905,7 @@
 }
 
 namespace {
-template <int CPW>
+template <int CPW, bool RECOMPUTE = false>
 __global__ __launch_bounds__(256) void dw0_xyz_kernel(const float* __restrict__ dN, const float* __restrict__ Y0, long ldp,
                                                       const float* __restrict__ A1, const float* __restrict__ A2,
                                                       const float* __restrict__ A3, const int32_t* __restrict__ gp,
@@ -902,7 +913,8 @@
                                                       const float* __restrict__ X, long ldz,
                                                       const float* __restrict__ centers,
                                                       const int32_t* __restrict__ meta, long start1, int C0,
-                                                      float* __restrict__ part) {
+                                                      float* __restrict__ part, const float* __restrict__ W0 = nullptr,
+                                                      int ldw = 0) {
     const long q0 = (long)blockIdx.x * 256;
     const int seg = (start1 > 0 && q0 >= start1) ? 1 : 0;
     float* prow = part + (long)blockIdx.x * C0 * 3;
@@ -918,11 +930,20 @@
     const int ids[4] = {id.x, id.y, id.z, id.w}, bb[4] = {bj.x, bj.y, bj.z, bj.w};
     const float wv[4] = {w.x, w.y, w.z, w.w};
     float rel[4][3];
-#pragma unroll
-    for (int t = 0; t < 4; ++t)
-#pragma unroll
-        for (int k = 0; k < 3; ++k)
-            rel[t][k] = wv[t] != 0.f ? X[(long)k * ldz + ids[t]] - centers[(long)bb[t] * 3 + k] : 0.f;
+    Sa0Rel yrel[4];
+    if constexpr (RECOMPUTE) {
+#pragma unroll
+        for (int t = 0; t < 4; ++t) {
+            yrel[t] = sa0_rel_gather(X, ldz, centers, ids[t], bb[t]);
+            rel[t][0] = -yrel[t].x; rel[t][1] = -yrel[t].y; rel[t][2] = -yrel[t].z;
+        }
+    } else {
+#pragma unroll
+        for (int t = 0; t < 4; ++t)
+#pragma unroll
+            for (int k = 0; k < 3; ++k)
+                rel[t][k] = wv[t] != 0.f ? X[(long)k * ldz + ids[t]] - centers[(long)bb[t] * 3 + k] : 0.f;
+    }
     const float* a1 = A1 + seg * C0;
     const float* a2 = A2 + seg * C0;
     const float* a3 = A3 + seg * C0;
@@ -934,13 +955,21 @@
             const int c = cbase + wave + 4 * i;
             const int cc = c < C0 ? c : C0 - 1;
             d[i] = *reinterpret_cast<const float4*>(&dN[(long)cc * ldp + q]);
-            y[i] = *reinterpret_cast<const float4*>(&Y0[(long)cc * ldp + q]);
+            if constexpr (RECOMPUTE) {
+                const float* wr = W0 + (long)cc * ldw;
+                y[i] = make_float4(wr[0], wr[1], wr[2], 0.f);
+            } else {
+                y[i] = *reinterpret_cast<const float4*>(&Y0[(long)cc * ldp + q]);
+            }
         }
 #pragma unroll
         for (int i = 0; i < CPW; ++i) {
             const int c = cbase + wave + 4 * i;
             const int cc = c < C0 ? c : C0 - 1;
             const float k1 = a1[cc], k2 = a2[cc], k3 = a3[cc];
+            if constexpr (RECOMPUTE)
+                y[i] = make_float4(sa0_y0(y[i].x, y[i].y, y[i].z, yrel[0]), sa0_y0(y[i].x, y[i].y, y[i].z, yrel[1]),
+                                   sa0_y0(y[i].x, y[i].y, y[i].z, yrel[2]), sa0_y0(y[i].x, y[i].y, y[i].z, yrel[3]));
             const float dv[4] = {d[i].x, d[i].y, d[i].z, d[i].w}, yv[4] = {y[i].x, y[i].y, y[i].z, y[i].w};
             float s0 = 0.f, s1 = 0.f, s2 = 0.f;
 #pragma unroll
@@ -986,6 +1015,21 @@
     const int nblk = (int)(ldp / 256);
     hipLaunchKernelGGL(dw0_xyz_kernel<8>, dim3(nblk), dim3(256), 0, s, dN, Y0, ldp, A1, A2, A3, gp, cball, cw, X, ldz, centers,
                        meta, start1, C0, part);
+    hipLaunchKernelGGL(dw0_reduce_kernel, dim3(C0 * 3), dim3(256), 0, s, part, nblk, C0 * 3, dW);
+    return o3d_launch_status();
+}
+
+extern "C" int o3d_group_dw0_xyz_c3(const float* dN, long ldp, const float* A1, const float* A2, const float* A3,
+                                    const int32_t* gp, const int32_t* cball, const float* cw, const float* X, long ldz,
+                                    const float* centers, const float* W0, int ldw, const int32_t* meta, long start1, int C0,
+                                    float* part, float* dW, void* stream) {
+    if (!dN || !A1 || !A2 || !A3 || !gp || !cball || !cw || !X || !centers || !W0 || ldw < 3 || !meta || !part || !dW ||
+        C0 <= 0 || ldp <= 0 || ldp % 256 != 0 || ldz <= 0 || start1 < 0 || start1 % 256 != 0)
+        return O3D_EINVAL;
+    hipStream_t s = o3d_stream(stream);
+    const int nblk = (int)(ldp / 256);
+    hipLaunchKernelGGL((dw0_xyz_kernel<8, true>), dim3(nblk), dim3(256), 0, s, dN, nullptr, ldp, A1, A2, A3, gp, cball, cw, X,
+                       ldz, centers, meta, start1, C0, part, W0, ldw);
     hipLaunchKernelGGL(dw0_reduce_kernel, dim3(C0 * 3), dim3(256), 0, s, part, nblk, C0 * 3, dW);
     return o3d_launch_status();
 }
@@ -1109,6 +1153,19 @@
     const int ysplit = C0 >= 128 ? 4 : C0 >= 64 ? 2 : 1;
     hipLaunchKernelGGL((expand_c_kernel<true, true>), dim3((unsigned)(ldp / 256), ysplit), dim3(256), 0, o3d_stream(stream),
                        X3, ldz, gp, cball, cw, centers, W0, ldw, C0, meta, start1, ldp, Y0, part, stat_c);
+    return o3d_launch_status();
+}
+
+extern "C" int o3d_group_expand_c3_stats(const float* X3, long ldz, const int32_t* gp, const int32_t* cball, const float* cw,
+                                         const float* centers, const float* W0, int ldw, int C0, const int32_t* meta,
+                                         long start1, long ldp, float* part, const float* stat_c, void* stream) {
+    if (!X3 || !gp || !cball || !cw || !centers || !W0 || ldw < 3 || !meta || !part || C0 <= 0 || ldp <= 0 ||
+        ldp % 256 != 0 || start1 < 0 || start1 % 256 != 0)
+        return O3D_EINVAL;
+    const int ysplit = C0 >= 128 ? 4 : C0 >= 64 ? 2 : 1;
+    hipLaunchKernelGGL((expand_c_kernel<true, true, false>), dim3((unsigned)(ldp / 256), ysplit), dim3(256), 0,
+                       o3d_stream(stream), X3, ldz, gp, cball, cw, centers, W0, ldw, C0, meta, start1, ldp, nullptr, part,
+                       stat_c);
     return o3d_launch_status();
 }
 
diff --git a/open3dsot_amd/csrc/mlp_direct.hip b/open3dsot_amd/csrc/mlp_direct.hip
--- a/open3dsot_amd/csrc/mlp_direct.hip
+++ b/open3dsot_amd/csrc/mlp_direct.hip
@@ -1,5 +1,6 @@
 #include <type_traits>
 #include "mlp_common.hpp"
+#include "sa0_layer0.hpp"
 
 namespace {
 
@@ -18,6 +19,18 @@
     }
 }
 template <int NT>
+__device__ __forceinline__ void ldvi(int (&d)[NT], const int32_t* p) {
+    if constexpr (NT == 4) {
+        const int4 t = *reinterpret_cast<const int4*>(p);
+        d[0] = t.x; d[1] = t.y; d[2] = t.z; d[3] = t.w;
+    } else if constexpr (NT == 2) {
+        const int2 t = *reinterpret_cast<const int2*>(p);
+        d[0] = t.x; d[1] = t.y;
+    } else {
+        d[0] = *p;
+    }
+}
+template <int NT>
 __device__ __forceinline__ void stv(float* p, const float (&d)[NT]) {
     if constexpr (NT == 4)      *reinterpret_cast<float4*>(p) = make_float4(d[0], d[1], d[2], d[3]);
     else if constexpr (NT == 2) *reinterpret_cast<float2*>(p) = make_float2(d[0], d[1]);
@@ -29,9 +42,13 @@
     float v[4][NT];
     float y[4][NT];
     float4 c1, c2, c3;
+    float4 g[4];
 };
 
-enum BMode { B_PLAIN = 0, B_XFORM = 1, B_DY = 2, B_DYPOOL = 3 };
+enum BMode { B_PLAIN = 0, B_XFORM = 1, B_DY = 2, B_DYPOOL = 3, B_GEO = 4 };
+constexpr int GEO_K = 64;
+constexpr bool b_has_y(int mode) { return mode == B_DY || mode == B_DYPOOL; }
+constexpr bool b_splitk_mode(int mode) { return mode <= B_DY || mode == B_GEO; }
 
 struct DirectArgs {
     const float* A;
@@ -51,15 +68,38 @@
     const float* resid;
     const float* cbias; int cb_N, cb_B;
     int tail_slots; long extra_row0;
+    Sa0Src geo;
 };
+
+template <int NT, int NTHREADS>
+__device__ __forceinline__ void geo_setup(const DirectArgs& a, long p, float4* gtab, float* gsh, Sa0Rel (&gr)[NT]) {
+    for (int k = threadIdx.x; k < GEO_K; k += NTHREADS) {
+        const float* wr = a.geo.W0 + (long)k * a.geo.ldw;
+        gtab[k] = make_float4(wr[0], wr[1], wr[2], a.c1[k]);
+        gsh[k] = a.c2[k];
+    }
+    int ids[NT], bb[NT];
+    ldvi<NT>(ids, a.geo.gp + p);
+    ldvi<NT>(bb, a.geo.cball + p);
+#pragma unroll
+    for (int t = 0; t < NT; ++t) gr[t] = sa0_rel_gather(a.geo.X3, a.geo.ldz, a.geo.centers, ids[t], bb[t]);
+    __syncthreads();
+}
 
 template <int MODE, int NT>
 __device__ __forceinline__ void load_b(const DirectArgs& a, const float* xb, const float* yb, long rowP, int kb,
-                                       long pool_base, int np, RawB<NT>& f) {
+                                       long pool_base, int np, RawB<NT>& f, const float4* gtab = nullptr,
+                                       const float* gsh = nullptr) {
+    if constexpr (MODE == B_GEO) {
+#pragma unroll
+        for (int s = 0; s < 4; ++s) f.g[s] = gtab[kb + s];
+        f.c2 = *reinterpret_cast<const float4*>(gsh + kb);
+        return;
+    }
 #pragma unroll
     for (int s = 0; s < 4; ++s) {
         if (MODE != B_DYPOOL) ldv<NT>(f.v[s], xb + (long)(kb + s) * rowP);
-        if (MODE >= B_DY) ldv<NT>(f.y[s], yb + (long)(kb + s) * rowP);
+        if (b_has_y(MODE)) ldv<NT>(f.y[s], yb + (long)(kb + s) * rowP);
         if constexpr (MODE == B_DYPOOL && NT >= 2) {
             const float2 t = a.pk[pool_base + (long)(kb + s) * np];
             f.v[s][0] = t.x; f.v[s][1] = t.y;
@@ -68,13 +108,13 @@
     if (MODE != B_PLAIN) {
         f.c1 = *reinterpret_cast<const float4*>(a.c1 + kb);
         f.c2 = *reinterpret_cast<const float4*>(a.c2 + kb);
-        if (MODE >= B_DY) f.c3 = *reinterpret_cast<const float4*>(a.c3 + kb);
+        if (b_has_y(MODE)) f.c3 = *reinterpret_cast<const float4*>(a.c3 + kb);
     }
 }
 
 template <int MODE, int NT, int MT>
 __device__ __forceinline__ void compute_group(const RawB<NT>& f, const float4& a0v, const float4& a1v, int kk,
-                                              const float (&wv)[NT], f32x16 (&acc)[MT][NT]) {
+                                              const float (&wv)[NT], f32x16 (&acc)[MT][NT], const Sa0Rel (&gr)[NT]) {
     const float a0[4] = {a0v.x, a0v.y, a0v.z, a0v.w}, a1[4] = {a1v.x, a1v.y, a1v.z, a1v.w};
     const float c1[4] = {f.c1.x, f.c1.y, f.c1.z, f.c1.w}, c2[4] = {f.c2.x, f.c2.y, f.c2.z, f.c2.w};
     const float c3[4] = {f.c3.x, f.c3.y, f.c3.z, f.c3.w};
@@ -86,6 +126,9 @@
             const int ak = __float_as_int(f.v[s][1]);
 #pragma unroll
             for (int t = 0; t < NT; ++t) bv[t] = (kk + t == ak) ? go : 0.f;
+        } else if constexpr (MODE == B_GEO) {
+#pragma unroll
+            for (int t = 0; t < NT; ++t) bv[t] = fmaxf(fmaf(sa0_y0(f.g[s].x, f.g[s].y, f.g[s].z, gr[t]), f.g[s].w, c2[s]), 0.f);
         } else {
 #pragma unroll
             for (int t = 0; t < NT; ++t) bv[t] = f.v[s][t];
@@ -93,7 +136,7 @@
         if (MODE == B_XFORM) {
 #pragma unroll
             for (int t = 0; t < NT; ++t) bv[t] = fmaxf(fmaf(bv[t], c1[s], c2[s]), 0.f);
-        } else if (MODE >= B_DY) {
+        } else if (b_has_y(MODE)) {
 #pragma unroll
             for (int t = 0; t < NT; ++t) bv[t] = fmaf(c1[s], bv[t], wv[t] * fmaf(c2[s], f.y[s][t], c3[s]));
         }
@@ -133,10 +176,19 @@
     for (int t = 0; t < NT; ++t) wv[t] = 1.f;
     if (a.w) ldv<NT>(wv, a.w + (long)b * a.P + p);
     const long rowP = a.P;
-    const float* xb = (MODE != B_DYPOOL) ? a.X + (long)b * a.K * rowP + p : nullptr;
-    const float* yb = (MODE >= B_DY) ? a.Y + (long)b * a.K * rowP + p : nullptr;
+    const float* xb = (MODE != B_DYPOOL && MODE != B_GEO) ? a.X + (long)b * a.K * rowP + p : nullptr;
+    const float* yb = b_has_y(MODE) ? a.Y + (long)b * a.K * rowP + p : nullptr;
     const float* wa = a.A + (long)(m0 + l31) * a.K + 4 * h;
     const long wstep = 32L * a.K;
+    Sa0Rel gr[NT] = {};
+    const float4* gtab = nullptr;
+    const float* gsh = nullptr;
+    if constexpr (MODE == B_GEO) {
+        __shared__ float4 gtab_s[GEO_K];
+        __shared__ __attribute__((aligned(16))) float gsh_s[GEO_K];
+        geo_setup<NT, WAVES * 64>(a, (long)b * a.P + p, gtab_s, gsh_s, gr);
+        gtab = gtab_s; gsh = gsh_s;
+    }
     int np = 1, kk = 0;
     long pool_base = 0;
     if (MODE == B_DYPOOL) {
@@ -160,7 +212,7 @@
     auto load = [&](auto stc, int g) {
         constexpr int st = decltype(stc)::value;
         const int kb = 8 * g + 4 * h;
-        load_b<MODE, NT>(a, xb, yb, rowP, kb, pool_base, np, f[st]);
+        load_b<MODE, NT>(a, xb, yb, rowP, kb, pool_base, np, f[st], gtab, gsh);
         wa0[st] = *reinterpret_cast<const float4*>(wa + 8 * g);
         if constexpr (MT == 2) wa1[st] = *reinterpret_cast<const float4*>(wa + 8 * g + wstep);
         else wa1[st] = wa0[st];
@@ -170,11 +222,11 @@
         for (int g = 0; g < G; g += 2) {
             load(std::integral_constant<int, 1>{}, g + 1);
             __builtin_amdgcn_sched_barrier(0);
-            compute_group<MODE, NT, MT>(f[0], wa0[0], wa1[0], kk, wv, acc);
+            compute_group<MODE, NT, MT>(f[0], wa0[0], wa1[0], kk, wv, acc, gr);
             __builtin_amdgcn_sched_barrier(0);
             load(std::integral_constant<int, 0>{}, g + 2 < G ? g + 2 : G - 1);
             __builtin_amdgcn_sched_barrier(0);
-            compute_group<MODE, NT, MT>(f[1], wa0[1], wa1[1], kk, wv, acc);
+            compute_group<MODE, NT, MT>(f[1], wa0[1], wa1[1], kk, wv, acc, gr);
             __builtin_amdgcn_sched_barrier(0);
         }
     }
@@ -333,7 +385,7 @@
 
 template <int MODE, int EPI>
 __device__ __forceinline__ void splitk_body(DirectArgs& a, const int bx, const int by, float* __restrict__ red) {
-    static_assert(MODE <= B_DY && EPI <= 2, "split-K tile: plain / transformed / BatchNorm-backward operands only");
+    static_assert(b_splitk_mode(MODE) && EPI <= 2, "split-K tile: plain / transformed / BatchNorm-backward operands only");
     constexpr int NT = 2;
     const int lane = threadIdx.x & 63, wave = threadIdx.x >> 6;
     const int l31 = lane & 31, h = lane >> 5;
@@ -357,9 +409,18 @@
     float wv[NT] = {1.f, 1.f};
     if (a.w) ldv<NT>(wv, a.w + (long)b * a.P + p);
     const long rowP = a.P;
-    const float* xb = a.X + (long)b * a.K * rowP + p;
-    const float* yb = (MODE >= B_DY) ? a.Y + (long)b * a.K * rowP + p : nullptr;
+    const float* xb = MODE != B_GEO ? a.X + (long)b * a.K * rowP + p : nullptr;
+    const float* yb = b_has_y(MODE) ? a.Y + (long)b * a.K * rowP + p : nullptr;
     const float* wa = a.A + (long)(m0 + l31) * a.K + 4 * h;
+    Sa0Rel gr[NT] = {};
+    const float4* gtab = nullptr;
+    const float* gsh = nullptr;
+    if constexpr (MODE == B_GEO) {
+        __shared__ float4 gtab_s[GEO_K];
+        __shared__ __attribute__((aligned(16))) float gsh_s[GEO_K];
+        geo_setup<NT, 256>(a, (long)b * a.P + p, gtab_s, gsh_s, gr);
+        gtab = gtab_s; gsh = gsh_s;
+    }
 
     const int mrow = m0 + 8 * wave + 4 * h;
     const long ob = ((long)b * a.M + mrow) * rowP + p;
@@ -397,7 +458,7 @@
     float4 wa0[2];
     auto load = [&](auto stc, int g) {
         constexpr int st = decltype(stc)::value;
-        load_b<MODE, NT>(a, xb, yb, rowP, 8 * g + 4 * h, 0, 1, f[st]);
+        load_b<MODE, NT>(a, xb, yb, rowP, 8 * g + 4 * h, 0, 1, f[st], gtab, gsh);
         wa0[st] = *reinterpret_cast<const float4*>(wa + 8 * g);
     };
     if (gs < ge) {
@@ -405,11 +466,11 @@
         for (int g = gs; g < ge; g += 2) {
             load(std::integral_constant<int, 1>{}, g + 1);
             __builtin_amdgcn_sched_barrier(0);
-            compute_group<MODE, NT, 1>(f[0], wa0[0], wa0[0], 0, wv, acc);
+            compute_group<MODE, NT, 1>(f[0], wa0[0], wa0[0], 0, wv, acc, gr);
             __builtin_amdgcn_sched_barrier(0);
             load(std::integral_constant<int, 0>{}, g + 2 < ge ? g + 2 : ge - 1);
             __builtin_amdgcn_sched_barrier(0);
-            compute_group<MODE, NT, 1>(f[1], wa0[1], wa0[1], 0, wv, acc);
+            compute_group<MODE, NT, 1>(f[1], wa0[1], wa0[1], 0, wv, acc, gr);
             __builtin_amdgcn_sched_barrier(0);
         }
     }
@@ -486,7 +547,7 @@
 }
 template <int MODE, int EPI>
 int launch_splitk(const DirectArgs& a, hipStream_t st) {
-    if constexpr (MODE <= B_DY && EPI <= 2) {
+    if constexpr (b_splitk_mode(MODE) && EPI <= 2) {
         hipLaunchKernelGGL((splitk_gemm_kernel<MODE, EPI>), dim3(a.B * (a.P / SK_COLS), a.M / SK_ROWS), dim3(256), 0, st, a);
         return o3d_launch_status();
     } else {
@@ -538,7 +599,7 @@
 
 template <int MODE, int EPI>
 int launch_direct(const DirectArgs& a, int tile, hipStream_t st) {
-    if constexpr (MODE <= B_DY && EPI <= 2) {
+    if constexpr (b_splitk_mode(MODE) && EPI <= 2) {
         if (splitk_ok(a, tile)) return launch_splitk<MODE, EPI>(a, st);
     }
     return tile == 64 ? launch_direct_nt<MODE, EPI, 2>(a, st) : launch_direct_nt<MODE, EPI, 4>(a, st);
@@ -591,6 +652,23 @@
     a.part = part; a.stat_c = stat_c; a.ns = 4;
     if (meta && tile == 128 && B == 1 && in_scale) { a.tail_slots = o3d_direct_tail_slots(Cout); a.extra_row0 = P / 128; }
     return in_scale ? launch_direct<B_XFORM, 0>(a, tile, st) : launch_direct<B_PLAIN, 0>(a, tile, st);
+}
+
+extern "C" int o3d_mlp_conv_fwd_c3(const float* X3, long ldz, const int32_t* gp, const int32_t* cball, const float* centers,
+                                   const float* W0, int ldw, const float* W, const float* in_scale, const float* in_shift,
+                                   int Cout, long ldp, const float* w, const int32_t* meta, long start1, int tile, float* Y,
+                                   float* part, const float* stat_c, void* stream) {
+    if (!X3 || ldz <= 0 || !gp || !cball || !centers || !W0 || ldw < 3 || !W || !in_scale || !in_shift || !w || !meta || !Y ||
+        ldp <= 0 || ldp > 0x7fffffff || !o3d_direct_ok(Cout, GEO_K, (int)ldp) || (tile != 64 && tile != 128) || start1 < 0 ||
+        start1 % 256 != 0)
+        return O3D_EINVAL;
+    DirectArgs a = {};
+    a.w = w; a.meta = meta; a.start1 = start1;
+    a.A = W; a.c1 = in_scale; a.c2 = in_shift; a.Out = Y; a.M = Cout; a.K = GEO_K; a.P = (int)ldp; a.B = 1;
+    a.part = part; a.stat_c = stat_c; a.ns = 4;
+    a.geo.X3 = X3; a.geo.ldz = ldz; a.geo.gp = gp; a.geo.cball = cball; a.geo.centers = centers; a.geo.W0 = W0; a.geo.ldw = ldw;
+    if (tile == 128) { a.tail_slots = o3d_direct_tail_slots(Cout); a.extra_row0 = ldp / 128; }
+    return launch_direct<B_GEO, 0>(a, tile, o3d_stream(stream));
 }
 
 int o3d_direct_dgrad(const float* dN, const float* pk, int ns,
diff --git a/open3dsot_amd/csrc/mlp_wgrad.hip b/open3dsot_amd/csrc/mlp_wgrad.hip
--- a/open3dsot_amd/csrc/mlp_wgrad.hip
+++ b/open3dsot_amd/csrc/mlp_wgrad.hip
@@ -1,4 +1,5 @@
 #include "mlp_common.hpp"
+#include "sa0_layer0.hpp"
 
 namespace {
 
@@ -297,9 +298,10 @@
     float* part_w;
     float* part_s;
     float* dX;
+    Sa0Src geo;
 };
 
-template <int TM>
+template <int TM, bool GEO = false>
 __global__ __launch_bounds__(256) void fused_bwd_kernel(FusedBwdArgs a) {
     constexpr int TN = 64;
     constexpr int WM = TM / 64, WK = 4 / WM;
@@ -358,17 +360,43 @@
 
     float4 rg[PA], ry[PA], rx[PB];
     float4 rw = make_float4(1.f, 1.f, 1.f, 1.f);
+    typedef float f32x3 __attribute__((ext_vector_type(3)));
+    float gw[PB][3], gpt[3] = {0.f, 0.f, 0.f};
+    f32x3 gct = {0.f, 0.f, 0.f};
+    int gi_p = 0, gi_b = 0, ni_p = 0, ni_b = 0;
+    float* relbuf = smem + 2 * ((TM + TN) * LD);
+    auto chunk_col = [&](int chl) -> long { return (col0 / CP + (chl < c_end ? chl : c_end - 1)) * CP + lane; };
+    auto geo_index = [&](int chl) { ni_p = a.geo.gp[chunk_col(chl)]; ni_b = a.geo.cball[chunk_col(chl)]; };
+    auto geo_gather = [&]() {
+#pragma unroll
+        for (int k = 0; k < 3; ++k) gpt[k] = a.geo.X3[(long)k * a.geo.ldz + gi_p];
+        __builtin_memcpy(&gct, a.geo.centers + (long)gi_b * 3, 12);
+    };
+    auto geo_publish = [&](int buf) {
+        const Sa0Rel r = sa0_rel(gpt[0], gpt[1], gpt[2], gct.x, gct.y, gct.z);
+        float* d = relbuf + buf * 3 * CP + lane;
+        d[0] = r.x; d[CP] = r.y; d[2 * CP] = r.z;
+    };
+    if constexpr (GEO) {
+        static_assert(!GEO || CP == 64, "one column per lane of wave 0");
+#pragma unroll
+        for (int i = 0; i < PB; ++i)
+#pragma unroll
+            for (int k = 0; k < 3; ++k) gw[i][k] = a.geo.W0[(long)(r0 + RPP * i) * a.geo.ldw + k];
+    }
     auto load_chunk = [&](int chl) {
         const long p = (col0 / CP + chl) * CP + 4 * c4;
-        if (a.w) rw = *reinterpret_cast<const float4*>(&a.w[p]);
+        if (GEO || a.w) rw = *reinterpret_cast<const float4*>(&a.w[p]);
 #pragma unroll
         for (int i = 0; i < PA; ++i) {
             const long row = r0 + RPP * i;
             ry[i] = *reinterpret_cast<const float4*>(&a.Y[row * a.P + p]);
             rg[i] = *reinterpret_cast<const float4*>(&a.dN[row * a.P + p]);
         }
-#pragma unroll
-        for (int i = 0; i < PB; ++i) rx[i] = *reinterpret_cast<const float4*>(&a.X[(long)(r0 + RPP * i) * a.P + p]);
+        if constexpr (!GEO) {
+#pragma unroll
+            for (int i = 0; i < PB; ++i) rx[i] = *reinterpret_cast<const float4*>(&a.X[(long)(r0 + RPP * i) * a.P + p]);
+        }
     };
     auto store_chunk = [&](int buf) {
 #pragma unroll
@@ -380,6 +408,16 @@
             o.w = fmaf(ka1[i], rg[i].w, rw.w * fmaf(ka2[i], ry[i].w, ka3[i]));
             *reinterpret_cast<float4*>(&As(buf)[(r0 + RPP * i) * LD + 4 * c4]) = o;
         }
+        if constexpr (GEO) {
+            const float* rb = relbuf + buf * 3 * CP + 4 * c4;
+            const float4 qx = *reinterpret_cast<const float4*>(rb), qy = *reinterpret_cast<const float4*>(rb + CP),
+                         qz = *reinterpret_cast<const float4*>(rb + 2 * CP);
+            const Sa0Rel rel[4] = {{qx.x, qy.x, qz.x}, {qx.y, qy.y, qz.y}, {qx.z, qy.z, qz.z}, {qx.w, qy.w, qz.w}};
+#pragma unroll
+            for (int i = 0; i < PB; ++i)
+                rx[i] = make_float4(sa0_y0(gw[i][0], gw[i][1], gw[i][2], rel[0]), sa0_y0(gw[i][0], gw[i][1], gw[i][2], rel[1]),
+                                    sa0_y0(gw[i][0], gw[i][1], gw[i][2], rel[2]), sa0_y0(gw[i][0], gw[i][1], gw[i][2], rel[3]));
+        }
 #pragma unroll
         for (int i = 0; i < PB; ++i) {
             float4 v = rx[i];
@@ -402,12 +440,37 @@
     for (int r = 0; r < 32; ++r) sacc[r] = 0.f;
 
     if (c_begin < c_end) {
-        load_chunk(c_begin);
+        if constexpr (GEO) {
+            load_chunk(c_begin);
+            {
+                geo_index(c_begin);
+                gi_p = ni_p; gi_b = ni_b;
+                geo_index(c_begin + 1);
+                geo_gather();
+                if (wave == 0) geo_publish(0);
+                gi_p = ni_p; gi_b = ni_b;
+                geo_index(c_begin + 2);
+                geo_gather();
+                if (wave == 0) geo_publish(1);
+                gi_p = ni_p; gi_b = ni_b;
+            }
+            __syncthreads();
+        } else {
+            load_chunk(c_begin);
+        }
         store_chunk(0);
         __syncthreads();
         for (int ch = c_begin; ch < c_end; ++ch) {
             const int t = ch - c_begin;
-            if (ch + 1 < c_end) load_chunk(ch + 1);
+            if constexpr (GEO) {
+                geo_index(ch + 3);
+                geo_gather();
+                __builtin_amdgcn_sched_barrier(0);
+                load_chunk(ch + 1 < c_end ? ch + 1 : ch);
+                __builtin_amdgcn_sched_barrier(0);
+            } else {
+                if (ch + 1 < c_end) load_chunk(ch + 1);
+            }
             const float* A_ = As(t & 1);
             const float* B_ = Bs(t & 1);
             {
@@ -430,6 +493,13 @@
 #pragma unroll
                             for (int tn = 0; tn < 2; ++tn) acc[tm][tn] = mfma32(av[tm][s], bv[tn][s], acc[tm][tn]);
                 }
+            }
+            if constexpr (GEO) {
+                __builtin_amdgcn_sched_barrier(0);
+                asm volatile("" : "+v"(ni_p), "+v"(ni_b), "+v"(gpt[0]), "+v"(gpt[1]), "+v"(gpt[2]));
+                if (wave == 0) geo_publish(t & 1);
+                gi_p = ni_p; gi_b = ni_b;
+                __builtin_amdgcn_sched_barrier(0);
             }
             if (dactive) {
                 f32x16 d;
@@ -456,6 +526,7 @@
                     sacc[16 + r] = fmaf(gq, xt, sacc[16 + r]);
                 }
             }
+            if constexpr (GEO) __builtin_amdgcn_sched_barrier(0);
             if (ch + 1 < c_end) store_chunk((t + 1) & 1);
             __syncthreads();
         }
@@ -483,8 +554,17 @@
             float t2 = 0.f;
             for (int ch = c_begin; ch < c_end; ++ch) {
                 const long qb = (col0 / CP + ch) * CP + 32 * dpt;
-                for (int j = 0; j < 32; ++j)
-                    t2 = fmaf(a.dX[(long)ci * a.P + qb + j], a.X[(long)ci * a.P + qb + j] - mu, t2);
+                for (int j = 0; j < 32; ++j) {
+                    float yp;
+                    if constexpr (GEO) {
+                        const float* wr = a.geo.W0 + (long)ci * a.geo.ldw;
+                        yp = sa0_y0(wr[0], wr[1], wr[2], sa0_rel_gather(a.geo.X3, a.geo.ldz, a.geo.centers, a.geo.gp[qb + j],
+                                                                        a.geo.cball[qb + j]));
+                    } else {
+                        yp = a.X[(long)ci * a.P + qb + j];
+                    }
+                    t2 = fmaf(a.dX[(long)ci * a.P + qb + j], yp - mu, t2);
+                }
             }
             s2 = t2;
         }
@@ -496,14 +576,14 @@
     }
 }
 
-template <int TM>
+template <int TM, bool GEO = false>
 int launch_fused_bwd(const FusedBwdArgs& a, hipStream_t s) {
     constexpr int CP = (TM + 64 == 128) ? 64 : 32;
-    const size_t lds = sizeof(float) * 2 * (TM + 64) * (CP + 4);
-    const void* fn = reinterpret_cast<const void*>(fused_bwd_kernel<TM>);
+    const size_t lds = sizeof(float) * (2 * (TM + 64) * (CP + 4) + (GEO ? 2 * 3 * CP : 0));
+    const void* fn = reinterpret_cast<const void*>(fused_bwd_kernel<TM, GEO>);
     if (lds > 48 * 1024 && hipFuncSetAttribute(fn, hipFuncAttributeMaxDynamicSharedMemorySize, (int)lds) != hipSuccess)
         return -3;
-    hipLaunchKernelGGL((fused_bwd_kernel<TM>), dim3(a.nslices), dim3(256), lds, s, a);
+    hipLaunchKernelGGL((fused_bwd_kernel<TM, GEO>), dim3(a.nslices), dim3(256), lds, s, a);
     return hipGetLastError() == hipSuccess ? 0 : -3;
 }
 
@@ -679,3 +759,30 @@
     o3d_wgrad_reduce(scratch, nsl * (4 / (Cout / 64)), n, dW, s);
     return o3d_launch_status();
 }
+
+extern "C" int o3d_mlp_conv_bwd_fused_c3(const float* dN, const float* Y, const float* A1, const float* A2, const float* A3,
+                                         const float* X3, long ldz, const int32_t* gp, const int32_t* cball,
+                                         const float* centers, const float* W0, int ldw, const float* in_scale,
+                                         const float* in_shift, const float* in_mean, const float* Wt, long ldp, const float* w,
+                                         const int32_t* meta, long start1, float* scratch, float* dW, float* part_s,
+                                         float* dNprev, void* stream) {
+    const int Cin = 64, Cout = 64;
+    if (!dN || !Y || !A1 || !A2 || !A3 || !X3 || ldz <= 0 || !gp || !cball || !centers || !W0 || ldw < 3 || !in_scale ||
+        !in_shift || !in_mean || !Wt || !scratch || !dW || !part_s || !dNprev || !fused_bwd_ok(Cin, Cout, ldp) || !meta || !w ||
+        start1 < 0 || start1 % 256 != 0)
+        return O3D_EINVAL;
+    const int CP = 64;
+    const int nsl = fused_bwd_slices(Cout, ldp);
+    FusedBwdArgs a = {};
+    a.dN = dN; a.Y = Y; a.A1 = A1; a.A2 = A2; a.A3 = A3; a.in_scale = in_scale; a.in_shift = in_shift;
+    a.in_mean = in_mean; a.Wt = Wt; a.Cin = Cin; a.Cout = Cout; a.P = (int)ldp;
+    a.total_chunks = (int)(ldp / CP);
+    a.chunks_per_block = (a.total_chunks + nsl - 1) / nsl;
+    a.nslices = nsl;
+    a.w = w; a.meta = meta; a.start1 = start1; a.part_w = scratch; a.part_s = part_s; a.dX = dNprev;
+    a.geo.X3 = X3; a.geo.ldz = ldz; a.geo.gp = gp; a.geo.cball = cball; a.geo.centers = centers; a.geo.W0 = W0; a.geo.ldw = ldw;
+    hipStream_t s = o3d_stream(stream);
+    if (launch_fused_bwd<64, true>(a, s) != 0) return O3D_ELAUNCH;
+    o3d_wgrad_reduce(scratch, nsl * 4, (long)Cout * Cin, dW, s);
+    return o3d_launch_status();
+}
diff --git a/open3dsot_amd/csrc/sa0_layer0.hpp b/open3dsot_amd/csrc/sa0_layer0.hpp
--- /dev/null
+++ b/open3dsot_amd/csrc/sa0_layer0.hpp
@@ -0,0 +1,28 @@
+#pragma once
+#include "o3d_common.hpp"
+
+struct Sa0Rel { float x, y, z; };
+
+__device__ __forceinline__ Sa0Rel sa0_rel(float px, float py, float pz, float cx, float cy, float cz) {
+    Sa0Rel r;
+    r.x = cx - px; r.y = cy - py; r.z = cz - pz;
+    return r;
+}
+
+__device__ __forceinline__ Sa0Rel sa0_rel_gather(const float* __restrict__ X3, long ldz, const float* __restrict__ centers,
+                                                 int point, int ball) {
+    const float* c = centers + (long)ball * 3;
+    return sa0_rel(X3[point], X3[ldz + point], X3[2 * ldz + point], c[0], c[1], c[2]);
+}
+
+__device__ __forceinline__ float sa0_y0(float w0, float w1, float w2, const Sa0Rel& r) {
+    return 0.f - fmaf(w2, r.z, fmaf(w1, r.y, w0 * r.x));
+}
+
+struct Sa0Src {
+    const float* X3; long ldz;
+    const int32_t* gp;
+    const int32_t* cball;
+    const float* centers;
+    const float* W0; int ldw;
+};
diff --git a/open3dsot_amd/fused.py b/open3dsot_amd/fused.py
--- a/open3dsot_amd/fused.py
+++ b/open3dsot_amd/fused.py
@@ -398,6 +398,9 @@
                   None, None, 1, Cin0p, C0, ldz, Z.data_ptr(), None, None, st, dims=(Cin0p, C0))
         counts = [float(pm) for pm in Pmaxs]
         Ys, means, invstds, scales, shifts = [], [], [], [], []
+        recompute0 = (direct3 and cfg.training and need_bwd and L >= 2 and C0 == 64 and tuple(Ws[1].shape) == (64, 64)
+                      and not any(ctx.needs_input_grad[2 + 4 * s_ + k] for s_ in range(nseg) for k in (0, 1))
+                      and FUSED_BWD_MAX_COUT >= 64 and lib.o3d_mlp_conv_bwd_fused_rows(64, 64, ldp) > 0)
         if cfg.training:
             if nseg == 1:
                 statcs = [bn.running_mean.detach().unsqueeze(0) for bn in cfg.bns]
@@ -407,11 +410,15 @@
             Cout, Cin = Ws[l].shape
             bn = cfg.bns[l]
             tile = ETILE if l == 0 else _direct_tile(lib, ldp, Cout)
-            Y = torch.empty((Cout, ldp), device=dev, dtype=f32)
+            Y = torch.empty((Cout, ldp), device=dev, dtype=f32) if not (l == 0 and recompute0) else None
             part = torch.empty((ldp // tile + _tail_rows(lib, tile, Cout, nseg, l), 2, Cout), device=dev, dtype=f32) \
                 if cfg.training else None
             statc = statcs[l] if cfg.training else None
-            if l == 0 and direct3:
+            if l == 0 and recompute0:
+                _call("group_expand", 0.0, lib.o3d_group_expand_c3_stats, X0n.data_ptr(), ldz, gp.data_ptr(), cball.data_ptr(),
+                      cw.data_ptr(), centers.data_ptr(), Ws[0].data_ptr(), Cin0, C0, meta.data_ptr(), start1, ldp,
+                      part.data_ptr(), _ptr(statc), st)
+            elif l == 0 and direct3:
                 _call("group_expand", 0.0, lib.o3d_group_expand_c3, X0n.data_ptr(), ldz, gp.data_ptr(), cball.data_ptr(),
                       cw.data_ptr(), centers.data_ptr(), Ws[0].data_ptr(), Cin0, C0, meta.data_ptr(), start1, ldp,
                       Y.data_ptr(), _ptr(part), _ptr(statc), st)
@@ -419,6 +426,11 @@
                 _call("group_expand", 0.0, lib.o3d_group_expand_c, Z.data_ptr(), ldz, gp.data_ptr(), cball.data_ptr(),
                       cw.data_ptr(), _ptr(centers), Ws[0].data_ptr(), Cin0, C0, meta.data_ptr(), start1, ldp, Y.data_ptr(),
                       _ptr(part), _ptr(statc), st)
+            elif l == 1 and recompute0:
+                _call("conv_fwd", (2.0 * Cin * Cout, meta, ldp), lib.o3d_mlp_conv_fwd_c3, X0n.data_ptr(), ldz, gp.data_ptr(),
+                      cball.data_ptr(), centers.data_ptr(), Ws[0].data_ptr(), Cin0, Ws[l].data_ptr(), scales[-1].data_ptr(),
+                      shifts[-1].data_ptr(), Cout, ldp, cw.data_ptr(), meta.data_ptr(), start1, tile, Y.data_ptr(),
+                      _ptr(part), _ptr(statc), st, dims=(Cin, Cout))
             else:
                 _call("conv_fwd", (2.0 * Cin * Cout, meta, ldp), lib.o3d_mlp_conv_fwd_c, Ys[-1].data_ptr(), Ws[l].data_ptr(),
                       scales[-1].data_ptr(), shifts[-1].data_ptr(), Cin, Cout, ldp, cw.data_ptr(), meta.data_ptr(), start1,
@@ -526,6 +538,12 @@
             if l == 0 and C == 0 and nxyz == 3 and not (want_xyz or want_feats):
                 part0 = torch.empty((ldp // 256, Cout, 3), device=dev, dtype=f32)
                 dW = torch.empty((Cout, 3), device=dev, dtype=f32)
+                if Ys[0] is None:
+                    _call("group_dw0", 0.0, lib.o3d_group_dw0_xyz_c3, dN.data_ptr(), ldp, A[0], A[1], A[2], gp.data_ptr(),
+                          cball.data_ptr(), cw.data_ptr(), X0n.data_ptr(), ldz, centers.data_ptr(), Ws[0].data_ptr(),
+                          Ws[0].shape[1], meta.data_ptr(), start1, Cout, part0.data_ptr(), dW.data_ptr(), st)
+                    grads[0] = dW
+                    continue
                 _call("group_dw0", 0.0, lib.o3d_group_dw0_xyz, dN.data_ptr(), Ys[0].data_ptr(), ldp, A[0], A[1], A[2],
                       gp.data_ptr(), cball.data_ptr(), cw.data_ptr(), X0n.data_ptr(), ldz, centers.data_ptr(), meta.data_ptr(),
                       start1, Cout, part0.data_ptr(), dW.data_ptr(), st)
@@ -606,6 +624,15 @@
                 wpart = torch.empty((lib.o3d_mlp_conv_bwd_fused_scratch(Cin, Cout, ldp),), device=dev, dtype=f32)
                 dNp = torch.empty((Cin, ldp), device=dev, dtype=f32)
                 part = torch.empty((2, rows_fb, 2, Cin), device=dev, dtype=f32)
+                if Ys[l - 1] is None:
+                    _call("conv_bwd_fused", (4.0 * Cin * Cout, meta, ldp), lib.o3d_mlp_conv_bwd_fused_c3, dN.data_ptr(),
+                          Ys[l].data_ptr(), A[0], A[1], A[2], X0n.data_ptr(), ldz, gp.data_ptr(), cball.data_ptr(),
+                          centers.data_ptr(), Ws[0].data_ptr(), Ws[0].shape[1], scales[0].data_ptr(), shifts[0].data_ptr(),
+                          means[0].data_ptr(), ctx.Wts[l].data_ptr(), ldp, cw.data_ptr(), meta.data_ptr(), start1,
+                          wpart.data_ptr(), dW.data_ptr(), part.data_ptr(), dNp.data_ptr(), st, dims=(Cin, Cout))
+                    grads[3 * l] = dW
+                    dN, part_rows = dNp, rows_fb
+                    continue
                 _call("conv_bwd_fused", (4.0 * Cin * Cout, meta, ldp), lib.o3d_mlp_conv_bwd_fused_c, dN.data_ptr(),
                       Ys[l].data_ptr(), A[0], A[1], A[2], Ys[l - 1].data_ptr(), scales[l - 1].data_ptr(),
                       shifts[l - 1].data_ptr(), means[l - 1].data_ptr(), ctx.Wts[l].data_ptr(), Cin, Cout, ldp, cw.data_ptr(),
```

After: 9305 pairs/s, median of 6. About the same (+0.8%).
